# AIGC-Audio/AudioGPT

Hardware: AMD Instinct MI355X
Metric: generated audio-seconds/sec (10s clip, 100 DDIM steps) [3 independent batches of 8 prompts in flight per GPU] (higher is better)
Workload: dtype bf16x3; 1 GPU; Make-An-Audio T2A batch=8/GPU, 100 DDIM steps, CFG 1.5, UNet+VAE+HiFi-GAN(16k), fp32 storage, bf16x3-split MFMA (hi/lo, fp32 accumulate; meets the fp32 parity gates); prompts_per_gpu=8, ddim_steps=100, mel_frames=624, hipgraph=True, batches_in_flight=3, cfg_lanes=1, concurrency_hint=3, parallelism=prompt-sharded x1 (RCCL bcast cond / gather wav)

## Files before the change

### audiogpt_amd/_lib.py

```python
import ctypes as C
import os

import torch

_HERE = os.path.dirname(os.path.abspath(__file__))
LIB_PATH = os.environ.get("AUDIOGPT_AMD_LIB") or os.path.join(_HERE, "libaudiogpt_mi355x.so")


class MaaError(RuntimeError):
    pass


class maa_tensor(C.Structure):
    _fields_ = [("name", C.c_char_p), ("data", C.POINTER(C.c_float)), ("ndim", C.c_int), ("shape", C.c_int64 * 6)]


class maa_prof_row(C.Structure):
    _fields_ = [("name", C.c_char * 48), ("launches", C.c_int64), ("ms", C.c_double), ("flops", C.c_double),
                ("bytes", C.c_double)]


class maa_unet_config(C.Structure):
    _fields_ = [("in_channels", C.c_int), ("out_channels", C.c_int), ("model_channels", C.c_int),
                ("num_res_blocks", C.c_int),
                ("n_channel_mult", C.c_int), ("channel_mult", C.c_int * 8),
                ("n_attention_resolutions", C.c_int), ("attention_resolutions", C.c_int * 8),
                ("num_heads", C.c_int), ("num_head_channels", C.c_int),
                ("use_spatial_transformer", C.c_int), ("transformer_depth", C.c_int), ("context_dim", C.c_int),
                ("legacy", C.c_int), ("resblock_updown", C.c_int), ("add_context_to_emb", C.c_int)]


class maa_ddim_args(C.Structure):
    _fields_ = [("S", C.c_int), ("B", C.c_int), ("C", C.c_int), ("H", C.c_int), ("W", C.c_int),
                ("scale", C.c_float),
                ("d_cond", C.c_void_p), ("d_uncond", C.c_void_p), ("L", C.c_int),
                ("d_concat", C.c_void_p), ("Cc", C.c_int),
                ("h_timesteps", C.POINTER(C.c_int32)), ("h_alphas", C.POINTER(C.c_float)),
                ("h_alphas_prev", C.POINTER(C.c_float)), ("use_graph", C.c_int),
                ("d_mask", C.c_void_p), ("d_x0", C.c_void_p), ("d_noise_q", C.c_void_p),
                ("h_sqrt_ac", C.POINTER(C.c_float)), ("h_sqrt_1mac", C.POINTER(C.c_float)),
                ("h_sigmas", C.POINTER(C.c_float)), ("d_noise_p", C.c_void_p), ("temperature", C.c_float),
                ("log_every_t", C.c_int), ("n_log", C.c_int), ("d_log_x", C.c_void_p), ("d_log_x0", C.c_void_p),
                ("split_kh", C.c_int), ("split_kw", C.c_int), ("split_sh", C.c_int), ("split_sw", C.c_int),
                ("h_split_weight", C.POINTER(C.c_float))]


class maa_ddpm_args(C.Structure):
    _fields_ = [("loop", maa_ddim_args), ("start", C.c_int), ("n", C.c_int), ("clip_denoised", C.c_int),
                ("h_sqrt_recip_ac", C.POINTER(C.c_float)), ("h_sqrt_recipm1_ac", C.POINTER(C.c_float)),
                ("h_coef1", C.POINTER(C.c_float)), ("h_coef2", C.POINTER(C.c_float)), ("h_logvar", C.POINTER(C.c_float)),
                ("h_sqrt_ac", C.POINTER(C.c_float)), ("h_sqrt_1mac", C.POINTER(C.c_float)),
                ("h_temperature", C.POINTER(C.c_float))]


class maa_vae_config(C.Structure):
    _fields_ = [("ch", C.c_int), ("out_ch", C.c_int), ("in_channels", C.c_int), ("z_channels", C.c_int),
                ("embed_dim", C.c_int), ("resolution", C.c_int), ("num_res_blocks", C.c_int), ("double_z", C.c_int),
                ("n_ch_mult", C.c_int), ("ch_mult", C.c_int * 8),
                ("n_attn_resolutions", C.c_int), ("attn_resolutions", C.c_int * 8)]


class maa_vocoder_config(C.Structure):
    _fields_ = [("kind", C.c_int), ("num_mels", C.c_int), ("upsample_initial_channel", C.c_int),
                ("n_upsamples", C.c_int), ("upsample_rates", C.c_int * 8), ("upsample_kernel_sizes", C.c_int * 8),
                ("n_kernels", C.c_int), ("resblock_kernel_sizes", C.c_int * 8),
                ("n_dilations", C.c_int), ("resblock_dilation_sizes", (C.c_int * 8) * 8),
                ("snake_beta", C.c_int), ("snake_logscale", C.c_int),
                ("use_pitch_embed", C.c_int), ("sampling_rate", C.c_int), ("harmonic_num", C.c_int),
                ("resblock", C.c_int)]


class maa_diffnet_config(C.Structure):
    _fields_ = [("in_dims", C.c_int), ("hidden_size", C.c_int), ("residual_layers", C.c_int),
                ("residual_channels", C.c_int), ("dilation_cycle_length", C.c_int)]


class maa_pitch_extractor_config(C.Structure):
    _fields_ = [("n_mel_bins", C.c_int), ("hidden_size", C.c_int), ("predictor_hidden", C.c_int), ("predictor_kernel", C.c_int),
                ("conv_layers", C.c_int), ("ffn_padding_same", C.c_int), ("use_uv", C.c_int), ("pitch_norm", C.c_int),
                ("f0_mean", C.c_float), ("f0_std", C.c_float)]


class maa_encoder_config(C.Structure):
    _fields_ = [("kind", C.c_int), ("layers", C.c_int), ("width", C.c_int), ("heads", C.c_int), ("mlp_dim", C.c_int),
                ("d_proj", C.c_int), ("vocab", C.c_int), ("max_positions", C.c_int), ("patch", C.c_int),
                ("image", C.c_int), ("ln_eps", C.c_float)]


class maa_clap_audio_config(C.Structure):
    _fields_ = [("mel_bins", C.c_int), ("n_blocks", C.c_int), ("channels", C.c_int * 8), ("out_emb", C.c_int),
                ("d_proj", C.c_int), ("bn_eps", C.c_float)]


class maa_spectral_config(C.Structure):
    _fields_ = [("n_fft", C.c_int), ("hop", C.c_int), ("n_freq", C.c_int), ("n_mels", C.c_int), ("pad_mode", C.c_int),
                ("power", C.c_int), ("log_kind", C.c_int), ("amin", C.c_float), ("ref", C.c_float), ("out_layout", C.c_int)]


class maa_plms_args(C.Structure):
    _fields_ = [("B", C.c_int), ("T", C.c_int), ("K_step", C.c_int), ("interval", C.c_int), ("timesteps", C.c_int),
                ("d_cond", C.c_void_p), ("h_alphas_cumprod", C.POINTER(C.c_float)), ("use_graph", C.c_int)]


class maa_ds_ddpm_args(C.Structure):
    _fields_ = [("B", C.c_int), ("T", C.c_int), ("start", C.c_int), ("n", C.c_int), ("timesteps", C.c_int),
                ("clip_denoised", C.c_int), ("use_graph", C.c_int),
                ("d_cond", C.c_void_p), ("d_noise", C.c_void_p),
                ("h_sqrt_recip_ac", C.POINTER(C.c_float)), ("h_sqrt_recipm1_ac", C.POINTER(C.c_float)),
                ("h_coef1", C.POINTER(C.c_float)), ("h_coef2", C.POINTER(C.c_float)), ("h_sigma", C.POINTER(C.c_float))]


EXPORTS = [
    "maa_last_error", "maa_version", "maa_ctx_create", "maa_ctx_destroy", "maa_ctx_synchronize",
    "maa_ctx_set_stream", "maa_ctx_set_precision", "maa_ctx_set_cfg_split", "maa_ctx_set_concurrency", "maa_ctx_reload_tuning", "maa_ctx_workspace_bytes", "maa_prof_begin", "maa_prof_end", "maa_unet_create", "maa_unet_destroy",
    "maa_unet_set_context", "maa_unet_forward", "maa_ddim_update", "maa_ddim_sample", "maa_ddim_stochastic_encode", "maa_ddim_decode",
    "maa_ldm_plms_sample", "maa_ddpm_sample", "maa_ddpm_update",
    "maa_vae_create",
    "maa_vae_destroy", "maa_vae_decode", "maa_vae_decode_spec", "maa_vae_encode_moments", "maa_vocoder_create", "maa_vocoder_destroy",
    "maa_vocoder_forward", "maa_vocoder_forward_f0", "maa_diffnet_create", "maa_diffnet_destroy", "maa_diffnet_forward",
    "maa_plms_sample", "maa_ds_ddpm_sample", "maa_ds_ddpm_update",
    "maa_pitch_extractor_create", "maa_pitch_extractor_destroy", "maa_pitch_extractor_forward",
    "maa_encoder_create", "maa_encoder_destroy", "maa_encoder_text", "maa_encoder_image",
    "maa_encoder_text_cls", "maa_clap_audio_create", "maa_clap_audio_destroy", "maa_clap_audio_embed", "maa_clap_similarity",
    "maa_spectral_create", "maa_spectral_destroy", "maa_spectral_forward", "maa_resampler_create", "maa_resampler_destroy",
    "maa_resampler_forward", "maa_op_linear", "maa_op_conv", "maa_op_groupnorm", "maa_op_layernorm",
    "maa_op_attention", "maa_op_attention_ex", "maa_op_conv_transpose1d", "maa_op_snake_aa", "maa_op_bench_conv", "maa_calib",
    "maa_op_mrf_pair", "maa_op_groupnorm_ex", "maa_op_layernorm_ex", "maa_op_split32",
    "maa_unet_forward_split", "maa_op_unfold", "maa_op_fold",
]

_lib = None


def load():
    global _lib
    if _lib is not None:
        return _lib
    if not os.path.exists(LIB_PATH):
        raise MaaError("%s not found -- run `python -m audiogpt_amd.build` (hipcc, gfx950)" % LIB_PATH)
    try:
        lib = C.CDLL(LIB_PATH)
    except OSError as e:
        raise MaaError("cannot load %s: %s" % (LIB_PATH, e))
    vp, ci, cf, fp = C.c_void_p, C.c_int, C.c_float, C.POINTER(C.c_float)
    lib.maa_last_error.restype = C.c_char_p
    lib.maa_version.restype = C.c_char_p
    sig = {
        "maa_ctx_create": [ci, vp, C.POINTER(vp)],
        "maa_ctx_destroy": [vp],
        "maa_ctx_synchronize": [vp],
        "maa_ctx_set_stream": [vp, vp],
        "maa_ctx_workspace_bytes": [vp, C.POINTER(C.c_size_t)],
        "maa_ctx_set_precision": [vp, ci],
        "maa_ctx_set_cfg_split": [vp, ci],
        "maa_ctx_set_concurrency": [vp, ci],
        "maa_ctx_reload_tuning": [vp],
        "maa_prof_begin": [vp, ci],
        "maa_prof_end": [vp, C.POINTER(maa_prof_row), ci, C.POINTER(ci)],
        "maa_unet_create": [vp, C.POINTER(maa_unet_config), C.POINTER(maa_tensor), ci, C.POINTER(vp)],
        "maa_unet_destroy": [vp],
        "maa_unet_set_context": [vp, vp, vp, ci, ci],
        "maa_unet_forward": [vp, vp, vp, vp, ci, ci, ci, vp],
        "maa_ddim_update": [vp, vp, vp, vp, cf, vp, C.c_int64, vp, vp],
        "maa_ddim_sample": [vp, vp, C.POINTER(maa_ddim_args), vp],
        "maa_ddim_stochastic_encode": [vp, vp, ci, cf, vp, vp, fp, fp, ci, vp, ci, ci, ci, ci, vp],
        "maa_ddim_decode": [vp, vp, C.POINTER(maa_ddim_args), ci, vp],
        "maa_ldm_plms_sample": [vp, vp, C.POINTER(maa_ddim_args), vp],
        "maa_ddpm_sample": [vp, vp, C.POINTER(maa_ddpm_args), vp],
        "maa_ddpm_update": [vp, vp, vp, vp, fp, fp, fp, fp, fp, ci, vp, cf, ci, ci, ci, ci, ci, vp, vp],
        "maa_vae_create": [vp, C.POINTER(maa_vae_config), C.POINTER(maa_tensor), ci, C.POINTER(vp)],
        "maa_vae_destroy": [vp],
        "maa_vae_decode": [vp, vp, vp, ci, ci, ci, cf, vp],
        "maa_vae_decode_spec": [vp, vp, vp, ci, ci, ci, cf, vp],
        "maa_vae_encode_moments": [vp, vp, vp, ci, ci, ci, vp],
        "maa_vocoder_create": [vp, C.POINTER(maa_vocoder_config), C.POINTER(maa_tensor), ci, C.POINTER(vp)],
        "maa_vocoder_destroy": [vp],
        "maa_vocoder_forward": [vp, vp, vp, ci, ci, vp],
        "maa_vocoder_forward_f0": [vp, vp, vp, vp, vp, vp, ci, ci, vp],
        "maa_diffnet_create": [vp, C.POINTER(maa_diffnet_config), C.POINTER(maa_tensor), ci, C.POINTER(vp)],
        "maa_diffnet_destroy": [vp],
        "maa_diffnet_forward": [vp, vp, vp, vp, vp, ci, ci, vp],
        "maa_plms_sample": [vp, vp, C.POINTER(maa_plms_args), vp],
        "maa_ds_ddpm_sample": [vp, vp, C.POINTER(maa_ds_ddpm_args), vp],
        "maa_ds_ddpm_update": [vp, vp, vp, vp, fp, fp, fp, fp, fp, ci, ci, ci, ci, ci, vp],
        "maa_pitch_extractor_create": [vp, C.POINTER(maa_pitch_extractor_config), C.POINTER(maa_tensor), ci, C.POINTER(vp)],
        "maa_pitch_extractor_destroy": [vp],
        "maa_pitch_extractor_forward": [vp, vp, vp, ci, ci, vp, vp, vp],
        "maa_encoder_create": [vp, C.POINTER(maa_encoder_config), C.POINTER(maa_tensor), ci, C.POINTER(vp)],
        "maa_encoder_destroy": [vp],
        "maa_encoder_text": [vp, vp, vp, ci, ci, vp],
        "maa_encoder_image": [vp, vp, vp, ci, vp],
        "maa_encoder_text_cls": [vp, vp, vp, ci, ci, vp],
        "maa_clap_audio_create": [vp, C.POINTER(maa_clap_audio_config), C.POINTER(maa_tensor), ci, C.POINTER(vp)],
        "maa_clap_audio_destroy": [vp],
        "maa_clap_audio_embed": [vp, vp, vp, ci, ci, vp, vp],
        "maa_clap_similarity": [vp, vp, vp, ci, ci, ci, cf, vp],
        "maa_spectral_create": [vp, C.POINTER(maa_spectral_config), fp, fp, C.POINTER(vp)],
        "maa_spectral_destroy": [vp],
        "maa_spectral_forward": [vp, vp, vp, ci, ci, vp],
        "maa_resampler_create": [vp, ci, ci, ci, ci, fp, C.POINTER(vp)],
        "maa_resampler_destroy": [vp],
        "maa_resampler_forward": [vp, vp, vp, ci, ci, vp],
        "maa_op_linear": [vp, vp, ci, ci, fp, fp, ci, ci, vp, vp, ci],
        "maa_op_conv": [vp, vp, ci, ci, ci, ci, fp, fp, ci, ci, ci, ci, ci, ci, ci, cf, vp, ci, ci, vp, vp, ci],
        "maa_op_groupnorm": [vp, vp, ci, ci, ci, fp, fp, cf, ci, vp],
        "maa_op_layernorm": [vp, vp, ci, ci, fp, fp, cf, vp],
        "maa_op_attention": [vp, vp, vp, vp, ci, ci, ci, ci, ci, cf, vp],
        "maa_op_attention_ex": [vp, vp, ci, ci, vp, ci, ci, vp, ci, ci, ci, ci, ci, ci, ci, cf, vp, ci, ci, ci],
        "maa_op_conv_transpose1d": [vp, vp, ci, ci, ci, fp, fp, ci, ci, ci, cf, vp],
        "maa_op_snake_aa": [vp, vp, ci, ci, ci, fp, fp, ci, vp],
        "maa_op_bench_conv": [vp, ci, ci, ci, ci, ci, ci, ci, ci, C.POINTER(C.c_float)],
        "maa_calib": [vp, ci, C.POINTER(C.c_double)],
        "maa_op_mrf_pair": [vp, vp, ci, ci, ci, fp, fp, ci, ci, cf, fp, fp, ci, ci, cf, cf, ci, vp],
        "maa_op_groupnorm_ex": [vp, vp, ci, ci, vp, ci, ci, ci, ci, ci, fp, fp, cf, ci, vp, ci, vp],
        "maa_op_layernorm_ex": [vp, vp, ci, ci, fp, fp, cf, vp, ci],
        "maa_op_split32": [vp, vp, ci, ci, cf, ci, vp],
        "maa_unet_forward_split": [vp, vp, vp, vp, vp, ci, ci, ci, ci, ci, ci, ci, fp, vp],
        "maa_op_unfold": [vp, vp, ci, ci, ci, ci, ci, ci, ci, ci, vp],
        "maa_op_fold": [vp, vp, fp, ci, ci, ci, ci, ci, ci, ci, ci, vp],
    }
    for name, argtypes in sig.items():
        fn = getattr(lib, name)
        fn.argtypes = argtypes
        fn.restype = ci
    _lib = lib
    return lib


def check(status):
    if status != 0:
        raise MaaError("libaudiogpt_mi355x: %s (status %d)" % (load().maa_last_error().decode(), status))


def host_f32(t):
    t = t.detach().to(device="cpu", dtype=torch.float32).contiguous()
    return t, C.cast(t.data_ptr(), C.POINTER(C.c_float))


def tensor_list(state_dict):
    items = list(state_dict.items())
    arr = (maa_tensor * len(items))()
    keep = []
    for i, (name, t) in enumerate(items):
        ht, ptr = host_f32(t)
        bname = name.encode()
        keep.append((ht, bname))
        arr[i].name = bname
        arr[i].data = ptr
        arr[i].ndim = ht.dim()
        for d, s in enumerate(ht.shape):
            arr[i].shape[d] = s
    return arr, len(items), keep


def dptr(t):
    assert t.is_cuda and t.dtype == torch.float32 and t.is_contiguous(), (t.device, t.dtype, t.is_contiguous())
    return C.c_void_p(t.data_ptr())
```

### audiogpt_amd/backend.py

```python
import ctypes as C
import threading
import weakref

import numpy as np
import torch

from . import _lib as L


def default_precision():
    import os
    p = os.environ.get("AUDIOGPT_AMD_PRECISION", "bf16x3")
    if p not in Context.PRECISIONS:
        raise ValueError("AUDIOGPT_AMD_PRECISION must be one of %s" % sorted(Context.PRECISIONS))
    return p


_contexts = weakref.WeakSet()


def reload_tuning():
    for c in list(_contexts):
        c.reload_tuning()


def _f32(t, device):
    return t.detach().to(device=device, dtype=torch.float32).contiguous()


class Context:

    PRECISIONS = {"f32": 0, "bf16x3": 1, "bf16": 2}

    def __init__(self, device="cuda:0", stream=None, precision="f32"):
        self.lib = L.load()
        if not torch.cuda.is_available():
            raise L.MaaError("no MI355X visible: the HIP backend has no CPU fallback")
        self.device = torch.device(device)
        idx = self.device.index if self.device.index is not None else torch.cuda.current_device()
        self.device = torch.device("cuda", idx)
        torch.cuda.set_device(idx)
        self._stream = stream
        sp = C.c_void_p(stream.cuda_stream) if stream is not None else None
        h = C.c_void_p()
        L.check(self.lib.maa_ctx_create(idx, sp, C.byref(h)))
        self.h = h
        self.lock = threading.RLock()
        self.precision = "f32"
        self.set_precision(precision)
        _contexts.add(self)

    def reload_tuning(self):
        if getattr(self, "h", None):
            with self.lock:
                L.check(self.lib.maa_ctx_reload_tuning(self.h))

    def set_precision(self, precision):
        L.check(self.lib.maa_ctx_set_precision(self.h, self.PRECISIONS[precision]))
        self.precision = precision

    def set_cfg_split(self, mode):
        L.check(self.lib.maa_ctx_set_cfg_split(self.h, -1 if mode is None else int(bool(mode))))

    def set_concurrency(self, n):
        L.check(self.lib.maa_ctx_set_concurrency(self.h, -1 if n is None else int(n)))

    def synchronize(self):
        L.check(self.lib.maa_ctx_synchronize(self.h))

    def workspace_bytes(self):
        n = C.c_size_t()
        L.check(self.lib.maa_ctx_workspace_bytes(self.h, C.byref(n)))
        return n.value

    def prof_begin(self, detail=False):
        L.check(self.lib.maa_prof_begin(self.h, int(detail)))

    def prof_end(self):
        rows = (L.maa_prof_row * 512)()
        n = C.c_int()
        L.check(self.lib.maa_prof_end(self.h, rows, 512, C.byref(n)))
        return {rows[i].name.decode(): dict(launches=int(rows[i].launches), ms=rows[i].ms, flops=rows[i].flops,
                                            bytes=rows[i].bytes) for i in range(n.value)}

    def calib(self):
        out = {}
        for kind, key in ((0, "mfma_bf16_tflops"), (1, "copy_gbs"), (2, "l2_read_gbs"), (3, "infinity_cache_read_gbs")):
            v = C.c_double()
            L.check(self.lib.maa_calib(self.h, kind, C.byref(v)))
            out[key] = v.value
        return out

    def close(self):
        if getattr(self, "h", None):
            self.lib.maa_ctx_destroy(self.h)
            self.h = None

    def __del__(self):
        try:
            self.close()
        except Exception:
            pass

    def op_linear(self, a, w, b=None, geglu=False, res=None, split_out=False):
        a = _f32(a, self.device)
        M, K = a.shape
        N = w.shape[0]
        wt, wp = L.host_f32(w)
        bt, bp = L.host_f32(b) if b is not None else (None, None)
        y = torch.empty(M, N // 2 if geglu else N, device=self.device)
        r = _f32(res, self.device) if res is not None else None
        assert r is None or tuple(r.shape) == tuple(y.shape)
        L.check(self.lib.maa_op_linear(self.h, L.dptr(a), M, K, wp, bp, N, int(geglu), L.dptr(y),
                                       L.dptr(r) if r is not None else None, int(split_out)))
        return y

    def op_conv(self, x, w, b=None, stride=1, pad=0, dil=1, up=False, leaky=0.0, out_hw=None, rowadd=None, res=None,
                split_out=False):
        x = _f32(x, self.device)
        B, Cin, H, W = x.shape
        Cout, _, KH, KW = w.shape
        if out_hw is None:
            He, We = (2 * H, 2 * W) if up else (H, W)
            ph = pad if KH > 1 else 0
            Ho = (He + 2 * ph - dil * (KH - 1) - 1) // stride + 1
            Wo = (We + 2 * pad - dil * (KW - 1) - 1) // stride + 1
        else:
            Ho, Wo = out_hw
        wt, wp = L.host_f32(w)
        bt, bp = L.host_f32(b) if b is not None else (None, None)
        y = torch.empty((B, Ho, Wo, Cout) if split_out else (B, Cout, Ho, Wo), device=self.device)
        ra = _f32(rowadd, self.device) if rowadd is not None else None
        r = _f32(res, self.device) if res is not None else None
        assert ra is None or tuple(ra.shape) == (B, Cout)
        assert r is None or tuple(r.shape) == (B, Cout, Ho, Wo)
        L.check(self.lib.maa_op_conv(self.h, L.dptr(x), B, Cin, H, W, wp, bp, Cout, KH, KW, stride, pad, dil,
                                     int(up), float(leaky), L.dptr(y), Ho, Wo, L.dptr(ra) if ra is not None else None,
                                     L.dptr(r) if r is not None else None, int(split_out)))
        return y

    def op_groupnorm(self, x, gamma, beta, eps, silu=False):
        x = _f32(x, self.device)
        B, Cc = x.shape[:2]
        HW = int(np.prod(x.shape[2:]))
        gt, gp = L.host_f32(gamma)
        bt, bp = L.host_f32(beta)
        y = torch.empty_like(x)
        L.check(self.lib.maa_op_groupnorm(self.h, L.dptr(x), B, Cc, HW, gp, bp, float(eps), int(silu), L.dptr(y)))
        return y

    def op_layernorm(self, x, gamma, beta, eps=1e-5):
        x = _f32(x, self.device)
        rows, Cc = x.reshape(-1, x.shape[-1]).shape
        gt, gp = L.host_f32(gamma)
        bt, bp = L.host_f32(beta)
        y = torch.empty_like(x)
        L.check(self.lib.maa_op_layernorm(self.h, L.dptr(x), rows, Cc, gp, bp, float(eps), L.dptr(y)))
        return y

    def op_attention(self, q, k, v, heads, alpha):
        q, k, v = _f32(q, self.device), _f32(k, self.device), _f32(v, self.device)
        B, Nq, Cc = q.shape
        Nk = k.shape[1]
        y = torch.empty_like(q)
        L.check(self.lib.maa_op_attention(self.h, L.dptr(q), L.dptr(k), L.dptr(v), B, heads, Cc // heads, Nq, Nk,
                                          float(alpha), L.dptr(y)))
        return y

    def op_attention_ex(self, q, ldq, hsq, k, ldk, hsk, v, ldv, hsv, B, heads, dh, Nq, Nk, alpha, out, ldo,
                        out_split=0, causal=0):
        for t in (q, k, v, out):
            assert t.is_cuda and t.dtype == torch.float32, (t.device, t.dtype)
        L.check(self.lib.maa_op_attention_ex(self.h, C.c_void_p(q.data_ptr()), int(ldq), int(hsq),
                                             C.c_void_p(k.data_ptr()), int(ldk), int(hsk),
                                             C.c_void_p(v.data_ptr()), int(ldv), int(hsv), int(B), int(heads), int(dh),
                                             int(Nq), int(Nk), float(alpha), C.c_void_p(out.data_ptr()), int(ldo),
                                             int(out_split), int(causal)))
        return out

    def op_groupnorm_ex(self, x1, ld1, C1, x2, ld2, C2, B, HW, groups, gamma, beta, eps, silu, out, out_split=0, raw=None):
        for t in (x1, x2, out, raw):
            assert t is None or (t.is_cuda and t.dtype == torch.float32), (t.device, t.dtype)
        gt, gp = L.host_f32(gamma)
        bt, bp = L.host_f32(beta)
        assert gt.numel() == C1 + C2 and bt.numel() == C1 + C2
        ptr = lambda t: C.c_void_p(t.data_ptr()) if t is not None else None
        L.check(self.lib.maa_op_groupnorm_ex(self.h, ptr(x1), int(ld1), int(C1), ptr(x2), int(ld2), int(C2), int(B), int(HW),
                                             int(groups), gp, bp, float(eps), int(silu), ptr(out), int(out_split), ptr(raw)))
        return out

    def op_layernorm_ex(self, x, gamma, beta, eps=1e-5, out_split=0):
        x = _f32(x, self.device)
        rows, Cc = x.reshape(-1, x.shape[-1]).shape
        gt, gp = L.host_f32(gamma)
        bt, bp = L.host_f32(beta)
        y = torch.empty_like(x)
        L.check(self.lib.maa_op_layernorm_ex(self.h, L.dptr(x), rows, Cc, gp, bp, float(eps), L.dptr(y), int(out_split)))
        return y

    def op_split32(self, x, slope=1.0, unpack=False):
        x = _f32(x, self.device)
        rows, Cc = x.shape
        y = torch.empty_like(x)
        L.check(self.lib.maa_op_split32(self.h, L.dptr(x), rows, Cc, float(slope), int(unpack), L.dptr(y)))
        return y

    def op_unfold(self, x, ks, stride):
        x = _f32(x, self.device)
        B, Cc, H, W = x.shape
        (kh, kw), (sh, sw) = ks, stride
        n = ((H - kh) // sh + 1) * ((W - kw) // sw + 1) if min(kh, kw, sh, sw) > 0 else 0
        y = torch.empty(B * max(n, 0), Cc, kh, kw, device=self.device)
        L.check(self.lib.maa_op_unfold(self.h, L.dptr(x), B, Cc, H, W, kh, kw, sh, sw, L.dptr(y)))
        return y

    def op_fold(self, crops, weight, size, ks, stride):
        crops = _f32(crops, self.device)
        (H, W), (kh, kw), (sh, sw) = size, ks, stride
        wt, wp = L.host_f32(weight)
        n = wt.shape[1]
        assert wt.shape[0] == kh * kw and crops.shape[0] % n == 0 and tuple(crops.shape[2:]) == (kh, kw)
        B, Cc = crops.shape[0] // n, crops.shape[1]
        y = torch.empty(B, Cc, H, W, device=self.device)
        L.check(self.lib.maa_op_fold(self.h, L.dptr(crops), wp, B, Cc, H, W, kh, kw, sh, sw, L.dptr(y)))
        return y

    def op_conv_transpose1d(self, x, w, b, stride, leaky=0.0):
        x = _f32(x, self.device)
        B, Cin, Ln = x.shape
        _, Cout, k = w.shape
        wt, wp = L.host_f32(w)
        bt, bp = L.host_f32(b)
        y = torch.empty(B, Cout, Ln * stride, device=self.device)
        L.check(self.lib.maa_op_conv_transpose1d(self.h, L.dptr(x), B, Cin, Ln, wp, bp, Cout, k, stride, float(leaky),
                                                 L.dptr(y)))
        return y

    def op_mrf_pair(self, x, w1, b1, d1, slope1, w2=None, b2=None, d2=1, slope2=0.0, out_scale=1.0, out=None):
        x = _f32(x, self.device)
        B, Cc, Ln = x.shape
        w1t, w1p = L.host_f32(w1)
        b1t, b1p = L.host_f32(b1) if b1 is not None else (None, None)
        w2t, w2p = L.host_f32(w2) if w2 is not None else (None, None)
        b2t, b2p = L.host_f32(b2) if b2 is not None else (None, None)
        y = _f32(out, self.device).clone() if out is not None else torch.empty_like(x)
        assert y.shape == x.shape
        L.check(self.lib.maa_op_mrf_pair(self.h, L.dptr(x), B, Cc, Ln, w1p, b1p, w1.shape[2], int(d1), float(slope1), w2p, b2p,
                                         w2.shape[2] if w2 is not None else 1, int(d2), float(slope2), float(out_scale),
                                         int(out is not None), L.dptr(y)))
        return y

    def op_bench_conv(self, B, H, W, Cin, Cout, taps=9, pre_split=True, iters=20):
        ms = C.c_float()
        L.check(self.lib.maa_op_bench_conv(self.h, B, H, W, Cin, Cout, taps, int(pre_split), iters, C.byref(ms)))
        return ms.value

    def op_snake_aa(self, x, alpha, beta, logscale):
        x = _f32(x, self.device)
        B, Cc, Ln = x.shape
        at, ap = L.host_f32(alpha)
        bt, bp = L.host_f32(beta)
        y = torch.empty_like(x)
        L.check(self.lib.maa_op_snake_aa(self.h, L.dptr(x), B, Cc, Ln, ap, bp, int(logscale), L.dptr(y)))
        return y


def _fill(arr, values):
# ... 934 lines not shown
```

### audiogpt_amd/csrc/api.cpp

```cpp
#include "models.h"

#include <cstdint>
#include <cstring>
#include <memory>

namespace maa {
const char* last_error_cstr();
}

struct maa_ctx {
    maa::Ctx c;
    bool owns_stream = false;
};
struct maa_unet {
    std::unique_ptr<maa::UNet> m;
};
struct maa_vae {
    std::unique_ptr<maa::VAE> m;
};
struct maa_vocoder {
    std::unique_ptr<maa::Vocoder> m;
};
struct maa_diffnet {
    std::unique_ptr<maa::DiffNet> m;
// ... 521 lines not shown
}

int maa_encoder_create(maa_ctx* ctx, const maa_encoder_config* cfg, const maa_tensor* tensors, int n_tensors,
                       maa_encoder** out) {
    return guarded([&] {
        bind(ctx);
        MAA_CHECK(cfg && out && cfg->kind >= 0 && cfg->kind <= 2 && cfg->layers > 0 && cfg->width > 0 && cfg->heads > 0 &&
                      cfg->width % cfg->heads == 0 && cfg->width % 4 == 0 && cfg->mlp_dim > 0 && cfg->d_proj > 0 &&
                      cfg->d_proj % 4 == 0 && cfg->ln_eps > 0.f,
                  "bad encoder config");
        if (cfg->kind != 1)
            MAA_CHECK(cfg->vocab > 0 && cfg->max_positions > 0, "bad text encoder config");
        else
            MAA_CHECK(cfg->patch > 0 && cfg->image > 0 && cfg->image % cfg->patch == 0, "bad image encoder config");
        auto sd = to_state_dict(tensors, n_tensors);
        auto* e = new maa_encoder;
        e->m.reset(new maa::Encoder(*cfg, sd, ctx->c.dtype));
        *out = e;
    });
}
int maa_encoder_destroy(maa_encoder* e) {
    return guarded([&] { delete e; });
}
int maa_encoder_text(maa_ctx* ctx, maa_encoder* e, const int* d_ids, int B, int L, float* d_out) {
    return guarded([&] {
        bind(ctx);
        MAA_CHECK(e && d_ids && d_out && B > 0 && L > 0, "bad encoder_text arguments");
        e->m->text(ctx->c, d_ids, B, L, d_out);
    });
}
int maa_encoder_image(maa_ctx* ctx, maa_encoder* e, const float* d_img, int B, float* d_out) {
    return guarded([&] {
        bind(ctx);
        MAA_CHECK(e && d_img && d_out && B > 0, "bad encoder_image arguments");
        e->m->image(ctx->c, d_img, B, d_out);
    });
}

int maa_encoder_text_cls(maa_ctx* ctx, maa_encoder* e, const int* d_ids, int B, int L, float* d_out) {
    return guarded([&] {
        bind(ctx);
        MAA_CHECK(e && d_ids && d_out && B > 0 && L > 0, "bad encoder_text_cls arguments");
        e->m->text_cls(ctx->c, d_ids, B, L, d_out);
    });
}

int maa_clap_audio_create(maa_ctx* ctx, const maa_clap_audio_config* cfg, const maa_tensor* tensors, int n_tensors,
                          maa_clap_audio** out) {
    return guarded([&] {
        bind(ctx);
        MAA_CHECK(cfg && out && cfg->mel_bins > 0 && cfg->n_blocks > 0 && cfg->n_blocks <= 8 && cfg->out_emb > 0 &&
                      cfg->d_proj > 0 && cfg->d_proj % 4 == 0 && cfg->bn_eps > 0.f,
                  "bad clap_audio config");
        for (int i = 0; i < cfg->n_blocks; ++i) MAA_CHECK(cfg->channels[i] > 0, "bad clap_audio channel list");
        auto sd = to_state_dict(tensors, n_tensors);
        auto* a = new maa_clap_audio;
        a->m.reset(new maa::ClapAudio(*cfg, sd, ctx->c.dtype));
        *out = a;
    });
}
int maa_clap_audio_destroy(maa_clap_audio* a) {
    return guarded([&] { delete a; });
}
int maa_clap_audio_embed(maa_ctx* ctx, maa_clap_audio* a, const float* d_logmel, int B, int T, float* d_embedding,
                         float* d_z) {
    return guarded([&] {
        bind(ctx);
        MAA_CHECK(a && d_logmel && d_z && B > 0 && T > 0, "bad clap_audio_embed arguments");
        a->m->embed(ctx->c, d_logmel, B, T, d_embedding, d_z);
    });
}
int maa_clap_similarity(maa_ctx* ctx, const float* d_audio, const float* d_text, int Na, int Nt, int D, float scale,
                        float* d_out) {
    return guarded([&] {
        bind(ctx);
        MAA_CHECK(d_audio && d_text && d_out && Na > 0 && Nt > 0 && D > 0, "bad clap_similarity arguments");
        maa::launch_similarity(ctx->c, d_audio, d_text, Na, Nt, D, scale, d_out);
    });
}

int maa_spectral_create(maa_ctx* ctx, const maa_spectral_config* cfg, const float* h_basis, const float* h_melw,
                        maa_spectral** out) {
    return guarded([&] {
        bind(ctx);
        MAA_CHECK(cfg && h_basis && h_melw && out, "bad spectral arguments");
        MAA_CHECK(cfg->n_fft > 0 && cfg->n_fft % 4 == 0 && cfg->hop > 0 && cfg->hop % 4 == 0 && cfg->n_freq == cfg->n_fft / 2 + 1 &&
                      cfg->n_mels > 0 && (cfg->pad_mode == 0 || cfg->pad_mode == 1) && (cfg->power == 1 || cfg->power == 2) &&
                      (cfg->log_kind == 0 || cfg->log_kind == 1) && cfg->amin > 0.f && (cfg->out_layout == 0 || cfg->out_layout == 1),
                  "bad spectral config (n_fft and hop must be multiples of 4)");
        auto* s = new maa_spectral;
        s->m.reset(new maa::Spectral(*cfg, h_basis, h_melw));
        *out = s;
    });
}
int maa_spectral_destroy(maa_spectral* s) {
    return guarded([&] { delete s; });
}
int maa_spectral_forward(maa_ctx* ctx, maa_spectral* s, const float* d_wav, int B, int n, float* d_out) {
    return guarded([&] {
        bind(ctx);
        MAA_CHECK(s && d_wav && d_out && B > 0 && n > 0, "bad spectral_forward arguments");
        MAA_CHECK(s->m->config().pad_mode == 0 || n > s->m->config().n_fft / 2, "signal too short for reflect padding");
        s->m->forward(ctx->c, d_wav, B, n, d_out);
    });
}

int maa_resampler_create(maa_ctx* ctx, int orig, int neu, int width, int klen, const float* h_kernels, maa_resampler** out) {
    return guarded([&] {
        bind(ctx);
        MAA_CHECK(out && h_kernels && orig > 0 && neu > 0 && width > 0 && klen > 0, "bad resampler arguments");
        auto* r = new maa_resampler;
        r->m.reset(new maa::Resampler(orig, neu, width, klen, h_kernels));
        *out = r;
    });
}
int maa_resampler_destroy(maa_resampler* r) {
    return guarded([&] { delete r; });
}
int maa_resampler_forward(maa_ctx* ctx, maa_resampler* r, const float* d_wav, int B, int n, float* d_out) {
    return guarded([&] {
        bind(ctx);
        MAA_CHECK(r && d_wav && d_out && B > 0 && n > 0, "bad resampler_forward arguments");
        r->m->forward(ctx->c, d_wav, B, n, d_out);
    });
}

static bool op_presplit(const maa::Ctx& c, int channels, bool other_prologue) {
    return c.tune.op_presplit && c.dtype != 0 && channels % 32 == 0 && !other_prologue;
}

int maa_op_linear(maa_ctx* ctx, const float* d_a, int M, int K, const float* h_w, const float* h_bias, int N,
                  int geglu, float* d_y, const float* d_res, int c_split) {
    return guarded([&] {
        bind(ctx);
        MAA_CHECK(d_a && h_w && d_y && M > 0 && K > 0 && N > 0, "bad op_linear arguments");
        MAA_CHECK(!c_split || N % 32 == 0, "op_linear: split32 output needs a multiple of 32 columns");
        MAA_CHECK(!geglu || (!d_res && !c_split), "op_linear: GEGLU takes neither a residual nor split32 output here");
        OneShot s;
        s.add("w", h_w, {N, K});
        if (h_bias) s.add("b", h_bias, {N});
        maa::WeightStore ws(ctx->c.dtype != 0);
        maa::Ctx& c = ctx->c;
        MAA_CHECK(!geglu || h_bias, "geglu needs a bias");
        maa::PackedW pw = geglu ? ws.pack_geglu(s.sd, "w", "b") : ws.pack_conv(s.sd, "w", h_bias ? "b" : "", 1, 1);
        const bool pre = op_presplit(c, K, false);
        maa::run_sized(c, [&] {
            const float* a = d_a;
            if (pre) {
                float* sp = c.ws.alloc_f((size_t)M * K);
                maa::launch_split32_pack(c, d_a, M, K, sp);
                a = sp;
            }
            maa::linear_into(c, a, K, M, K, pw, d_res, N, d_y, geglu ? N / 2 : N, geglu, 0, pre ? M : 0, c_split);
        });
        MAA_HIP(hipStreamSynchronize(c.stream));
    });
}

int maa_op_conv(maa_ctx* ctx, const float* d_x, int B, int Cin, int H, int W, const float* h_w, const float* h_bias,
                int Cout, int KH, int KW, int stride, int pad, int dil, int upsample2, float leaky_slope, float* d_y,
                int Ho, int Wo, const float* d_rowadd, const float* d_res, int c_split) {
    return guarded([&] {
        bind(ctx);
        MAA_CHECK(d_x && h_w && d_y, "bad op_conv arguments");
        const bool extras = d_rowadd || d_res || c_split;
        MAA_CHECK(!extras || !upsample2, "op_conv: row add, residual and split32 output are not combined with the upsample");
        MAA_CHECK(!c_split || Cout % 32 == 0, "op_conv: split32 output needs a multiple of 32 channels");
        OneShot s;
        s.add("w", h_w, {Cout, Cin, KH, KW});
        if (h_bias) s.add("b", h_bias, {Cout});
        maa::WeightStore ws(ctx->c.dtype != 0);
        maa::Ctx& c = ctx->c;
        maa::PackedW pw = ws.pack_conv(s.sd, "w", h_bias ? "b" : "", KH, KW);
        maa::PackedW pw4;
        if (upsample2 && KH == 3 && KW == 3 && stride == 1 && pad == 1 && dil == 1 && leaky_slope == 0.f)
            pw4 = ws.pack_conv_up2(s.sd, "w", h_bias ? "b" : "");
        maa::run_sized(c, [&] {
            maa::T4 x = maa::alloc_t(c, B, H, W, Cin);
            maa::launch_nchw_to_nhwc(c, d_x, B, Cin, H * W, x.p);
            if (!pw4.w && op_presplit(c, Cin, leaky_slope != 0.f)) {
                maa::T4 xs = maa::alloc_t(c, B, H, W, Cin);
                maa::launch_split32_pack(c, x.p, (long long)B * H * W, Cin, xs.p);
                xs.split = true;
                x = xs;
            }
            if (x.split && Cout <= 4 && h_bias && KH == 3 && KW == 3 && stride == 1 && pad == 1 && dil == 1 && !upsample2 && !extras && c.tune.up2) {
                maa::PackedW pn = ws.pack_narrow3x3(s.sd, "w", "b");
                if (maa::launch_narrow_conv3x3(c, x.p, Cin, B, H, W, Cin, pn.w, pn.bias, Cout, d_y)) return;
            }
            maa::T4 y = maa::alloc_t(c, B, Ho, Wo, Cout);
            maa::ConvOpt o;
            o.KH = KH;
            o.KW = KW;
            o.stride = stride;
            o.pad = pad;
            o.dil = dil;
            o.up = upsample2;
            if (leaky_slope != 0.f) {
                o.a_act = 1;
                o.a_slope = leaky_slope;
            }
            o.rowadd = d_rowadd;
            o.ld_rowadd = Cout;
            if (d_res) {
                maa::T4 r = maa::alloc_t(c, B, Ho, Wo, Cout);
                maa::launch_nchw_to_nhwc(c, d_res, B, Cout, Ho * Wo, r.p);
                o.res = r.p;
            }
            if (c_split) {
                o.c_split = 1;
                y.p = d_y;
                maa::conv_into(c, x, nullptr, pw, o, y);
                return;
            }
            if (!(pw4.w && maa::conv_up2_into(c, x, pw4, y))) maa::conv_into(c, x, nullptr, pw, o, y);
            maa::launch_nhwc_to_nchw(c, y.p, B, Cout, Ho * Wo, d_y, Cout);
        });
        MAA_HIP(hipStreamSynchronize(c.stream));
    });
}

int maa_calib(maa_ctx* ctx, int kind, double* out_value) {
    return guarded([&] {
        bind(ctx);
        MAA_CHECK(out_value && kind >= 0 && kind <= 3, "bad calib arguments");
        *out_value = maa::calib_run(ctx->c, kind);
    });
}

int maa_op_groupnorm(maa_ctx* ctx, const float* d_x, int B, int C, int HW, const float* h_gamma, const float* h_beta,
                     float eps, int silu, float* d_y) {
    return guarded([&] {
        bind(ctx);
        MAA_CHECK(d_x && h_gamma && h_beta && d_y, "bad op_groupnorm arguments");
        maa::WeightStore ws(ctx->c.dtype != 0);
        maa::Ctx& c = ctx->c;
        float* g = ws.upload(std::vector<float>(h_gamma, h_gamma + C));
        float* b = ws.upload(std::vector<float>(h_beta, h_beta + C));
        maa::run_sized(c, [&] {
            maa::T4 x = maa::alloc_t(c, B, 1, HW, C), y = maa::alloc_t(c, B, 1, HW, C);
            maa::launch_nchw_to_nhwc(c, d_x, B, C, HW, x.p);
            maa::launch_groupnorm(c, x.p, C, C, nullptr, 0, 0, B, HW, 32, g, b, eps, silu, y.p);
            maa::launch_nhwc_to_nchw(c, y.p, B, C, HW, d_y, C);
        });
        MAA_HIP(hipStreamSynchronize(c.stream));
    });
}

int maa_op_layernorm(maa_ctx* ctx, const float* d_x, int rows, int C, const float* h_gamma, const float* h_beta,
                     float eps, float* d_y) {
    return guarded([&] {
        bind(ctx);
        MAA_CHECK(d_x && h_gamma && h_beta && d_y, "bad op_layernorm arguments");
        maa::WeightStore ws(ctx->c.dtype != 0);
        maa::Ctx& c = ctx->c;
        float* g = ws.upload(std::vector<float>(h_gamma, h_gamma + C));
        float* b = ws.upload(std::vector<float>(h_beta, h_beta + C));
        maa::launch_layernorm(c, d_x, rows, C, g, b, eps, d_y);
        MAA_HIP(hipStreamSynchronize(c.stream));
    });
}

int maa_op_attention(maa_ctx* ctx, const float* d_q, const float* d_k, const float* d_v, int B, int heads, int dh,
                     int Nq, int Nk, float alpha, float* d_y) {
    return guarded([&] {
        bind(ctx);
        MAA_CHECK(d_q && d_k && d_v && d_y, "bad op_attention arguments");
        maa::Ctx& c = ctx->c;
        const int C = heads * dh;
        maa::run_sized(c, [&] {
            maa::attention_into(c, d_q, C, dh, d_k, C, dh, d_v, C, dh, B, heads, dh, Nq, Nk, alpha, d_y, C);
        });
        MAA_HIP(hipStreamSynchronize(c.stream));
    });
}

int maa_op_attention_ex(maa_ctx* ctx, const float* d_q, int ldq, int hsq, const float* d_k, int ldk, int hsk,
                        const float* d_v, int ldv, int hsv, int B, int heads, int dh, int Nq, int Nk, float alpha,
                        float* d_y, int ldo, int out_split, int causal) {
    return guarded([&] {
        bind(ctx);
        MAA_CHECK(d_q && d_k && d_v && d_y, "bad op_attention_ex arguments");
        MAA_CHECK(B > 0 && heads > 0 && dh > 0 && Nq > 0 && Nk > 0, "bad op_attention_ex sizes");
        MAA_CHECK(ldq >= dh && ldk >= dh && ldv >= dh && hsq >= 0 && hsk >= 0 && hsv >= 0 && ldo >= heads * dh,
                  "bad op_attention_ex strides");
        maa::Ctx& c = ctx->c;
        maa::run_sized(c, [&] {
            maa::attention_into(c, d_q, ldq, hsq, d_k, ldk, hsk, d_v, ldv, hsv, B, heads, dh, Nq, Nk, alpha, d_y, ldo,
                                out_split, causal);
        });
        MAA_HIP(hipStreamSynchronize(c.stream));
    });
}

int maa_op_groupnorm_ex(maa_ctx* ctx, const float* d_x1, int ld1, int C1, const float* d_x2, int ld2, int C2, int B, int HW,
                        int groups, const float* h_gamma, const float* h_beta, float eps, int silu, float* d_y, int out_split,
                        float* d_raw) {
    return guarded([&] {
        bind(ctx);
        MAA_CHECK(d_x1 && h_gamma && h_beta && d_y, "bad op_groupnorm_ex arguments");
        MAA_CHECK(B > 0 && HW > 0 && groups > 0 && C1 > 0 && C2 >= 0 && eps > 0.f, "bad op_groupnorm_ex sizes");
        MAA_CHECK((C2 == 0) == (d_x2 == nullptr), "op_groupnorm_ex: a second source needs both d_x2 and C2");
        MAA_CHECK(ld1 >= C1 && (C2 == 0 || ld2 >= C2), "bad op_groupnorm_ex strides");
        const int C = C1 + C2;
        MAA_CHECK(C % groups == 0 && C / groups <= 256 && C1 % 4 == 0 && C2 % 4 == 0 && ld1 % 4 == 0 && ld2 % 4 == 0,
                  "op_groupnorm_ex: channels and pitches in whole float4s, at most 256 channels per group");
// ... 272 lines not shown
```

### audiogpt_amd/csrc/blocks.cpp

```cpp
#include "blocks.h"

namespace maa {

void conv_into(Ctx& ctx, const T4& x1, const T4* x2, const PackedW& w, const ConvOpt& o, T4& out) {
    IGemm p;
    p.a1 = x1.p;
    p.lda1 = x1.ld ? x1.ld : x1.C;
    p.C1 = x1.C;
    if (x2) {
        MAA_CHECK(x2->B == x1.B && x2->H == x1.H && x2->W == x1.W, "concat sources differ in shape");
        p.a2 = x2->p;
        p.lda2 = x2->C;
        p.C2 = x2->C;
    }
    p.Hin = x1.H;
    p.Win = x1.W;
    p.Hout = out.H;
    p.Wout = out.W;
    p.KH = o.KH;
    p.KW = o.KW;
    p.sh = p.sw = o.stride;
    p.dh = p.dw = o.dil;
    p.pw = o.pad;
    p.ph = o.pad_h >= 0 ? o.pad_h : (o.KH > 1 ? o.pad : 0);
    p.up = o.up;
    p.a_act = o.a_act;
    p.a_slope = o.a_slope;
    p.b = w.w;
    p.ldb = w.ld;
    p.b_nk = w.nk;
    p.b_split = w.split;
    if (x1.split) {
        MAA_CHECK(!x2, "a split source cannot be concatenated");
        p.a_split = 1;
    }
    p.M = out.B * out.H * out.W;
    p.K = o.KH * o.KW * (p.C1 + p.C2);
    MAA_CHECK(p.K == w.K, "conv weight K mismatch");
    p.N = o.geglu ? w.N : out.C;
    MAA_CHECK(p.N <= w.N, "conv weight N mismatch");
    p.bias = w.bias;
    p.rowadd = o.rowadd;
    p.ld_rowadd = o.ld_rowadd;
    p.res = o.res;
    p.ldr = out.C;
    p.act = o.act;
    p.act_slope = o.act_slope;
    p.out_scale = o.out_scale;
    p.accumulate = o.accumulate;
    p.geglu = o.geglu;
    p.c_split = o.c_split;
    p.c = out.p;
    p.ldc = out.C;
    p.c2 = o.c2;
    p.ldc2 = out.C;
    p.c2_slope = o.c2_slope;
    launch_igemm(ctx, p);
}

void conv1d_same(Ctx& ctx, const T4& x, const PackedW& w, int k, int dil, float leaky, const float* res, float out_scale,
                 int accumulate, T4& out) {
    if (x.C == out.C && !x.split && x.H == 1 && x.ld == 0 &&
        launch_halo_conv1d(ctx, x.p, x.B, x.W, x.C, w, k, dil, leaky != 0.f ? leaky : 1.f, res, out_scale, accumulate, out.p))
        return;
    ConvOpt o;
    o.KH = 1;
    o.KW = k;
    o.dil = dil;
    o.pad = (k * dil - dil) / 2;
    o.pad_h = 0;
    if (leaky != 0.f) {
        o.a_act = 1;
        o.a_slope = leaky;
    }
    o.res = res;
    o.out_scale = out_scale;
    o.accumulate = accumulate;
    conv_into(ctx, x, nullptr, w, o, out);
}

void mrf_pair(Ctx& ctx, const T4& x, const PackedW& w1, int k1, int d1, float slope1, const PackedW& w2, int k2, int d2,
              float slope2, const float* res, float out_scale, int accumulate, T4& t1, T4& out) {
    if (!x.split && x.ld == 0 &&
        launch_halo_pair(ctx, x.p, x.B, x.W, x.C, w1, k1, d1, slope1 != 0.f ? slope1 : 1.f, w2, k2, d2,
                         slope2 != 0.f ? slope2 : 1.f, res, out_scale, accumulate, out.p))
        return;
    conv1d_same(ctx, x, w1, k1, d1, slope1, nullptr, 1.f, 0, t1);
    conv1d_same(ctx, t1, w2, k2, d2, slope2, res, out_scale, accumulate, out);
}

void check_convtr_polyphase(int k, int stride) {
    const std::string at = " (kernel " + std::to_string(k) + ", stride " + std::to_string(stride) + ")";
    MAA_CHECK(stride >= 1 && k >= stride, "conv-transpose needs stride >= 1 and kernel >= stride" + at);
    MAA_CHECK(k % stride == 0, "conv-transpose kernel must be a multiple of the stride" + at);
    MAA_CHECK((k - stride) % 2 == 0, "conv-transpose kernel - stride must be even: padding (kernel - stride) / 2 gives length * stride outputs" + at);
    MAA_CHECK((stride - 1 + (k - stride) / 2) / stride <= 1,
              "conv-transpose polyphase carry (stride - 1 + (kernel - stride) / 2) / stride must be 0 or 1" + at);
}

bool conv_up2_into(Ctx& ctx, const T4& x, const PackedW& w4, T4& out) {
    if (!ctx.tune.up2 || !w4.w || w4.phase_rows == 0 || ctx.dtype == 0 || x.split || x.C % 32 != 0 || x.ld != 0) return false;
    MAA_CHECK(out.B == x.B && out.H == 2 * x.H && out.W == 2 * x.W && out.C == w4.N, "conv_up2: output shape");
    const size_t mk = ctx.ws.mark();
    const long long M = x.rows();
    float* xs = ctx.ws.alloc_f((size_t)x.numel());
    float* planes = ctx.ws.alloc_f((size_t)4 * M * out.C);
    IGemm p;
    p.a1 = xs;
    p.lda1 = x.C;
    p.C1 = x.C;
    p.a_split = 1;
    p.Hin = p.Hout = x.H;
    p.Win = p.Wout = x.W;
    p.KH = p.KW = 2;
    p.ph = p.pw = 1;
    p.b = w4.w;
    p.ldb = w4.ld;
    p.b_nk = w4.nk;
    p.b_split = w4.split;
    p.M = (int)M;
    p.K = 4 * x.C;
    p.N = out.C;
    p.bias = w4.bias;
    p.c = planes;
    p.ldc = out.C;
    p.ldr = out.C;
    p.ldc2 = out.C;
    p.zeros = ctx.zeros;
    MAA_CHECK(p.K == w4.K, "conv_up2 weight K mismatch");
    if (!ctx.ws.dry) launch_split32_pack(ctx, x.p, M, x.C, xs);
    const bool ok = launch_igemm_pp_up2(ctx, p, w4.Npad, (long long)w4.phase_rows * w4.ld);
    if (ok) launch_pixel_shuffle2(ctx, planes, x.B, x.H, x.W, out.C, out.p);
    ctx.ws.release(mk);
    return ok;
}

void linear_into(Ctx& ctx, const float* a, int lda, long long rows, int K, const PackedW& w, const float* res,
                 int ldr, float* out, int ldc, int geglu, int a_act, long long a_split_rows, int c_split, int act) {
    IGemm p;
    p.a1 = a;
    p.lda1 = lda;
    p.C1 = K;
    p.Hout = 1;
    p.Wout = 1;
    p.M = (int)rows;
    p.K = K;
    MAA_CHECK(K == w.K, "linear weight K mismatch");
    p.N = w.N;
    p.b = w.w;
    p.ldb = w.ld;
    p.b_nk = w.nk;
    p.b_split = w.split;
    if (a_split_rows > 0) {
        p.a_split = 1;
    }
    p.bias = w.bias;
    p.res = res;
    p.ldr = ldr;
    p.geglu = geglu;
    p.a_act = a_act;
    p.c_split = c_split;
    p.act = act;
    p.c = out;
    p.ldc = ldc;
    launch_igemm(ctx, p);
}

void attention_into(Ctx& ctx, const float* q, int ldq, int hsq, const float* k, int ldk, int hsk, const float* v,
                    int ldv, int hsv, int B, int heads, int dh, int Nq, int Nk, float alpha, float* out, int ldo,
                    int out_split, int causal) {
    MAA_CHECK(!causal || Nq == Nk, "causal attention needs Nq == Nk");
    if (launch_flash_attention(ctx, q, ldq, hsq, k, ldk, hsk, v, ldv, hsv, B, heads, dh, Nq, Nk, alpha, out, ldo,
                               out_split, causal))
        return;
    MAA_CHECK(!out_split, "split32 attention output needs the fused kernel");
    const size_t mk = ctx.ws.mark();
    const int ldS = (Nk + 3) / 4 * 4;
    float* S = ctx.ws.alloc_f((size_t)B * heads * Nq * ldS);
    IGemm p;
    p.a1 = q;
    p.lda1 = ldq;
    p.C1 = dh;
    p.M = Nq;
    p.K = dh;
    p.N = Nk;
    p.b = k;
    p.ldb = ldk;
    p.b_nk = 1;
    p.Z = B * heads;
    p.zin = heads;
    p.a_so = (long long)Nq * ldq;
    p.a_si = hsq;
    p.b_so = (long long)Nk * ldk;
    p.b_si = hsk;
    p.c_so = (long long)heads * Nq * ldS;
    p.c_si = (long long)Nq * ldS;
    p.alpha = alpha;
    p.c = S;
    p.ldc = ldS;
    launch_igemm(ctx, p);
    launch_softmax(ctx, S, (long long)B * heads * Nq, Nk, ldS, causal ? Nq : 0);
    IGemm r;
    r.a1 = S;
    r.lda1 = ldS;
    r.C1 = Nk;
    r.M = Nq;
    r.K = Nk;
    r.N = dh;
    r.b = v;
    r.ldb = ldv;
    r.Z = B * heads;
    r.zin = heads;
    r.a_so = (long long)heads * Nq * ldS;
    r.a_si = (long long)Nq * ldS;
    r.b_so = (long long)Nk * ldv;
    r.b_si = hsv;
    r.c_so = (long long)Nq * ldo;
    r.c_si = dh;
    r.c = out;
    r.ldc = ldo;
    launch_igemm(ctx, r);
    ctx.ws.release(mk);
}

}
```

### audiogpt_amd/csrc/blocks.h

```cpp
#pragma once
#include "maa_internal.h"

namespace maa {

struct T4 {
    float* p = nullptr;
    int B = 0, H = 0, W = 0, C = 0;
    bool split = false;
    int ld = 0;
    long long numel() const { return (long long)B * H * W * C; }
    long long rows() const { return (long long)B * H * W; }
};

inline T4 alloc_t(Ctx& ctx, int B, int H, int W, int C) {
    T4 t;
    t.B = B;
    t.H = H;
    t.W = W;
    t.C = C;
    t.p = ctx.ws.alloc_f((size_t)t.numel());
    return t;
}

struct ConvOpt {
    int KH = 1, KW = 1, stride = 1, pad = 0, dil = 1;
    int pad_h = -1;
    int up = 0;
    int a_act = 0;
    float a_slope = 0.f;
    const float* rowadd = nullptr;
    int ld_rowadd = 0;
    const float* res = nullptr;
    int act = 0;
    float act_slope = 0.f;
    float out_scale = 1.f;
    int accumulate = 0;
    int geglu = 0;
    int c_split = 0;
    float* c2 = nullptr;
    float c2_slope = 1.f;
};

void conv_into(Ctx& ctx, const T4& x1, const T4* x2, const PackedW& w, const ConvOpt& o, T4& out);
void conv1d_same(Ctx& ctx, const T4& x, const PackedW& w, int k, int dil, float leaky, const float* res, float out_scale,
                 int accumulate, T4& out);
void mrf_pair(Ctx& ctx, const T4& x, const PackedW& w1, int k1, int d1, float slope1, const PackedW& w2, int k2, int d2,
              float slope2, const float* res, float out_scale, int accumulate, T4& t1, T4& out);
void check_convtr_polyphase(int k, int stride);
bool conv_up2_into(Ctx& ctx, const T4& x, const PackedW& w4, T4& out);
void linear_into(Ctx& ctx, const float* a, int lda, long long rows, int K, const PackedW& w, const float* res,
                 int ldr, float* out, int ldc, int geglu = 0, int a_act = 0, long long a_split_rows = 0,
                 int c_split = 0, int act = 0);

void attention_into(Ctx& ctx, const float* q, int ldq, int hsq, const float* k, int ldk, int hsk, const float* v,
                    int ldv, int hsv, int B, int heads, int dh, int Nq, int Nk, float alpha, float* out, int ldo,
                    int out_split = 0, int causal = 0);

inline bool split_for_gemm(const Ctx& ctx, int C) { return ctx.dtype != 0 && C % 32 == 0; }

struct PrecisionGuard {
    Ctx& ctx;
    int saved;
    PrecisionGuard(Ctx& c, int mode) : ctx(c), saved(c.dtype) { c.dtype = mode; }
    ~PrecisionGuard() { ctx.dtype = saved; }
};

template <class F>
void run_sized(Ctx& ctx, F&& f) {
    ctx.ws.reset();
    ctx.ws.dry = true;
    try {
        f();
    } catch (...) {
        ctx.ws.dry = false;
        throw;
    }
    ctx.ws.dry = false;
    const size_t need = ctx.ws.mark_high();
    if (need > ctx.ws.capacity()) ctx.ws.reserve(need + need / 8);
    ctx.ws.reset();
    f();
}

}
```

### audiogpt_amd/csrc/igemm_dispatch.cpp

```cpp
#include "maa_internal.h"

namespace maa {

namespace {

bool al16(const void* q) { return (reinterpret_cast<uintptr_t>(q) & 15) == 0; }

bool gather_aligned(const IGemm& p, int chunk) {
    const int taps = p.KH * p.KW, Ctot = p.C1 + p.C2;
    bool fast = (taps == 1 ? (p.C2 == 0 ? (Ctot % 4 == 0 || p.lda1 >= (Ctot + 3) / 4 * 4)
                                        : (p.C1 % chunk == 0 && Ctot % 4 == 0))
                           : (Ctot % chunk == 0 && p.C1 % chunk == 0)) &&
                p.lda1 % 4 == 0 && al16(p.a1) && p.a_so % 4 == 0 && p.a_si % 4 == 0;
    if (p.C2 > 0) fast = fast && p.lda2 % 4 == 0 && al16(p.a2);
    return fast;
}

constexpr int kTileM[5] = {128, 128, 64, 256, 128}, kTileN[5] = {128, 64, 64, 32, 32};

struct TileKnobs {
    double eff[3] = {1.00, 0.92, 0.80};
    double conc[3] = {0.55, 0.85, 1.00};
};

bool plan_bf16(const Ctx& ctx, const IGemm& p, IGemmPlan& pl) {
    if (!p.b_nk) {
        MAA_CHECK(!p.a_split && !p.b_split, "split operands need the k-contiguous bf16 engine");
        return false;
    }
    const int taps = p.KH * p.KW, Ctot = p.C1 + p.C2;
    bool fast;
    if (p.a_split)
        fast = p.C2 == 0 && Ctot % 32 == 0 && p.lda1 % 32 == 0 && al16(p.a1) && p.Z == 1 && p.a_act == 0;
    else
        fast = gather_aligned(p, 32);
    if (p.b_split)
        fast = fast && p.ldb % 32 == 0 && al16(p.b) && p.K % 32 == 0 && p.ldb >= p.K && p.Z == 1;
    else
        fast = fast && p.ldb % 4 == 0 && al16(p.b) && p.b_so % 4 == 0 && p.b_si % 4 == 0 && p.ldb >= (p.K + 3) / 4 * 4;
    fast = fast && p.K == taps * Ctot && (p.a_act == 0 || p.a_act == 1);
    if (!fast) {
        MAA_CHECK(!p.a_split && !p.b_split, "split operand given to a problem the bf16 engine cannot take");
        return false;
    }
    MAA_CHECK(!(p.c_split || p.c2) || p.N % 32 == 0, "split32 outputs are whole 32-channel lines");
    const int ncols = p.N * (p.geglu ? 2 : 1);
    pl.fast = true;
    pl.Nb = ncols;
    if (p.geglu) {
        if (ncols % 64 != 0) return false;
        pl.cfg = 0;
    } else if (ncols <= 32) {
        pl.cfg = (long long)((p.M + 255) / 256) * p.Z < 128 ? 4 : 3;
    } else {
        pl.cfg = choose_tile(p.M, ncols, p.Z, true, ctx.kept_full() ? 1 : 0);
    }
    pl.engine = IGemmPlan::BF16_REG;
    if (p.a_split && p.b_split && pl.cfg < 3 && !ctx.tune.no_dma) {
        if (!igemm_pp_takes(ctx, p, pl) && !igemm_pp1_takes(ctx, p, pl) && !igemm_dma2_takes(ctx, p, pl)) igemm_dma_takes(ctx, p, pl);
    }
    if (pl.S > 1) {
        const int bm = pl.engine == IGemmPlan::DMA2 ? 128 : 256, bn = pl.engine == IGemmPlan::DMA2 ? 128 : pl.bn;
        const long long tiles = (long long)((p.M + bm - 1) / bm) * ((ncols + bn - 1) / bn);
        pl.slab_floats = (size_t)(tiles * pl.S * bm * bn);
    }
    return true;
}

const char* plan_row(const Ctx& ctx, const IGemm& p, const IGemmPlan& pl, char (&buf)[64], double& flops, double& bytes) {
    const int ncols = p.N * (p.geglu ? 2 : 1), taps = p.KH * p.KW;
    flops = 2.0 * p.M * (double)ncols * p.K * p.Z;
    bytes = 4.0 * ((double)p.K * ncols + (double)p.M * p.N * p.Z);
    const bool detail = ctx.prof && ctx.prof->detail;
    const char* mode = ctx.dtype == 2 ? "_bf16" : "_bf16x3";
    const char* splitk = pl.S > 1 ? ",splitK" : "";
    switch (pl.engine) {
        case IGemmPlan::PP:
        case IGemmPlan::PP1: {
            const bool one = pl.engine == IGemmPlan::PP1;
            if (detail) std::snprintf(buf, sizeof(buf), "p%c%d M%d N%d K%d S%d", one ? 'q' : 'p', pl.bn, p.M, ncols, p.K, pl.S);
            else std::snprintf(buf, sizeof(buf), "igemm_pp%s%s<256x%d%s>", one ? "1" : "", mode, pl.bn, splitk);
            break;
        }
        case IGemmPlan::DMA2:
            if (detail) std::snprintf(buf, sizeof(buf), "b2 M%d N%d K%d t%d", p.M, ncols, p.K, taps);
            else std::snprintf(buf, sizeof(buf), "igemm_dma2%s<128x128%s>", mode, splitk);
            break;
        case IGemmPlan::DMA:
        case IGemmPlan::BF16_REG: {
            const bool dma = pl.engine == IGemmPlan::DMA;
            if (detail) std::snprintf(buf, sizeof(buf), "b%c%d M%d N%d K%d t%d Z%d", dma ? 'd' : 'g', pl.cfg, p.M, ncols, p.K, taps, p.Z);
            else std::snprintf(buf, sizeof(buf), "igemm%s%s<%dx%d>", dma ? "_dma" : "", mode, kTileM[pl.cfg], kTileN[pl.cfg]);
            break;
        }
        default:
            if (detail) std::snprintf(buf, sizeof(buf), "ig%d M%d N%d K%d t%d Z%d%s", pl.cfg, p.M, ncols, p.K, taps, p.Z, p.b_nk ? "T" : "");
            else std::snprintf(buf, sizeof(buf), "igemm_f32<%dx%d>", kTileM[pl.cfg], kTileN[pl.cfg]);
            break;
    }
    return buf;
}

}

int choose_tile(long long M, long long N, int Z, bool bf16, int mode) {
    static const TileKnobs k;
    const int max_occ[3] = {bf16 ? 2 : 3, bf16 ? 2 : 4, 4};
    int best = 0;
    double best_cost = 1e300;
    for (int c = 0; c < 3; ++c) {
        const int bm = kTileM[c], bn = kTileN[c];
        const long long blocks = ((M + bm - 1) / bm) * ((N + bn - 1) / bn) * Z;
        const long long per_cu = (blocks + 255) / 256;
        const int co = (int)(per_cu < max_occ[c] ? per_cu : max_occ[c]);
        const double cost = mode == 1 ? (double)blocks * bm * bn / k.eff[c]
                                      : (double)per_cu * bm * bn / (k.eff[c] * k.conc[co >= 3 ? 2 : co - 1]);
        if (cost < best_cost) {
            best_cost = cost;
            best = c;
        }
    }
    return best;
}

int fit_slices(int nchunks, int S) {
    if (S < 1) S = 1;
    if (S > nchunks) S = nchunks;
    for (; S > 1; --S) {
        const int cps = (nchunks + S - 1) / S;
        if ((nchunks + cps - 1) / cps == S) break;
    }
    return S;
}

IGemmPlan igemm_plan(const Ctx& ctx, const IGemm& p) {
    IGemmPlan pl;
    if (ctx.dtype != 0 && plan_bf16(ctx, p, pl)) return pl;
    pl = IGemmPlan();
    if (ctx.ws.dry) return pl;
    MAA_CHECK(p.M > 0 && p.N > 0 && p.K > 0, "empty igemm");
    MAA_CHECK(!p.c_split, "split32 output asked of a problem only the fp32 engine can take");
    const int taps = p.KH * p.KW, Ctot = p.C1 + p.C2;
    MAA_CHECK(p.K <= taps * Ctot && p.K > (taps - 1) * Ctot, "igemm K mismatch");
    MAA_CHECK(p.a_act == 0 || p.a_act == 1, "igemm A activation");
    pl.fast = gather_aligned(p, 16);
    if (p.Z > 1) MAA_CHECK(p.C2 == 0, "batched igemm takes one A source");
    MAA_CHECK(pl.fast || p.K == taps * Ctot, "padded K needs the aligned gather");
    const int ncols = p.N * (p.geglu ? 2 : 1);
    pl.Nb = ncols;
    MAA_CHECK(p.ldb % 4 == 0 && al16(p.b) && p.b_so % 4 == 0 && p.b_si % 4 == 0, "B operand alignment");
    if (!p.b_nk) {
        pl.Nb = (ncols + 3) / 4 * 4;
        if (pl.Nb > p.ldb) pl.Nb = p.ldb / 4 * 4;
    } else {
        MAA_CHECK(p.ldb >= (p.K + 3) / 4 * 4, "B [N][K] rows must be padded to a multiple of 4");
    }
    if (p.geglu) {
        MAA_CHECK(ncols % 64 == 0, "geglu needs packed N multiple of 64");
        pl.cfg = 0;
    } else if (ncols <= 32) {
        pl.cfg = 3;
    } else {
        pl.cfg = choose_tile(p.M, ncols, p.Z, false);
    }
    return pl;
}

void launch_igemm(const Ctx& ctx, const IGemm& p_in) {
    IGemm p = p_in;
    p.zeros = ctx.zeros;
    MAA_CHECK(p.zeros != nullptr, "context has no zero page");
    const IGemmPlan pl = igemm_plan(ctx, p);
    const size_t mk = ctx.ws.mark();
    float* part = pl.slab_floats ? ctx.ws.alloc_f(pl.slab_floats) : nullptr;
    if (!ctx.ws.dry) {
        char row[64];
        double flops, bytes;
        const char* name = plan_row(ctx, p, pl, row, flops, bytes);
        ProfScope prof(ctx, name, flops, bytes);
        switch (pl.engine) {
            case IGemmPlan::PP: launch_igemm_pp(ctx, p, pl, part); break;
            case IGemmPlan::PP1: launch_igemm_pp1(ctx, p, pl, part); break;
            case IGemmPlan::DMA2: launch_igemm_dma2(ctx, p, pl, part); break;
            case IGemmPlan::DMA: launch_igemm_dma(ctx, p, pl); break;
            case IGemmPlan::BF16_REG: launch_igemm_bf16_reg(ctx, p, pl); break;
            case IGemmPlan::F32: launch_igemm_f32(ctx, p, pl); break;
        }
        MAA_HIP(hipGetLastError());
    }
    ctx.ws.release(mk);
}

}
```

### audiogpt_amd/csrc/igemm_epilogue.h

```cpp
#pragma once
#include "igemm_device.h"
#include "maa_internal.h"

namespace maa {

__device__ __forceinline__ float fast_erff(float x) {
    const float t = fminf(fabsf(x), 4.0f);
    const float s = t * t;
    float r = -5.654105860e-04f;
    r = fmaf(r, s, 4.923277665e-03f);
    r = fmaf(r, s, -2.671638510e-02f);
    r = fmaf(r, s, 1.128036441e-01f);
    r = fmaf(r, s, -3.761234978e-01f);
    r = fmaf(r, s, 1.128379127e+00f);
    const float small = r * t;
    float q = 1.330939039e-05f;
    q = fmaf(q, t, -3.175720346e-04f);
    q = fmaf(q, t, 3.436867598e-03f);
    q = fmaf(q, t, -2.262198592e-02f);
    q = fmaf(q, t, 1.033189800e-01f);
    q = fmaf(q, t, 6.390933195e-01f);
    q = fmaf(q, t, 1.125925949e+00f);
    q = fmaf(q, t, 7.569686250e-04f);
    const float large = 1.0f - __builtin_amdgcn_exp2f(q * -1.4426950408889634f);
    return copysignf(t < 1.0f ? small : large, x);
}

__device__ __forceinline__ void settle(float& x) { asm volatile("" : "+v"(x)); }

__device__ __forceinline__ void store_split_pair(float* row, int n, float v) {
    const __bf16 h = (__bf16)v;
    const unsigned hb = __builtin_bit_cast(unsigned short, h);
    const __bf16 l = (__bf16)(v - __builtin_bit_cast(float, hb << 16));
    const unsigned lb = __builtin_bit_cast(unsigned short, l);
    const bool even = (n & 1) == 0;
    const unsigned mine = even ? lb : hb;
    const unsigned theirs = (unsigned)__builtin_amdgcn_update_dpp(0, (int)mine, 0xB1, 0xF, 0xF, false);
    unsigned* o = reinterpret_cast<unsigned*>(reinterpret_cast<unsigned short*>(row) + (n >> 5) * 64 + ((n & 31) & ~1) + (even ? 0 : 32));
    *o = even ? (hb | (theirs << 16)) : (theirs | (lb << 16));
}

template <int MI, int NI, bool PAIR, bool RSEL>
__device__ __forceinline__ void igemm_epilogue_impl(const IGemm& p, f32x16 (&acc)[MI][NI], int m_base, int n_base,
                                                    int lrow, int lk, long long coff, int Nb, int rpb) {
    float* cp = p.c + coff;
    const float* resp = p.res ? p.res + coff : nullptr;
    if (p.geglu) {
        if constexpr (NI % 2 == 0) {
#pragma unroll
            for (int i = 0; i < MI; ++i)
#pragma unroll
                for (int j = 0; j < NI; j += 2) {
                    const int cpk = n_base + j * 32 + lrow;
                    const int ncol = (cpk >> 6) * 32 + lrow;
                    if (cpk + 32 < Nb && ncol < p.N) {
                        float bv = p.bias ? p.bias[cpk] : 0.f;
                        float bg = p.bias ? p.bias[cpk + 32] : 0.f;
                        settle(bv);
                        settle(bg);
                        float outv[16];
#pragma unroll
                        for (int r = 0; r < 16; ++r) {
                            const float val = acc[i][j][r] * p.alpha + bv;
                            const float g = acc[i][j + 1][r] * p.alpha + bg;
                            const float gl = 0.5f * g * (1.f + fast_erff(g * 0.70710678118654752440f));
                            outv[r] = val * gl;
                        }
#pragma unroll
                        for (int r = 0; r < 16; ++r) {
                            const int m = m_base + i * 32 + (r & 3) + 8 * (r >> 2) + 4 * lk;
                            if (m < p.M) {
                                if (p.c_split)
                                    store_split_pair(cp + (long long)m * p.ldc, ncol, outv[r]);
                                else
                                    cp[(long long)m * p.ldc + ncol] = outv[r];
                            }
                        }
                    }
                }
        }
        return;
    }
#pragma unroll
    for (int i = 0; i < MI; ++i) {
        const int mb = m_base + i * 32;
        const int b0 = (mb < p.M ? mb : p.M - 1) / rpb;
        const int nextb = (b0 + 1) * rpb;
#pragma unroll
        for (int j = 0; j < NI; ++j) {
            const int n = n_base + j * 32 + lrow;
            if (n < p.N) {
                float bias = p.bias ? p.bias[n] : 0.f;
                float ra[16], rs[16], cv[16];
                long long mc[16];
#pragma unroll
                for (int r = 0; r < 16; ++r) {
                    const int m = mb + (r & 3) + 8 * (r >> 2) + 4 * lk;
                    mc[r] = m < p.M ? m : p.M - 1;
                    ra[r] = rs[r] = cv[r] = 0.f;
                }
                if (p.rowadd) {
                    if constexpr (RSEL) {
                        const float* ra0 = p.rowadd + (long long)b0 * p.ld_rowadd + n;
#pragma unroll
                        for (int r = 0; r < 16; ++r) ra[r] = ra0[mc[r] < nextb ? 0 : p.ld_rowadd];
                    } else {
#pragma unroll
                        for (int r = 0; r < 16; ++r) ra[r] = p.rowadd[(long long)((int)mc[r] / rpb) * p.ld_rowadd + n];
                    }
                }
                if (resp) {
#pragma unroll
                    for (int r = 0; r < 16; ++r) rs[r] = resp[mc[r] * p.ldr + n];
                }
                if (p.accumulate && !p.c_split) {
#pragma unroll
                    for (int r = 0; r < 16; ++r) cv[r] = cp[mc[r] * p.ldc + n];
                }
                settle(bias);
#pragma unroll
                for (int r = 0; r < 16; ++r) {
                    settle(ra[r]);
                    settle(rs[r]);
                    settle(cv[r]);
                }
                float outv[16];
#pragma unroll
                for (int r = 0; r < 16; ++r) {
                    float v = acc[i][j][r] * p.alpha + bias;
                    if (p.rowadd) v += ra[r];
                    if (resp) v += rs[r];
                    outv[r] = v;
                }
                if (p.act != 0) {
#pragma unroll
                    for (int r = 0; r < 16; ++r) {
                        float v = outv[r];
                        if (p.act == 1) v = tanhf(v);
                        else if (p.act == 2) v = fmaxf(v, 0.f);
                        else if (p.act == 3) v = 0.5f * v * (1.f + fast_erff(v * 0.70710678118654752440f));
                        else if (p.act == 4) v = v > 0.f ? v : v * p.act_slope;
                        outv[r] = v;
                    }
                }
#pragma unroll
                for (int r = 0; r < 16; ++r) {
                    float v = outv[r] * p.out_scale;
                    if (p.accumulate && !p.c_split) v += cv[r];
                    outv[r] = v;
                }
                if constexpr (PAIR) {
                    const bool even = (lrow & 1) == 0;
#pragma unroll
                    for (int rp = 0; rp < 8; ++rp) {
                        const float keep = even ? outv[2 * rp] : outv[2 * rp + 1];
                        const float give = even ? outv[2 * rp + 1] : outv[2 * rp];
                        const float got = __builtin_bit_cast(float, __builtin_amdgcn_update_dpp(0, __builtin_bit_cast(int, give), 0xB1, 0xF, 0xF, false));
                        const int r = 2 * rp + (even ? 0 : 1);
                        const int m = mb + (r & 3) + 8 * (r >> 2) + 4 * lk;
                        if (m < p.M) {
                            const f32x2 v2 = even ? f32x2{keep, got} : f32x2{got, keep};
                            *reinterpret_cast<f32x2*>(cp + (long long)m * p.ldc + (n & ~1)) = v2;
                        }
                    }
                } else {
#pragma unroll
                    for (int r = 0; r < 16; ++r) {
                        const int m = mb + (r & 3) + 8 * (r >> 2) + 4 * lk;
                        if (m < p.M) {
                            if (p.c_split)
                                store_split_pair(cp + (long long)m * p.ldc, n, outv[r]);
                            else
                                cp[(long long)m * p.ldc + n] = outv[r];
                            if (p.c2) {
                                const float w = outv[r] > 0.f ? outv[r] : outv[r] * p.c2_slope;
                                store_split_pair(p.c2 + coff + (long long)m * p.ldc2, n, w);
                            }
                        }
                    }
                }
            }
        }
    }
}

template <int MI, int NI>
__device__ __forceinline__ void igemm_epilogue(const IGemm& p, f32x16 (&acc)[MI][NI], int m_base, int n_base, int lrow,
                                               int lk, long long coff, int Nb, int rpb) {
    const bool pair = !p.geglu && !p.c_split && p.c2 == nullptr && (p.N & 1) == 0 && (p.ldc & 1) == 0 && (coff & 1) == 0 &&
                      (reinterpret_cast<uintptr_t>(p.c) & 7) == 0;
    const bool rsel = !(p.rowadd && rpb < 32);
    if (pair && rsel)
        igemm_epilogue_impl<MI, NI, true, true>(p, acc, m_base, n_base, lrow, lk, coff, Nb, rpb);
    else if (pair)
        igemm_epilogue_impl<MI, NI, true, false>(p, acc, m_base, n_base, lrow, lk, coff, Nb, rpb);
    else if (rsel)
        igemm_epilogue_impl<MI, NI, false, true>(p, acc, m_base, n_base, lrow, lk, coff, Nb, rpb);
    else
        igemm_epilogue_impl<MI, NI, false, false>(p, acc, m_base, n_base, lrow, lk, coff, Nb, rpb);
}

}
```

### audiogpt_amd/csrc/igemm_pp.hip

```cpp
#include "igemm_epilogue.h"

#include <cstdio>
#include <cstdlib>
#include <type_traits>

namespace maa {

namespace {

constexpr int BM = 256;
constexpr int NSB = 3;

__device__ __forceinline__ void wait_lgkm0() { asm volatile("s_waitcnt lgkmcnt(0)" ::: "memory"); }

struct PPArgs {
    int W, H;
    int T, KW;
    int rowstep, colstep;
    int dh, dw, ph, pw;
    int padflat;
    int NLp;
    int CAPl;
    int ntiles, tiles;
    int items;
// ... 130 lines not shown

    const int cap8 = q.CAPl >> 3;
    int a_o = 0, a_on8 = 0;
    int ci = 0, t = 0, kx = 0, shift = 0, slot = 0;
    int slot2 = 0, t2 = 0;
    long long boff2 = 0;

    auto reads = [&]() __attribute__((always_inline)) {
#pragma unroll
        for (int i = 0; i < MI; ++i) {
            const unsigned l0 = (unsigned)(a_o + shift) + (unsigned)a_r[i];
            const unsigned line = min(l0, l0 - (unsigned)q.CAPl);
            const unsigned t1 = (unsigned)lk16 ^ ((line << 3) & 0x70u);
            const bool ok = (valid9[i] >> t) & 1u;
            const unsigned base = ok ? line * 128u : zaddr;
            ah[0][i] = *reinterpret_cast<const bf16x8*>(smem + (base + (0x00u ^ t1)));
            ah[1][i] = *reinterpret_cast<const bf16x8*>(smem + (base + (0x20u ^ t1)));
            if constexpr (TERMS == 3) {
                al[0][i] = *reinterpret_cast<const bf16x8*>(smem + (base + (0x40u ^ t1)));
                al[1][i] = *reinterpret_cast<const bf16x8*>(smem + (base + (0x60u ^ t1)));
            }
        }
        const char* const bs = sB + slot * (BN * 128);
#pragma unroll
        for (int jn = 0; jn < NI; ++jn) {
#pragma unroll
            for (int ks = 0; ks < 2; ++ks) {
                bh[ks][jn] = *reinterpret_cast<const bf16x8*>(bs + jn * 4096 + b_off[0][ks]);
                if constexpr (TERMS == 3) bl[ks][jn] = *reinterpret_cast<const bf16x8*>(bs + jn * 4096 + b_off[1][ks]);
            }
        }
    };
    auto copies = [&](int j) __attribute__((always_inline)) {
        const bool live = j + (NSB - 1) < NQ;
        static_for<0, NPB>([&](auto kc) {
            constexpr int k = decltype(kc)::value;
            const bool real = live && (k * 4 + wq < BPG);
            char* dst = real ? sB + slot2 * (BN * 128) + (grp * BPG + k * 4 + wq) * 1024 : sD;
            __builtin_amdgcn_global_load_lds((gptr_t)(gpb[k] + boff2), (lptr_t)dst, 16, 0, 0);
        });
        static_for<0, NPA>([&](auto ic) {
            constexpr int i = decltype(ic)::value;
            const int pa = ((t * 2 + grp) * 4 + wq) * NPA + i;
            const bool real = t < TAPS - 1 && ci + 1 < c_end && pa < a_pieces;
            const int P = min(max(a_P0 + 8 * pa, 0), Mlast);
            const unsigned swz16 = (unsigned)((sl ^ (((r8 >> 1) + 4 * (pa & 1)) & 7)) << 4);
            const char* src = a_base + ((unsigned long long)(ci + 1) * 128u) + ((unsigned long long)(unsigned)P * lda4 + swz16);
            int pp = a_on8 + pa;
            if (pp >= cap8) pp -= cap8;
            char* dst = real ? sA + pp * 1024 : sD;
            __builtin_amdgcn_global_load_lds((gptr_t)src, (lptr_t)dst, 16, 0, 0);
        });
    };
    auto load_phase = [&](int j) __attribute__((always_inline)) {
        reads();
        copies(j);
        wait_lgkm0();
        wait_vmcnt<NP>();
    };
    auto advance = [&]() __attribute__((always_inline)) {
        shift += q.colstep;
        if (++kx == q.KW) {
            kx = 0;
            shift += q.rowstep - q.KW * q.colstep;
        }
        if (++t == TAPS) {
            t = 0;
            shift = 0;
            ++ci;
            a_o = a_on8 * 8;
            a_on8 += a_pieces;
            if (a_on8 >= cap8) a_on8 -= cap8;
        }
        if (++slot == NSB) slot = 0;
        if (++slot2 == NSB) slot2 = 0;
        boff2 += C4;
        if (++t2 == TAPS) {
            t2 = 0;
            boff2 += 128 - (long long)TAPS * C4;
        }
    };

    auto mma_phase = [&]() __attribute__((always_inline)) {
#pragma unroll
        for (int ks = 0; ks < 2; ++ks) {
            if constexpr (TERMS == 3) {
#pragma unroll
                for (int i = 0; i < MI; ++i)
#pragma unroll
                    for (int jn = 0; jn < NI; ++jn)
                        acc[i][jn] = __builtin_amdgcn_mfma_f32_32x32x16_bf16(al[ks][i], bh[ks][jn], acc[i][jn], 0, 0, 0);
#pragma unroll
                for (int i = 0; i < MI; ++i)
#pragma unroll
                    for (int jn = 0; jn < NI; ++jn)
                        acc[i][jn] = __builtin_amdgcn_mfma_f32_32x32x16_bf16(ah[ks][i], bl[ks][jn], acc[i][jn], 0, 0, 0);
            }
#pragma unroll
            for (int i = 0; i < MI; ++i)
#pragma unroll
                for (int jn = 0; jn < NI; ++jn)
                    acc[i][jn] = __builtin_amdgcn_mfma_f32_32x32x16_bf16(ah[ks][i], bh[ks][jn], acc[i][jn], 0, 0, 0);
        }
    };

    setup_item(w_cur);
    prologue();
    for (;;) {
        wait_vmcnt<0>();
        __syncthreads();
#pragma unroll
        for (int i = 0; i < MI; ++i)
#pragma unroll
            for (int j = 0; j < NI; ++j)
#pragma unroll
                for (int r = 0; r < 16; ++r) acc[i][j][r] = 0.f;
        a_o = 0;
        a_on8 = a_pieces;
        ci = c_begin;
        t = kx = shift = slot = 0;
        slot2 = t2 = NSB - 1;
        boff2 = (long long)(NSB - 1) * C4 + (long long)c_begin * 128;

        if (grp == 1) {
            __builtin_amdgcn_sched_barrier(0);
            __builtin_amdgcn_s_barrier();
            __builtin_amdgcn_sched_barrier(0);
        }
        for (int j = 0; j < NQ; ++j) {
            load_phase(j);
            __builtin_amdgcn_sched_barrier(0);
            __builtin_amdgcn_s_barrier();
            __builtin_amdgcn_sched_barrier(0);
            mma_phase();
            __builtin_amdgcn_sched_barrier(0);
            if (!(grp == 1 && j == NQ - 1)) __builtin_amdgcn_s_barrier();
            __builtin_amdgcn_sched_barrier(0);
            advance();
        }
        const int e_slab = cur_slab, e_m0 = m0, e_n0 = n0, e_phase = phase;
        const int w_next = w_cur + w_step;
        bool more = false;
        if constexpr (PERSIST) {
            more = w_next < w_cnt;
            if (more) {
                setup_item(w_next);
                prologue();
            }
        }

        const int rpb = p.Hout * p.Wout;
        const int row_base = e_m0 + grp * 128 + wm * (32 * MI), col_base = e_n0 + wn * (32 * NI);
        if constexpr (OUT == 1) {
            igemm_epilogue<MI, NI>(p, acc, row_base, col_base, lrow, lk, UP2 ? (long long)e_phase * p.M * p.ldc : 0LL, q.Nb, rpb);
        } else {
            float* pp = q.part + ((long long)e_slab * (MI * NI * 4) * 512 + tid) * 4;
#pragma unroll
            for (int i = 0; i < MI; ++i)
#pragma unroll
                for (int jn = 0; jn < NI; ++jn)
#pragma unroll
                    for (int qd = 0; qd < 4; ++qd) {
                        const f32x4 v = {acc[i][jn][4 * qd], acc[i][jn][4 * qd + 1], acc[i][jn][4 * qd + 2], acc[i][jn][4 * qd + 3]};
                        *reinterpret_cast<f32x4*>(pp + (long long)((i * NI + jn) * 4 + qd) * 512 * 4) = v;
                    }
        }
        if (!more) break;
        w_cur = w_next;
    }
    wait_vmcnt<0>();
}

struct PPGeom {
    int T, KW, rowstep, colstep, padflat, NLp, npa;
};
PPGeom pp_geom(const IGemm& p) {
    PPGeom g;
    g.T = p.KH * p.KW;
    g.KW = p.KW;
    g.rowstep = p.dh * p.Win;
    g.colstep = p.dw;
    g.padflat = p.ph * p.Win + p.pw;
    g.NLp = (BM + (p.KH - 1) * g.rowstep + (p.KW - 1) * g.colstep + 15) / 16 * 16;
    const int need = (g.NLp / 8 + 8 * (g.T - 1) - 1) / (8 * (g.T - 1));
    g.npa = need <= 1 ? 1 : need <= 3 ? 3 : 0;
    return g;
}
int pp_ring_lines(const PPGeom& g, int bn) {
    const int room = (163840 - 1152 - NSB * bn * 128) / 128 / 16 * 16;
    if (room >= 2 * g.NLp) return 2 * g.NLp;
    int X = 0;
    for (int pa = 0; pa < g.NLp / 8; ++pa) {
        const int t = pa / (8 * g.npa);
        if (t >= g.T - 1) return 0;
        const int need = 8 * pa + 8 - ((t / g.KW) * g.rowstep + (t % g.KW) * g.colstep);
        if (need > X) X = need;
    }
    const int cap = g.NLp + (X + 15) / 16 * 16;
    return cap <= room ? cap : 0;
}

template <int MI, int NI, int GWM, int GWN, int NPA, int TERMS>
void launch_npa_terms(const Ctx& ctx, const IGemm& p, const PPArgs& q, int items, size_t lds) {
    auto go = [&](auto kern) {
        ensure_dynamic_lds(reinterpret_cast<const void*>(kern), ctx.device, 163840);
        hipLaunchKernelGGL(kern, dim3((unsigned)items), dim3(512), lds, ctx.stream, p, q);
    };
    const bool persist = q.items > items, slab = q.part != nullptr;
    if (persist && slab) go(igemm_pp_kernel<MI, NI, GWM, GWN, NPA, true, 2, TERMS>);
    else if (persist) go(igemm_pp_kernel<MI, NI, GWM, GWN, NPA, true, 1, TERMS>);
    else if (slab) go(igemm_pp_kernel<MI, NI, GWM, GWN, NPA, false, 2, TERMS>);
    else go(igemm_pp_kernel<MI, NI, GWM, GWN, NPA, false, 1, TERMS>);
}

template <int MI, int NI, int GWM, int GWN, int NPA>
void launch_npa(const Ctx& ctx, const IGemm& p, const PPArgs& q, int items, size_t lds) {
    if (ctx.dtype == 2)
        launch_npa_terms<MI, NI, GWM, GWN, NPA, 1>(ctx, p, q, items, lds);
    else
        launch_npa_terms<MI, NI, GWM, GWN, NPA, 3>(ctx, p, q, items, lds);
}

template <int MI, int NI, int GWM, int GWN>
void launch_one(const Ctx& ctx, const IGemm& p, const IGemmPlan& pl, float* part) {
    const int Nb = pl.Nb;
    constexpr int BN = GWN * NI * 32;
    const int ncols = p.N;
    const int mtiles = (p.M + BM - 1) / BM, ntiles = (ncols + BN - 1) / BN;
    const PPGeom g = pp_geom(p);
    PPArgs q;
    q.W = p.Win;
    q.H = p.Hin;
    q.T = g.T;
    q.KW = g.KW;
    q.rowstep = g.rowstep;
    q.colstep = g.colstep;
    q.dh = p.dh;
    q.dw = p.dw;
    q.ph = p.ph;
    q.pw = p.pw;
    q.padflat = g.padflat;
    q.NLp = g.NLp;
    q.CAPl = pp_ring_lines(g, BN);
    q.ntiles = ntiles;
    q.tiles = mtiles * ntiles;
    q.nci = p.C1 / BK;
    q.cps = (q.nci + pl.S - 1) / pl.S;
    q.Nb = Nb;
    q.part = pl.S > 1 ? part : nullptr;
    q.S = pl.S;
    q.tile_major = ctx.tune.pp_tile_major && pl.S > 1 ? 1 : 0;
    q.tiles_pp = q.tiles;
    q.b_phase = 0;
    MAA_CHECK((q.nci + q.cps - 1) / q.cps == pl.S, "igemm_pp: K split leaves an empty slice");
    MAA_CHECK(q.CAPl > 0, "igemm_pp: the A ring does not fit beside the weight ring");
    const size_t lds = (size_t)q.CAPl * 128 + (size_t)NSB * BN * 128 + 128 + 1024;
    MAA_CHECK(lds <= 163840, "igemm_pp: LDS per workgroup");
    q.items = q.tiles * pl.S;
    const int cus = device_cu_count(ctx.device);
    const int grid = q.items < cus ? q.items : cus;
    if (g.npa == 1)
        launch_npa<MI, NI, GWM, GWN, 1>(ctx, p, q, grid, lds);
    else
        launch_npa<MI, NI, GWM, GWN, 3>(ctx, p, q, grid, lds);
    if (pl.S > 1) launch_splitk_reduce(ctx, p, part, pl.S, q.tiles, ntiles, Nb, BM, BN, GWN, MI, NI, 512);
}

template <int MI, int NI, int GWM, int GWN>
void launch_up2(const Ctx& ctx, const IGemm& p, int Nb, long long b_phase) {
    constexpr int BN = GWN * NI * 32;
    const int mtiles = (p.M + BM - 1) / BM, ntiles = (p.N + BN - 1) / BN;
    const PPGeom g = pp_geom(p);
    PPArgs q;
    q.W = p.Win;
    q.H = p.Hin;
    q.T = g.T;
    q.KW = g.KW;
    q.rowstep = g.rowstep;
    q.colstep = g.colstep;
    q.dh = p.dh;
    q.dw = p.dw;
    q.ph = 1;
    q.pw = 1;
    q.padflat = p.Win + 1;
    q.NLp = g.NLp;
    q.CAPl = pp_ring_lines(g, BN);
    q.ntiles = ntiles;
    q.tiles_pp = mtiles * ntiles;
    q.tiles = 4 * q.tiles_pp;
    q.nci = p.C1 / BK;
    q.cps = q.nci;
    q.Nb = Nb;
    q.part = nullptr;
    q.S = 1;
    q.tile_major = 0;
    q.b_phase = b_phase;
    MAA_CHECK(q.CAPl > 0, "igemm_pp up2: the A ring does not fit beside the weight ring");
    const size_t lds = (size_t)q.CAPl * 128 + (size_t)NSB * BN * 128 + 128 + 1024;
    MAA_CHECK(lds <= 163840, "igemm_pp up2: LDS per workgroup");
    q.items = q.tiles;
    const int cus = device_cu_count(ctx.device);
    const int grid = q.items < cus ? q.items : cus;
    auto go = [&](auto kern) {
        ensure_dynamic_lds(reinterpret_cast<const void*>(kern), ctx.device, 163840);
        hipLaunchKernelGGL(kern, dim3((unsigned)grid), dim3(512), lds, ctx.stream, p, q);
    };
    const bool one = ctx.dtype == 2;
// ... 319 lines not shown
```

### audiogpt_amd/csrc/maa_internal.h

```cpp
#pragma once
#include <hip/hip_runtime.h>

#include <cstdint>
#include <cstdio>
#include <map>
#include <stdexcept>
#include <string>
#include <vector>

namespace maa {

struct Error : std::runtime_error {
    using std::runtime_error::runtime_error;
};
void set_last_error(const std::string& s);

#define MAA_HIP(expr)                                                                              \
    do {                                                                                           \
        hipError_t _e = (expr);                                                                    \
        if (_e != hipSuccess)                                                                      \
            throw ::maa::Error(std::string(#expr) + ": " + hipGetErrorString(_e));                 \
    } while (0)
#define MAA_CHECK(cond, msg)                                                                       \
    do {                                                                                           \
        if (!(cond)) throw ::maa::Error(std::string("check failed: ") + #cond + " -- " + (msg));   \
    } while (0)

class Arena {
public:
    ~Arena();
    void reserve(size_t bytes);
    void reset() { off_ = 0; run_high_ = 0; }
    size_t mark() const { return off_; }
    void release(size_t m) { off_ = m; }
    float* alloc_f(size_t n_floats);
    size_t capacity() const { return cap_; }
    const void* base() const { return base_; }
    size_t high_water() const { return high_; }
    size_t mark_high() const { return run_high_; }
    bool dry = false;

private:
    char* base_ = nullptr;
    size_t cap_ = 0, off_ = 0, high_ = 0, run_high_ = 0;
};

struct ProfRow {
    std::string name;
    long long launches = 0;
    double ms = 0.0, flops = 0.0, bytes = 0.0;
};
class Profiler {
public:
    ~Profiler();
    struct Pending {
        std::string name;
        double flops, bytes;
        hipEvent_t e0, e1;
    };
    hipEvent_t get_event();
    std::vector<Pending> pending;
    std::vector<hipEvent_t> pool;
    size_t next = 0;
    int detail = 0;
    std::vector<ProfRow> collect(hipStream_t stream);
};
struct Ctx;
struct ProfScope {
    ProfScope(const Ctx& ctx, const char* name, double flops, double bytes);
    ~ProfScope();
    const Ctx* ctx_ = nullptr;
    size_t idx_ = 0;
};

void ensure_dynamic_lds(const void* kernel, int device, int bytes);
int device_cu_count(int device);

struct DevSlab {
    void* p = nullptr;
    size_t cap = 0;
    ~DevSlab();
    void* get(size_t bytes, hipStream_t stream);
    DevSlab() = default;
    DevSlab(const DevSlab&) = delete;
    DevSlab& operator=(const DevSlab&) = delete;
};

struct StepGraph {
    std::vector<unsigned long long> key;
    hipGraph_t graph = nullptr;
    hipGraphExec_t exec = nullptr;
    void clear();
    ~StepGraph() { clear(); }
    StepGraph() = default;
    StepGraph(const StepGraph&) = delete;
    StepGraph& operator=(const StepGraph&) = delete;
};

struct Tuning {
    std::string dma2;
    std::string pp, pp1;
    int pp_s_narrow = 2, pp_s_wide = 4;
    bool up2 = true;
    bool pp_tile_major = false;
    bool op_presplit = false;
    bool no_dma = false;
    int halo = 2;
    bool cfg_shared = true;
    bool gn_two_pass = false;
    void load();
};

struct Ctx {
    Ctx() = default;
    Ctx(const Ctx&) = delete;
    Ctx& operator=(const Ctx&) = delete;
    ~Ctx();
    Ctx* side = nullptr;
    hipEvent_t ev_fork = nullptr, ev_join = nullptr;
    int concurrency = -1;
    bool kept_full() const { return concurrency >= 3; }
    int cfg_split = -1;
    bool split_cfg() const { return cfg_split < 0 ? !kept_full() : cfg_split != 0; }
    Tuning tune;
    StepGraph ddim_graph;
    DevSlab sampler_scratch;
    DevSlab encode_scratch;
    StepGraph plms_graph;
    DevSlab plms_ring;
    StepGraph ddpm_graph;
    DevSlab ddpm_tab;
    DevSlab ddpm_scratch;
    DevSlab split_scratch;
    Profiler* prof = nullptr;
    float* zeros = nullptr;
    int device = 0;
    hipStream_t stream = nullptr;
    mutable Arena ws;
    int dtype = 0;
};

Ctx& side_lane(Ctx& ctx);

struct IGemm {
    const float* a1 = nullptr;
    const float* a2 = nullptr;
    int lda1 = 0, lda2 = 0;
    int C1 = 0, C2 = 0;
    int Hin = 1, Win = 1, Hout = 1, Wout = 1;
    int KH = 1, KW = 1, sh = 1, sw = 1, ph = 0, pw = 0, dh = 1, dw = 1;
    int up = 0;
    int a_split = 0;
    int a_act = 0;
    float a_slope = 0.f;
    const float* b = nullptr;
    int ldb = 0;
    int b_nk = 0;
    int b_split = 0;
    int M = 0, N = 0, K = 0;
    int Z = 1, zin = 1;
    long long a_so = 0, a_si = 0, b_so = 0, b_si = 0, c_so = 0, c_si = 0;
    float alpha = 1.f;
    const float* bias = nullptr;
    const float* rowadd = nullptr;
    int ld_rowadd = 0;
    const float* res = nullptr;
    int ldr = 0;
    int geglu = 0;
    int act = 0;
    float act_slope = 0.f;
    float out_scale = 1.f;
    int accumulate = 0;
    int c_split = 0;
    float* c = nullptr;
    int ldc = 0;
    float* c2 = nullptr;
    int ldc2 = 0;
    float c2_slope = 1.f;
    const float* zeros = nullptr;
};
struct IGemmPlan {
    enum Engine { F32, BF16_REG, DMA, DMA2, PP, PP1 } engine = F32;
    int cfg = 0;
    int bn = 0;
    int S = 1;
    int Nb = 0;
    bool fast = false;
    size_t slab_floats = 0;
};
IGemmPlan igemm_plan(const Ctx& ctx, const IGemm& p);
void launch_igemm(const Ctx& ctx, const IGemm& p);
int choose_tile(long long M, long long N, int Z, bool bf16, int mode = 0);
int fit_slices(int nchunks, int S);
void launch_igemm_f32(const Ctx& ctx, const IGemm& p, const IGemmPlan& pl);
void launch_igemm_bf16_reg(const Ctx& ctx, const IGemm& p, const IGemmPlan& pl);
bool igemm_dma_takes(const Ctx& ctx, const IGemm& p, IGemmPlan& pl);
void launch_igemm_dma(const Ctx& ctx, const IGemm& p, const IGemmPlan& pl);
bool igemm_dma2_takes(const Ctx& ctx, const IGemm& p, IGemmPlan& pl);
void launch_igemm_dma2(const Ctx& ctx, const IGemm& p, const IGemmPlan& pl, float* part);
bool igemm_pp_takes(const Ctx& ctx, const IGemm& p, IGemmPlan& pl);
void launch_igemm_pp(const Ctx& ctx, const IGemm& p, const IGemmPlan& pl, float* part);
bool igemm_pp1_takes(const Ctx& ctx, const IGemm& p, IGemmPlan& pl);
void launch_igemm_pp1(const Ctx& ctx, const IGemm& p, const IGemmPlan& pl, float* part);
void launch_splitk_reduce(const Ctx& ctx, const IGemm& p, const float* part, int S, int tiles, int ntiles, int Nb, int BM,
                          int BN, int WGN, int MI, int NI, int NTH);

void launch_groupnorm(Ctx& ctx, const float* x1, int ld1, int C1, const float* x2, int ld2, int C2, int B, int HW,
                      int groups, const float* gamma, const float* beta, float eps, int silu, float* out,
                      int out_split = 0, float* raw_split = nullptr);
void launch_layernorm(const Ctx& ctx, const float* x, long long rows, int C, const float* gamma, const float* beta,
                      float eps, float* out, int out_split = 0);
bool launch_igemm_pp_up2(const Ctx& ctx, const IGemm& p, int Nb, long long b_phase);
bool launch_narrow_conv3x3(const Ctx& ctx, const float* a_split, int lda, int B, int H, int W, int C, const float* w4, const float* bias,
                           int N, float* out_nchw);
void launch_pixel_shuffle2(const Ctx& ctx, const float* planes, int B, int H, int W, int C, float* out);
void launch_split32_pack(const Ctx& ctx, const float* x, long long rows, int C, float* out, float slope = 1.f);
void launch_split32_unpack(const Ctx& ctx, const float* x, long long rows, int C, float* out);
bool launch_flash_attention(const Ctx& ctx, const float* q, int ldq, int hsq, const float* k, int ldk, int hsk,
                            const float* v, int ldv, int hsv, int B, int heads, int dh, int Nq, int Nk, float alpha,
                            float* out, int ldo, int out_split = 0, int causal = 0);
bool flash_attention_covers(const Ctx& ctx, int dh);
void launch_softmax(const Ctx& ctx, float* s, long long rows, int cols, int ld, int causal_nq = 0);

void launch_timestep_embedding(const Ctx& ctx, const float* t, int B, int dim, float* out);
void launch_silu(const Ctx& ctx, const float* x, long long n, float* out);
void launch_add(const Ctx& ctx, const float* a, const float* b, long long n, float* out);
void launch_nchw_to_nhwc(const Ctx& ctx, const float* x, int B, int C, int HW, float* out);
void launch_nhwc_to_nchw(const Ctx& ctx, const float* x, int B, int C, int HW, float* out, int ld_in);
void launch_avgpool2(const Ctx& ctx, const float* x, int B, int H, int W, int C, float* out);
void launch_upsample2(const Ctx& ctx, const float* x, int B, int H, int W, int C, float* out);
void launch_dup_half(const Ctx& ctx, const float* x, long long n, float* out);
void split_check(int H, int W, int kh, int kw, int sh, int sw);
int split_crops(int H, int W, int kh, int kw, int sh, int sw);
void launch_split_unfold(const Ctx& ctx, const float* x, int nB, int C, int H, int W, int kh, int kw, int sh, int sw, float* out);
void launch_split_norm(const Ctx& ctx, const float* wT, int H, int W, int kh, int kw, int sh, int sw, float* norm);
void launch_split_fold(const Ctx& ctx, const float* e, const float* wT, const float* norm, int nB, int C, int H, int W, int kh,
                       int kw, int sh, int sw, float* out);
void launch_repeat_rows(const Ctx& ctx, const float* src, long long rows, long long len, int rep, float* dst);
void launch_scale(const Ctx& ctx, const float* x, long long n, float s, float* out);
void launch_ddim_update(const Ctx& ctx, const float* x, const float* eps_u, const float* eps_c, float scale,
                        const float* coef, long long n, float* x_prev, float* pred_x0, int* step = nullptr);
void launch_ddim_prepare(const Ctx& ctx, const float* x, const float* concat, int B, int nB, long long per,
                         long long per_c, const float* tab_t, const float* tab_coef, const int* step, float* xin,
                         float* cur_t, float* cur_coef, const float* mask = nullptr, const float* x0 = nullptr,
                         const float* noise_q = nullptr, int S = 0, const float* emb_tab = nullptr, int emb_w = 0,
                         float* cur_emb = nullptr, int n_t = 0);
void launch_ddim_step(const Ctx& ctx, const float* xin, long long per, long long per_in, const float* eps_u, const float* eps_c,
                      float scale, const float* coef, long long n, float* x_prev, const float* noise_p, float temperature, int S,
                      float* log_x, float* log_x0, int* step);
void launch_ldm_plms_step(const Ctx& ctx, const float* xin, long long per, long long per_in, const float* eps_u, const float* eps_c,
                          float scale, const float* coef, long long n, float* x_prev, float* ring, int S, float* log_x, float* log_x0,
                          int* step);
void launch_ldm_plms_euler_mid(const Ctx& ctx, float* xin, long long per, long long per_in, int B, int nB, const float* eps_u,
                               const float* eps_c, float scale, const float* coef, float* x_save, float* e_keep, const float* tab_t,
                               float* cur_t, const float* emb_tab, int emb_w, float* cur_emb, int n_t = 0);
void launch_ldm_plms_euler_final(const Ctx& ctx, const float* eps_u, const float* eps_c, float scale, const float* coef, long long n,
                                 float* x, const float* e_keep, float* log_x, float* log_x0, int* step);
constexpr int DDPM_TAB_W = 9;
void launch_ddpm_step(const Ctx& ctx, const float* xin, long long per, long long per_in, const float* eps_u, const float* eps_c,
                      float scale, const float* coef, const float* tab, long long n, float* x_prev, const float* noise_p, int start,
                      bool clip, const float* mask, const float* x0, const float* noise_q, float* log_x, float* log_x0, int* step);
void launch_ddpm_update(const Ctx& ctx, const float* x, const float* eps, const int* t, const float* tab, int n_tab, const float* noise,
                        float temperature, bool clip, int B, long long per, float* x_prev, float* x_recon, int* bad);
void launch_ddim_stochastic_encode(const Ctx& ctx, const float* x0, const float* moments, float scale_factor, const float* n_post,
                                   const int* t, const float* tab, int n_tab, const float* noise, int B, long long per, float* out,
                                   int* bad);
void launch_snake_aa(const Ctx& ctx, const float* x, int B, int L, int C, const float* inv_beta, const float* alpha,
                     float* out);
void launch_nsf_source(const Ctx& ctx, const float* f0, int B, int T, int hop, float sampling_rate, const float* rand_ini,
                       const float* noise, int harmonics, const float* w, const float* bias, float* sines, float* har);
void launch_similarity(const Ctx& ctx, const float* audio, const float* text, int Na, int Nt, int D, float scale, float* out);
void launch_leaky(const Ctx& ctx, const float* x, long long n, float slope, float* out);
void launch_clamp_affine(const Ctx& ctx, const float* x, long long n, float mul, float add, float lo, float hi,
                         float* out);
void launch_spec_from_mel(const Ctx& ctx, const float* mel, long long n, float* spec);

double calib_run(const Ctx& ctx, int kind);

struct HostTensor {
    const float* data = nullptr;
    std::vector<long long> shape;
    long long numel() const {
        long long n = 1;
        for (auto s : shape) n *= s;
        return n;
    }
};
using StateDict = std::map<std::string, HostTensor>;

struct PackedW {
    int phase_rows = 0;
    float* w = nullptr;
    float* bias = nullptr;
    int K = 0, N = 0, Npad = 0;
    int ld = 0, nk = 0;
    int split = 0;
};

bool launch_halo_conv1d(const Ctx& ctx, const float* x, int B, int L, int C, const PackedW& w, int k, int dil, float slope,
                        const float* res, float out_scale, int accumulate, float* out);
bool launch_halo_pair(const Ctx& ctx, const float* x, int B, int L, int C, const PackedW& w1, int k1, int d1, float slope1,
                      const PackedW& w2, int k2, int d2, float slope2, const float* res, float out_scale, int accumulate,
                      float* out);

class WeightStore {
public:
    explicit WeightStore(bool nk_layout = false) : nk_(nk_layout) {}
    ~WeightStore();
    void finish(PackedW& pw, const std::vector<float>& kn, bool bf16_ok = false);
    PackedW pack_conv_up2(const StateDict& sd, const std::string& wname, const std::string& bname);
    PackedW pack_narrow3x3(const StateDict& sd, const std::string& wname, const std::string& bname);
    void* upload_raw(const void* host, size_t bytes);
    float* upload(const std::vector<float>& host);
    PackedW pack_conv(const StateDict& sd, const std::string& wname, const std::string& bname, int KH, int KW);
    PackedW pack_concat(const StateDict& sd, const std::vector<std::string>& wnames,
                        const std::vector<std::string>& bnames);
    PackedW pack_geglu(const StateDict& sd, const std::string& wname, const std::string& bname);
    PackedW pack_convtr_phase(const StateDict& sd, const std::string& wname, const std::string& bname, int stride,
                              int pad, int carry, int* r_start, int* r_count);
    float* vec(const StateDict& sd, const std::string& name);
    size_t bytes() const { return bytes_; }

private:
    std::vector<void*> bufs_;
    size_t bytes_ = 0;
    bool nk_ = false;
};

const HostTensor& get(const StateDict& sd, const std::string& name);
bool has(const StateDict& sd, const std::string& name);

}
```

### audiogpt_amd/csrc/runtime.cpp

```cpp
#include "maa_internal.h"

#include <mutex>

#include <cstdlib>
#include <cstring>

extern char** environ;

namespace maa {

static thread_local std::string g_last_error;
void set_last_error(const std::string& s) { g_last_error = s; }
const char* last_error_cstr() { return g_last_error.c_str(); }

Arena::~Arena() {
    if (base_) (void)hipFree(base_);
}
void Arena::reserve(size_t bytes) {
    if (bytes <= cap_) return;
    if (base_) MAA_HIP(hipFree(base_));
    base_ = nullptr;
    cap_ = 0;
    MAA_HIP(hipMalloc(reinterpret_cast<void**>(&base_), bytes));
    cap_ = bytes;
}
float* Arena::alloc_f(size_t n_floats) {
    const size_t bytes = (n_floats * sizeof(float) + 255) / 256 * 256;
    const size_t at = off_;
    off_ += bytes;
    if (off_ > high_) high_ = off_;
    if (off_ > run_high_) run_high_ = off_;
    if (dry) return reinterpret_cast<float*>(static_cast<uintptr_t>(0x1000) + at);
    if (off_ > cap_) throw Error("workspace arena exhausted (" + std::to_string(off_) + " > " + std::to_string(cap_) + ")");
    return reinterpret_cast<float*>(base_ + at);
}

DevSlab::~DevSlab() {
    if (p) (void)hipFree(p);
}
void* DevSlab::get(size_t bytes, hipStream_t stream) {
    if (bytes > cap) {
        if (p) {
            MAA_HIP(hipStreamSynchronize(stream));
            MAA_HIP(hipFree(p));
            p = nullptr;
            cap = 0;
        }
        const size_t want = bytes + bytes / 4;
        MAA_HIP(hipMalloc(&p, want));
        cap = want;
    }
    return p;
}

Profiler::~Profiler() {
    for (hipEvent_t e : pool) (void)hipEventDestroy(e);
}
hipEvent_t Profiler::get_event() {
    if (next == pool.size()) {
        hipEvent_t e;
        MAA_HIP(hipEventCreate(&e));
        pool.push_back(e);
    }
    return pool[next++];
}
std::vector<ProfRow> Profiler::collect(hipStream_t stream) {
    MAA_HIP(hipStreamSynchronize(stream));
    std::map<std::string, ProfRow> agg;
    for (auto& p : pending) {
        float ms = 0.f;
        MAA_HIP(hipEventElapsedTime(&ms, p.e0, p.e1));
        ProfRow& r = agg[p.name];
        r.name = p.name;
        r.launches += 1;
        r.ms += ms;
        r.flops += p.flops;
        r.bytes += p.bytes;
    }
    pending.clear();
    next = 0;
    std::vector<ProfRow> out;
    for (auto& kv : agg) out.push_back(kv.second);
    return out;
}
ProfScope::ProfScope(const Ctx& ctx, const char* name, double flops, double bytes) {
    if (!ctx.prof || ctx.ws.dry) return;
    hipStreamCaptureStatus st = hipStreamCaptureStatusNone;
    if (hipStreamIsCapturing(ctx.stream, &st) != hipSuccess || st != hipStreamCaptureStatusNone) return;
    ctx_ = &ctx;
    Profiler::Pending p;
    p.name = name;
    p.flops = flops;
    p.bytes = bytes;
    p.e0 = ctx.prof->get_event();
    p.e1 = ctx.prof->get_event();
    (void)hipEventRecord(p.e0, ctx.stream);
    idx_ = ctx.prof->pending.size();
    ctx.prof->pending.push_back(p);
}
ProfScope::~ProfScope() {
    if (ctx_) (void)hipEventRecord(ctx_->prof->pending[idx_].e1, ctx_->stream);
}

const HostTensor& get(const StateDict& sd, const std::string& name) {
    auto it = sd.find(name);
    if (it == sd.end()) throw Error("missing weight tensor: " + name);
    return it->second;
}
bool has(const StateDict& sd, const std::string& name) { return sd.find(name) != sd.end(); }

void Tuning::load() {
#ifdef MAA_NO_TUNING
    return;
#endif
    auto get_s = [](const char* name) {
        const char* e = std::getenv(name);
        return std::string(e ? e : "");
    };
    dma2 = get_s("MAA_DMA2");
    pp = get_s("MAA_PP");
    pp1 = get_s("MAA_PP1");
    pp_s_narrow = 2;
    pp_s_wide = 4;
    const std::string pss = get_s("MAA_PP_S");
    if (!pss.empty()) std::sscanf(pss.c_str(), "%d,%d", &pp_s_narrow, &pp_s_wide);
    if (pp_s_narrow < 1) pp_s_narrow = 1;
    if (pp_s_wide < 1) pp_s_wide = 1;
    pp_tile_major = get_s("MAA_PP_TILE_MAJOR") == "1";
    up2 = get_s("MAA_UP2") != "0";
    cfg_shared = get_s("MAA_CFG_SHARED") != "0";
    const std::string ps = get_s("MAA_OP_PRESPLIT");
    op_presplit = !ps.empty() && ps[0] == '1';
    no_dma = !get_s("MAA_NO_DMA").empty();
    const std::string hs = get_s("MAA_HALO");
    halo = hs == "off" ? 0 : hs == "single" ? 1 : 2;
    gn_two_pass = get_s("MAA_GN_TWO_PASS") == "1";
    if (!dma2.empty() && dma2 != "off") {
        int cfg = 0, ns = 4, pipe = 1, S = 1, kmin = 0, kmax = 0;
        const int k = std::sscanf(dma2.c_str(), "%d,%d,%d,%d,%d,%d", &cfg, &ns, &pipe, &S, &kmin, &kmax);
        if (k < 4 || cfg != 0 || ns != 4 || pipe != 1 || S < 1) {
            const std::string bad = dma2;
            dma2.clear();
            throw Error("MAA_DMA2=\"" + bad + "\": expected \"off\" or \"0,4,1,S[,kmin[,kmax]]\" (the split-K engine keeps one "
                        "instantiation: tile 0, 4 stages, pipelined; S = K slices)");
        }
    }
}

Ctx::~Ctx() {
    if (side) {
        (void)hipStreamSynchronize(side->stream);
        (void)hipStreamDestroy(side->stream);
        side->stream = nullptr;
        delete side->prof;
        side->prof = nullptr;
        delete side;
    }
    if (ev_fork) (void)hipEventDestroy(ev_fork);
    if (ev_join) (void)hipEventDestroy(ev_join);
}
Ctx& side_lane(Ctx& ctx) {
    if (!ctx.side) {
        hipStream_t s = nullptr;
        MAA_HIP(hipStreamCreateWithFlags(&s, hipStreamNonBlocking));
        Ctx* sd = new Ctx;
        sd->stream = s;
        sd->device = ctx.device;
        sd->zeros = ctx.zeros;
        ctx.side = sd;
        MAA_HIP(hipEventCreateWithFlags(&ctx.ev_fork, hipEventDisableTiming));
        MAA_HIP(hipEventCreateWithFlags(&ctx.ev_join, hipEventDisableTiming));
    }
    ctx.side->tune = ctx.tune;
    ctx.side->dtype = ctx.dtype;
    ctx.side->concurrency = ctx.kept_full() ? 3 : 1;
    return *ctx.side;
}

void StepGraph::clear() {
    if (exec) (void)hipGraphExecDestroy(exec);
    if (graph) (void)hipGraphDestroy(graph);
    exec = nullptr;
    graph = nullptr;
    key.clear();
}

namespace {
std::mutex g_launch_mu;
std::map<std::pair<const void*, int>, int> g_lds_attr;
std::map<int, int> g_cus;
}

void ensure_dynamic_lds(const void* kernel, int device, int bytes) {
    std::lock_guard<std::mutex> lk(g_launch_mu);
    int& have = g_lds_attr[{kernel, device}];
    if (have >= bytes) return;
    MAA_HIP(hipFuncSetAttribute(kernel, hipFuncAttributeMaxDynamicSharedMemorySize, bytes));
    have = bytes;
}

int device_cu_count(int device) {
    std::lock_guard<std::mutex> lk(g_launch_mu);
    int& c = g_cus[device];
    if (!c) {
        hipDeviceProp_t prop;
        MAA_HIP(hipGetDeviceProperties(&prop, device));
        c = prop.multiProcessorCount;
    }
    return c;
}

WeightStore::~WeightStore() {
    for (void* p : bufs_) (void)hipFree(p);
}
float* WeightStore::upload(const std::vector<float>& host) {
    void* d = nullptr;
    const size_t bytes = host.size() * sizeof(float);
    MAA_HIP(hipMalloc(&d, bytes ? bytes : 4));
    if (bytes) MAA_HIP(hipMemcpy(d, host.data(), bytes, hipMemcpyHostToDevice));
    bufs_.push_back(d);
    bytes_ += bytes;
    return static_cast<float*>(d);
}
float* WeightStore::vec(const StateDict& sd, const std::string& name) {
    const HostTensor& t = get(sd, name);
    return upload(std::vector<float>(t.data, t.data + t.numel()));
}

static int pad32(int n) { return (n + 31) / 32 * 32; }

static inline unsigned short f2bf(float f) {
    unsigned u;
    std::memcpy(&u, &f, 4);
    u += 0x7fffu + ((u >> 16) & 1u);
    return (unsigned short)(u >> 16);
}
static inline float bf2f(unsigned short h) {
    const unsigned u = (unsigned)h << 16;
    float f;
    std::memcpy(&f, &u, 4);
    return f;
}
void* WeightStore::upload_raw(const void* host, size_t bytes) {
    void* d = nullptr;
    MAA_HIP(hipMalloc(&d, bytes ? bytes : 4));
    if (bytes) MAA_HIP(hipMemcpy(d, host, bytes, hipMemcpyHostToDevice));
    bufs_.push_back(d);
    bytes_ += bytes;
    return d;
}

void WeightStore::finish(PackedW& pw, const std::vector<float>& kn, bool bf16_ok) {
    if (nk_ && bf16_ok) {
        MAA_CHECK(pw.K % 32 == 0, "split32 weights need K % 32 == 0");
        const int ldk = pw.K;
        std::vector<unsigned short> t((size_t)pw.Npad * ldk * 2, 0);
        for (int k = 0; k < pw.K; ++k)
            for (int n = 0; n < pw.Npad; ++n) {
                const float w = kn[(size_t)k * pw.Npad + n];
                const unsigned short hi = f2bf(w);
                const size_t at = (size_t)n * ldk * 2 + (size_t)(k >> 5) * 64 + (k & 31);
                t[at] = hi;
                t[at + 32] = f2bf(w - bf2f(hi));
            }
        pw.w = static_cast<float*>(upload_raw(t.data(), t.size() * sizeof(unsigned short)));
        pw.ld = ldk;
        pw.nk = 1;
        pw.split = 1;
        return;
    }
    if (!nk_) {
        pw.w = upload(kn);
        pw.ld = pw.Npad;
        pw.nk = 0;
        return;
    }
    const int Kp = (pw.K + 3) / 4 * 4;
    std::vector<float> t((size_t)pw.Npad * Kp, 0.f);
    for (int k = 0; k < pw.K; ++k)
        for (int n = 0; n < pw.Npad; ++n) t[(size_t)n * Kp + k] = kn[(size_t)k * pw.Npad + n];
    pw.w = upload(t);
    pw.ld = Kp;
    pw.nk = 1;
}

PackedW WeightStore::pack_conv(const StateDict& sd, const std::string& wname, const std::string& bname, int KH,
                               int KW) {
    const HostTensor& w = get(sd, wname);
    MAA_CHECK(w.shape.size() >= 2, wname);
    const int Cout = (int)w.shape[0], Cin = (int)w.shape[1];
    MAA_CHECK(w.numel() == (long long)Cout * Cin * KH * KW, "conv weight shape " + wname);
    PackedW pw;
    pw.K = KH * KW * Cin;
    pw.N = Cout;
    pw.Npad = pad32(Cout);
    std::vector<float> h((size_t)pw.K * pw.Npad, 0.f);
    for (int co = 0; co < Cout; ++co)
        for (int ci = 0; ci < Cin; ++ci)
            for (int t = 0; t < KH * KW; ++t)
                h[((size_t)t * Cin + ci) * pw.Npad + co] = w.data[((size_t)co * Cin + ci) * KH * KW + t];
    finish(pw, h, Cin % 32 == 0);
    if (!bname.empty()) {
        const HostTensor& b = get(sd, bname);
        std::vector<float> hb(pw.Npad, 0.f);
        std::memcpy(hb.data(), b.data, sizeof(float) * Cout);
        pw.bias = upload(hb);
    }
    return pw;
}

PackedW WeightStore::pack_conv_up2(const StateDict& sd, const std::string& wname, const std::string& bname) {
    PackedW pw;
    const HostTensor& w = get(sd, wname);
    const int Cout = (int)w.shape[0], Cin = (int)w.shape[1];
    if (!nk_ || Cin % 32 != 0 || w.numel() != (long long)Cout * Cin * 9) return pw;
    const int np = pad32(Cout);
    pw.K = 4 * Cin;
    pw.Npad = 4 * np;
    std::vector<float> h((size_t)pw.K * pw.Npad, 0.f);
    for (int py = 0; py < 2; ++py)
        for (int px = 0; px < 2; ++px) {
            const int phase = py * 2 + px;
            for (int ky = 0; ky < 3; ++ky)
                for (int kx = 0; kx < 3; ++kx) {
                    const int ty = py == 0 ? (ky == 0 ? 0 : 1) : (ky == 2 ? 1 : 0);
                    const int tx = px == 0 ? (kx == 0 ? 0 : 1) : (kx == 2 ? 1 : 0);
                    const int t = ty * 2 + tx;
                    for (int co = 0; co < Cout; ++co)
                        for (int ci = 0; ci < Cin; ++ci)
                            h[((size_t)t * Cin + ci) * pw.Npad + (size_t)phase * np + co] += w.data[((size_t)co * Cin + ci) * 9 + ky * 3 + kx];
                }
        }
    finish(pw, h, true);
    pw.N = Cout;
    pw.Npad = np;
    pw.phase_rows = np;
    if (!bname.empty()) {
        const HostTensor& b = get(sd, bname);
        std::vector<float> hb(np, 0.f);
        std::memcpy(hb.data(), b.data, sizeof(float) * Cout);
        pw.bias = upload(hb);
    }
    return pw;
}

PackedW WeightStore::pack_narrow3x3(const StateDict& sd, const std::string& wname, const std::string& bname) {
    PackedW pw;
    const HostTensor& w = get(sd, wname);
    const int Cout = (int)w.shape[0], Cin = (int)w.shape[1];
    if (Cout > 4 || Cin % 8 != 0 || w.numel() != (long long)Cout * Cin * 9 || bname.empty()) return pw;
    std::vector<float> h((size_t)9 * Cin * 4, 0.f), hb(4, 0.f);
    for (int t = 0; t < 9; ++t)
        for (int ci = 0; ci < Cin; ++ci)
            for (int co = 0; co < Cout; ++co)
                h[(((size_t)t * 8 + (ci & 7)) * (Cin / 8) + (ci >> 3)) * 4 + co] = w.data[((size_t)co * Cin + ci) * 9 + t];
    const HostTensor& b = get(sd, bname);
    std::memcpy(hb.data(), b.data, sizeof(float) * Cout);
    pw.w = upload(h);
    pw.bias = upload(hb);
    pw.K = 9 * Cin;
    pw.N = Cout;
    pw.Npad = 4;
    return pw;
}

PackedW WeightStore::pack_concat(const StateDict& sd, const std::vector<std::string>& wnames,
                                 const std::vector<std::string>& bnames) {
    int N = 0, Cin = -1;
    for (auto& n : wnames) {
        const HostTensor& w = get(sd, n);
        const int cin = (int)(w.numel() / w.shape[0]);
        MAA_CHECK(Cin < 0 || Cin == cin, "pack_concat: input width mismatch " + n);
        Cin = cin;
        N += (int)w.shape[0];
    }
    PackedW pw;
    pw.K = Cin;
    pw.N = N;
    pw.Npad = pad32(N);
    std::vector<float> h((size_t)Cin * pw.Npad, 0.f), hb(pw.Npad, 0.f);
    int col = 0;
    for (size_t i = 0; i < wnames.size(); ++i) {
        const HostTensor& w = get(sd, wnames[i]);
        const int co_n = (int)w.shape[0];
        for (int co = 0; co < co_n; ++co)
            for (int ci = 0; ci < Cin; ++ci) h[(size_t)ci * pw.Npad + col + co] = w.data[(size_t)co * Cin + ci];
        if (!bnames.empty() && !bnames[i].empty()) {
            const HostTensor& b = get(sd, bnames[i]);
            std::memcpy(hb.data() + col, b.data, sizeof(float) * co_n);
        }
        col += co_n;
    }
    finish(pw, h, Cin % 32 == 0);
    bool any_bias = false;
    for (auto& b : bnames) any_bias = any_bias || !b.empty();
    if (any_bias) pw.bias = upload(hb);
    return pw;
}

PackedW WeightStore::pack_geglu(const StateDict& sd, const std::string& wname, const std::string& bname) {
    const HostTensor& w = get(sd, wname);
    const HostTensor& b = get(sd, bname);
    const int N2 = (int)w.shape[0], Cin = (int)w.shape[1], inner = N2 / 2;
    MAA_CHECK(inner % 32 == 0, "geglu inner width must be a multiple of 32");
    PackedW pw;
    pw.K = Cin;
    pw.N = inner;
    pw.Npad = N2;
    std::vector<float> h((size_t)Cin * N2), hb(N2);
    for (int j = 0; j < inner; ++j) {
        const int g = j / 32, jj = j % 32;
        const int cv = g * 64 + jj, cg = g * 64 + 32 + jj;
        for (int ci = 0; ci < Cin; ++ci) {
            h[(size_t)ci * N2 + cv] = w.data[(size_t)j * Cin + ci];
            h[(size_t)ci * N2 + cg] = w.data[(size_t)(inner + j) * Cin + ci];
        }
        hb[cv] = b.data[j];
        hb[cg] = b.data[inner + j];
    }
    finish(pw, h, Cin % 32 == 0);
    pw.bias = upload(hb);
    return pw;
}

PackedW WeightStore::pack_convtr_phase(const StateDict& sd, const std::string& wname, const std::string& bname,
                                       int stride, int pad, int carry, int* r_start, int* r_count) {
    const HostTensor& w = get(sd, wname);
    const int Cin = (int)w.shape[0], Cout = (int)w.shape[1], k = (int)w.shape[2];
    MAA_CHECK(k % stride == 0, "conv-transpose kernel must be a multiple of the stride");
    const int U = k / stride;
    std::vector<int> rs;
    for (int r = 0; r < stride; ++r)
        if ((r + pad) / stride == carry) rs.push_back(r);
    MAA_CHECK(!rs.empty(), "empty polyphase group");
    *r_start = rs.front();
    *r_count = (int)rs.size();
    MAA_CHECK(rs.back() - rs.front() + 1 == (int)rs.size(), "polyphase group not contiguous");
    PackedW pw;
    pw.K = U * Cin;
    pw.N = (int)rs.size() * Cout;
    pw.Npad = pad32(pw.N);
    std::vector<float> h((size_t)pw.K * pw.Npad, 0.f), hb(pw.Npad, 0.f);
    const HostTensor& b = get(sd, bname);
    for (size_t ri = 0; ri < rs.size(); ++ri) {
        const int phi = (rs[ri] + pad) % stride;
        for (int kx = 0; kx < U; ++kx) {
            const int u = U - 1 - kx;
            for (int ci = 0; ci < Cin; ++ci)
                for (int co = 0; co < Cout; ++co)
                    h[((size_t)kx * Cin + ci) * pw.Npad + ri * Cout + co] =
                        w.data[((size_t)ci * Cout + co) * k + phi + stride * u];
        }
        for (int co = 0; co < Cout; ++co) hb[ri * Cout + co] = b.data[co];
    }
    finish(pw, h, Cin % 32 == 0);
    pw.bias = upload(hb);
    return pw;
}

}
```

### audiogpt_amd/csrc/unet.cpp

```cpp
#include "models.h"

#include <atomic>
#include <cmath>
#include <cstdlib>

namespace maa {

namespace {

struct ResW {
    int cin = 0, cout = 0, updown = 0;
    float *g1 = nullptr, *b1 = nullptr, *g2 = nullptr, *b2 = nullptr;
    PackedW conv1, conv2, skip;
    bool has_skip = false;
    int emb_off = 0;
};
struct STBlockW {
    float *ln1g, *ln1b, *ln2g, *ln2b, *ln3g, *ln3b;
    PackedW qkv1, out1, q2, kv2, out2, ff1, ff2;
    int kv_slot = -1;
};
struct STW {
    int ch = 0, heads = 0, dh = 0;
    float *ng = nullptr, *nb = nullptr;
    PackedW proj_in, proj_out;
    std::vector<STBlockW> blocks;
};
struct AttnW {
    int ch = 0, heads = 0;
    float *ng = nullptr, *nb = nullptr;
    PackedW qkv, proj;
};
struct ConvW {
    PackedW w, w_up2;
    int cin = 0, cout = 0;
};
enum Kind { kConv, kRes, kST, kAttn, kDown, kUp };
struct Layer {
    Kind kind;
    int idx;
};

}

struct UNet::Impl {
    maa_unet_config cfg;
    int precision = 0;
    WeightStore ws;
    explicit Impl(int prec) : precision(prec), ws(prec != 0) {}
    std::vector<ResW> res;
    std::vector<STW> st;
    std::vector<AttnW> attn;
    std::vector<ConvW> convs;
    std::vector<std::vector<Layer>> input, output;
    std::vector<Layer> middle;
    PackedW te0, te2, emb_all, out_conv, out_narrow;
    float *out_g = nullptr, *out_b = nullptr;
    int emb_dim = 0, emb_total = 0;
    unsigned long long serial = next_serial();
    static unsigned long long next_serial() {
        static std::atomic<unsigned long long> n{1};
        return n.fetch_add(1);
    }
    std::vector<float*> kv_cache;
    std::vector<int> kv_inner;
    int kv_rows = 0, kv_len = 0, kv_batch = 0;
    size_t kv_cap_rows = 0;
    DevSlab cfg_context;
    DevSlab tiled_context;
    struct Prefix {
        const float *hs0 = nullptr, *xres = nullptr, *y1 = nullptr, *q = nullptr;
        int B = 0, H = 0, W = 0;
        hipEvent_t ready = nullptr;
    } prefix;
    int share = 0;

    bool prefix_ok() const {
        return cfg.use_spatial_transformer && !cfg.add_context_to_emb && input.size() >= 2 && input[0].size() == 1 &&
               input[0][0].kind == kConv && input[1].size() == 2 && input[1][0].kind == kRes && input[1][1].kind == kST &&
               !st[input[1][1].idx].blocks.empty();
    }

    ~Impl() {
        for (float* p : kv_cache)
            if (p) (void)hipFree(p);
        if (prefix.ready) (void)hipEventDestroy(prefix.ready);
    }

    Layer add_res(const StateDict& sd, const std::string& p, int cin, int cout, int updown) {
        ResW r;
        r.cin = cin;
        r.cout = cout;
        r.updown = updown;
        r.g1 = ws.vec(sd, p + "in_layers.0.weight");
        r.b1 = ws.vec(sd, p + "in_layers.0.bias");
        r.conv1 = ws.pack_conv(sd, p + "in_layers.2.weight", p + "in_layers.2.bias", 3, 3);
        r.g2 = ws.vec(sd, p + "out_layers.0.weight");
        r.b2 = ws.vec(sd, p + "out_layers.0.bias");
        r.conv2 = ws.pack_conv(sd, p + "out_layers.3.weight", p + "out_layers.3.bias", 3, 3);
        r.has_skip = has(sd, p + "skip_connection.weight");
        if (r.has_skip) r.skip = ws.pack_conv(sd, p + "skip_connection.weight", p + "skip_connection.bias", 1, 1);
        MAA_CHECK(r.has_skip == (cin != cout), "skip_connection presence " + p);
        r.emb_off = emb_total;
        emb_total += cout;
        emb_w.push_back(p + "emb_layers.1.weight");
        emb_b.push_back(p + "emb_layers.1.bias");
        res.push_back(r);
        return {kRes, (int)res.size() - 1};
    }
    Layer add_st(const StateDict& sd, const std::string& p, int ch, int heads, int dh) {
        STW s;
        s.ch = ch;
        s.heads = heads;
        s.dh = dh;
        const int inner = heads * dh;
        s.ng = ws.vec(sd, p + "norm.weight");
        s.nb = ws.vec(sd, p + "norm.bias");
        s.proj_in = ws.pack_conv(sd, p + "proj_in.weight", p + "proj_in.bias", 1, 1);
        s.proj_out = ws.pack_conv(sd, p + "proj_out.weight", p + "proj_out.bias", 1, 1);
        for (int d = 0; d < cfg.transformer_depth; ++d) {
            const std::string t = p + "transformer_blocks." + std::to_string(d) + ".";
            STBlockW b;
            b.ln1g = ws.vec(sd, t + "norm1.weight");
            b.ln1b = ws.vec(sd, t + "norm1.bias");
            b.ln2g = ws.vec(sd, t + "norm2.weight");
            b.ln2b = ws.vec(sd, t + "norm2.bias");
            b.ln3g = ws.vec(sd, t + "norm3.weight");
            b.ln3b = ws.vec(sd, t + "norm3.bias");
            b.qkv1 = ws.pack_concat(sd, {t + "attn1.to_q.weight", t + "attn1.to_k.weight", t + "attn1.to_v.weight"}, {});
            b.out1 = ws.pack_conv(sd, t + "attn1.to_out.0.weight", t + "attn1.to_out.0.bias", 1, 1);
            b.q2 = ws.pack_conv(sd, t + "attn2.to_q.weight", "", 1, 1);
            b.kv2 = ws.pack_concat(sd, {t + "attn2.to_k.weight", t + "attn2.to_v.weight"}, {});
            b.out2 = ws.pack_conv(sd, t + "attn2.to_out.0.weight", t + "attn2.to_out.0.bias", 1, 1);
            b.ff1 = ws.pack_geglu(sd, t + "ff.net.0.proj.weight", t + "ff.net.0.proj.bias");
            b.ff2 = ws.pack_conv(sd, t + "ff.net.2.weight", t + "ff.net.2.bias", 1, 1);
            b.kv_slot = (int)kv_cache.size();
            kv_cache.push_back(nullptr);
            kv_inner.push_back(inner);
            s.blocks.push_back(b);
        }
        st.push_back(s);
        return {kST, (int)st.size() - 1};
    }
    Layer add_attn(const StateDict& sd, const std::string& p, int ch, int heads) {
        AttnW a;
        a.ch = ch;
        a.heads = heads;
        a.ng = ws.vec(sd, p + "norm.weight");
        a.nb = ws.vec(sd, p + "norm.bias");
        a.qkv = ws.pack_conv(sd, p + "qkv.weight", p + "qkv.bias", 1, 1);
        a.proj = ws.pack_conv(sd, p + "proj_out.weight", p + "proj_out.bias", 1, 1);
        attn.push_back(a);
        return {kAttn, (int)attn.size() - 1};
    }
    Layer add_conv(const StateDict& sd, const std::string& p, int cin, int cout, Kind kind) {
        ConvW c;
        c.cin = cin;
        c.cout = cout;
        c.w = ws.pack_conv(sd, p + "weight", p + "bias", 3, 3);
        if (kind == kUp) c.w_up2 = ws.pack_conv_up2(sd, p + "weight", p + "bias");
        convs.push_back(c);
        return {kind, (int)convs.size() - 1};
    }
    std::vector<std::string> emb_w, emb_b;

    int cur_heads = 0;
    Layer attn_layer(const StateDict& sd, const std::string& p, int ch) {
        int heads, dh;
        if (cfg.num_head_channels == -1) {
            heads = cur_heads;
            dh = ch / heads;
        } else {
            heads = ch / cfg.num_head_channels;
            cur_heads = heads;
            dh = cfg.num_head_channels;
        }
        if (cfg.legacy) dh = cfg.use_spatial_transformer ? ch / heads : cfg.num_head_channels;
        if (cfg.use_spatial_transformer) return add_st(sd, p, ch, heads, dh);
        return add_attn(sd, p, ch, dh == -1 ? heads : ch / dh);
    }

    void build(const StateDict& sd) {
        const int mc = cfg.model_channels;
        emb_dim = mc * 4;
        cur_heads = cfg.num_heads;
        te0 = ws.pack_conv(sd, "time_embed.0.weight", "time_embed.0.bias", 1, 1);
        te2 = ws.pack_conv(sd, "time_embed.2.weight", "time_embed.2.bias", 1, 1);
        auto in_attn = [&](int ds) {
            for (int i = 0; i < cfg.n_attention_resolutions; ++i)
                if (cfg.attention_resolutions[i] == ds) return true;
            return false;
        };
        std::vector<int> chans;
        input.push_back({add_conv(sd, "input_blocks.0.0.", cfg.in_channels, mc, kConv)});
        chans.push_back(mc);
        int ch = mc, ds = 1;
        for (int level = 0; level < cfg.n_channel_mult; ++level) {
            const int m = cfg.channel_mult[level];
            for (int i = 0; i < cfg.num_res_blocks; ++i) {
                const std::string p = "input_blocks." + std::to_string(input.size()) + ".";
                std::vector<Layer> blk;
                blk.push_back(add_res(sd, p + "0.", ch, m * mc, 0));
                ch = m * mc;
                if (in_attn(ds)) blk.push_back(attn_layer(sd, p + "1.", ch));
                input.push_back(blk);
                chans.push_back(ch);
            }
            if (level != cfg.n_channel_mult - 1) {
                const std::string p = "input_blocks." + std::to_string(input.size()) + ".0.";
                if (cfg.resblock_updown)
                    input.push_back({add_res(sd, p, ch, ch, 1)});
                else
                    input.push_back({add_conv(sd, p + "op.", ch, ch, kDown)});
                chans.push_back(ch);
                ds *= 2;
            }
        }
        middle.push_back(add_res(sd, "middle_block.0.", ch, ch, 0));
        middle.push_back(attn_layer(sd, "middle_block.1.", ch));
        middle.push_back(add_res(sd, "middle_block.2.", ch, ch, 0));
        for (int level = cfg.n_channel_mult - 1; level >= 0; --level) {
            const int m = cfg.channel_mult[level];
            for (int i = 0; i < cfg.num_res_blocks + 1; ++i) {
                const int ich = chans.back();
                chans.pop_back();
                const std::string p = "output_blocks." + std::to_string(output.size()) + ".";
                std::vector<Layer> blk;
                blk.push_back(add_res(sd, p + "0.", ch + ich, mc * m, 0));
                ch = mc * m;
                int j = 1;
                if (in_attn(ds)) blk.push_back(attn_layer(sd, p + std::to_string(j++) + ".", ch));
                if (level && i == cfg.num_res_blocks) {
                    const std::string q = p + std::to_string(j++) + ".";
                    if (cfg.resblock_updown)
                        blk.push_back(add_res(sd, q, ch, ch, 2));
                    else
                        blk.push_back(add_conv(sd, q + "conv.", ch, ch, kUp));
                    ds /= 2;
                }
                output.push_back(blk);
            }
        }
        out_g = ws.vec(sd, "out.0.weight");
        out_b = ws.vec(sd, "out.0.bias");
        out_conv = ws.pack_conv(sd, "out.2.weight", "out.2.bias", 3, 3);
        out_narrow = ws.pack_narrow3x3(sd, "out.2.weight", "out.2.bias");
        emb_all = ws.pack_concat(sd, emb_w, emb_b);
        MAA_CHECK(emb_all.N == emb_total, "emb_layers packing");
    }

    T4 run_res(Ctx& ctx, const ResW& r, const T4& x1, const T4* x2, const float* emb_out) {
        const int B = x1.B, H = x1.H, W = x1.W;
        const int Ho = r.updown == 1 ? H / 2 : (r.updown == 2 ? H * 2 : H);
        const int Wo = r.updown == 1 ? W / 2 : (r.updown == 2 ? W * 2 : W);
        T4 out = alloc_t(ctx, B, Ho, Wo, r.cout);
        const size_t mk = ctx.ws.mark();
        T4 t1 = alloc_t(ctx, B, H, W, r.cin);
        t1.split = r.updown != 1 && split_for_gemm(ctx, r.cin);
        T4 xraw;
        if (r.has_skip && r.updown == 0 && split_for_gemm(ctx, r.cin) && r.skip.split) {
            xraw = alloc_t(ctx, B, H, W, r.cin);
            xraw.split = true;
        }
        launch_groupnorm(ctx, x1.p, x1.C, x1.C, x2 ? x2->p : nullptr, x2 ? x2->C : 0, x2 ? x2->C : 0, B, H * W, 32,
                         r.g1, r.b1, 1e-5f, 1, t1.p, t1.split, xraw.p);
        T4 h1 = alloc_t(ctx, B, Ho, Wo, r.cout);
        ConvOpt o1;
        o1.KH = o1.KW = 3;
        o1.pad = 1;
        o1.rowadd = emb_out + r.emb_off;
        o1.ld_rowadd = emb_ld;
        const float* resid = nullptr;
        if (r.updown == 1) {
            MAA_CHECK(!x2, "down ResBlock takes one source");
            T4 tp = alloc_t(ctx, B, Ho, Wo, r.cin), xp = alloc_t(ctx, B, Ho, Wo, r.cin);
            launch_avgpool2(ctx, t1.p, B, H, W, r.cin, tp.p);
            launch_avgpool2(ctx, x1.p, B, H, W, r.cin, xp.p);
            conv_into(ctx, tp, nullptr, r.conv1, o1, h1);
            resid = xp.p;
        } else if (r.updown == 2) {
            MAA_CHECK(!x2, "up ResBlock takes one source");
            T4 xu = alloc_t(ctx, B, Ho, Wo, r.cin);
            launch_upsample2(ctx, x1.p, B, H, W, r.cin, xu.p);
            o1.up = 1;
            conv_into(ctx, t1, nullptr, r.conv1, o1, h1);
            resid = xu.p;
        } else {
            conv_into(ctx, t1, nullptr, r.conv1, o1, h1);
            resid = x1.p;
        }
        T4 t2 = alloc_t(ctx, B, Ho, Wo, r.cout);
        t2.split = split_for_gemm(ctx, r.cout);
        launch_groupnorm(ctx, h1.p, r.cout, r.cout, nullptr, 0, 0, B, Ho * Wo, 32, r.g2, r.b2, 1e-5f, 1, t2.p, t2.split);
        if (r.has_skip) {
            MAA_CHECK(r.updown == 0, "skip conv with up/down");
            T4 sk = alloc_t(ctx, B, H, W, r.cout);
            ConvOpt os;
            if (xraw.p)
                conv_into(ctx, xraw, nullptr, r.skip, os, sk);
            else
                conv_into(ctx, x1, x2, r.skip, os, sk);
            resid = sk.p;
        } else {
            MAA_CHECK(!x2, "identity skip needs a single source");
        }
        ConvOpt o2;
        o2.KH = o2.KW = 3;
        o2.pad = 1;
        o2.res = resid;
        conv_into(ctx, t2, nullptr, r.conv2, o2, out);
        ctx.ws.release(mk);
        return out;
    }

    T4 run_st(Ctx& ctx, const STW& s, const T4& x, bool expand = false, int xp = 0) {
        const int HW = x.H * x.W, inner = s.heads * s.dh;
        int B = x.B;
        const int Bo = expand ? 2 * x.B : x.B;
        long long M = (long long)B * HW;
        const long long Mo = (long long)Bo * HW;
        T4 out = alloc_t(ctx, Bo, x.H, x.W, s.ch);
        float *y1_keep = nullptr, *q_keep = nullptr;
        if (xp == 2) {
            y1_keep = ctx.ws.alloc_f((size_t)M * inner);
            q_keep = ctx.ws.alloc_f((size_t)M * inner);
        }
        const size_t mk = ctx.ws.mark();
        const float* xres = x.p;
        if (expand) {
            float* xd = ctx.ws.alloc_f((size_t)Mo * s.ch);
            launch_dup_half(ctx, x.p, M * s.ch, xd);
            xres = xd;
        }
        const bool sp_in = split_for_gemm(ctx, s.ch), sp = split_for_gemm(ctx, inner);
        float* y = nullptr;
        if (xp != 3) {
            float* xn = ctx.ws.alloc_f((size_t)M * s.ch);
            launch_groupnorm(ctx, x.p, s.ch, s.ch, nullptr, 0, 0, B, HW, 32, s.ng, s.nb, 1e-6f, 0, xn, sp_in);
            y = ctx.ws.alloc_f((size_t)M * inner);
            linear_into(ctx, xn, s.ch, M, s.ch, s.proj_in, nullptr, 0, y, inner, 0, 0, sp_in ? M : 0);
        }
        const float scale = 1.0f / std::sqrt((float)s.dh);
        const bool no_osplit = false;
        const int o_sp = !no_osplit && sp && flash_attention_covers(ctx, s.dh) ? 1 : 0;
        const int g_sp = !no_osplit && split_for_gemm(ctx, 4 * inner) ? 1 : 0;
        int y_sp = 0;
        for (const STBlockW& b : s.blocks) {
            const bool first_block = &b == &s.blocks.front();
            float* ln = ctx.ws.alloc_f((size_t)Mo * inner);
            float* o = ctx.ws.alloc_f((size_t)Mo * inner);
            float *y1 = nullptr, *q = nullptr;
            if (xp == 3 && first_block) {
                y1 = const_cast<float*>(prefix.y1);
                q = const_cast<float*>(prefix.q);
            } else {
                launch_layernorm(ctx, y, M, inner, b.ln1g, b.ln1b, 1e-5f, ln, sp);
                float* qkv = ctx.ws.alloc_f((size_t)M * 3 * inner);
                linear_into(ctx, ln, inner, M, inner, b.qkv1, nullptr, 0, qkv, 3 * inner, 0, 0, sp ? M : 0);
                attention_into(ctx, qkv, 3 * inner, s.dh, qkv + inner, 3 * inner, s.dh, qkv + 2 * inner, 3 * inner, s.dh,
                               B, s.heads, s.dh, HW, HW, scale, o, inner, o_sp);
                y1 = xp == 2 && first_block ? y1_keep : ctx.ws.alloc_f((size_t)M * inner);
                linear_into(ctx, o, inner, M, inner, b.out1, y, inner, y1, inner, 0, 0, o_sp ? M : 0);
                launch_layernorm(ctx, y1, M, inner, b.ln2g, b.ln2b, 1e-5f, ln, sp);
                q = xp == 2 && first_block ? q_keep : ctx.ws.alloc_f((size_t)M * inner);
                linear_into(ctx, ln, inner, M, inner, b.q2, nullptr, 0, q, inner, 0, 0, sp ? M : 0);
                if (xp == 2 && first_block) {
                    prefix.y1 = y1;
                    prefix.q = q;
                    prefix.xres = x.p;
                    if (!ctx.ws.dry) MAA_HIP(hipEventRecord(prefix.ready, ctx.stream));
                }
            }
            if (B != Bo) {
                float* qd = ctx.ws.alloc_f((size_t)Mo * inner);
                float* yd = ctx.ws.alloc_f((size_t)Mo * inner);
                launch_dup_half(ctx, q, M * inner, qd);
                launch_dup_half(ctx, y1, M * inner, yd);
                q = qd;
                y1 = yd;
                B = Bo;
                M = Mo;
            }
            MAA_CHECK(ctx.ws.dry || (kv_cache[b.kv_slot] && (lane ? batch_off + B <= kv_batch : kv_batch == B)),
                      "set_context must precede forward (batch)");
            const float* kv = kv_cache[b.kv_slot] + (size_t)batch_off * kv_len * 2 * inner;
            attention_into(ctx, q, inner, s.dh, kv, 2 * inner, s.dh, kv + inner, 2 * inner, s.dh, B, s.heads, s.dh, HW,
                           kv_len, scale, o, inner, o_sp);
            float* y2 = ctx.ws.alloc_f((size_t)M * inner);
            linear_into(ctx, o, inner, M, inner, b.out2, y1, inner, y2, inner, 0, 0, o_sp ? M : 0);
            launch_layernorm(ctx, y2, M, inner, b.ln3g, b.ln3b, 1e-5f, ln, sp);
            float* g = ctx.ws.alloc_f((size_t)M * 4 * inner);
            linear_into(ctx, ln, inner, M, inner, b.ff1, nullptr, 0, g, 4 * inner, 1, 0, sp ? M : 0, g_sp);
            float* y3 = ctx.ws.alloc_f((size_t)M * inner);
            const bool last = &b == &s.blocks.back();
            y_sp = last && sp && !no_osplit ? 1 : 0;
            linear_into(ctx, g, 4 * inner, M, 4 * inner, b.ff2, y2, inner, y3, inner, 0, 0, g_sp ? M : 0, y_sp);
            y = y3;
        }
        MAA_CHECK(B == Bo, "SpatialTransformer without a transformer block cannot part the halves of a guided step");
        linear_into(ctx, y, inner, M, inner, s.proj_out, xres, s.ch, out.p, s.ch, 0, 0, y_sp ? M : 0);
        ctx.ws.release(mk);
        return out;
    }

    T4 run_attn(Ctx& ctx, const AttnW& a, const T4& x) {
        const int B = x.B, HW = x.H * x.W, C = a.ch, dh = C / a.heads;
        const long long M = (long long)B * HW;
        T4 out = alloc_t(ctx, B, x.H, x.W, C);
        const size_t mk = ctx.ws.mark();
        float* xn = ctx.ws.alloc_f((size_t)M * C);
        const bool sp = split_for_gemm(ctx, C);
        launch_groupnorm(ctx, x.p, C, C, nullptr, 0, 0, B, HW, 32, a.ng, a.nb, 1e-5f, 0, xn, sp);
        float* qkv = ctx.ws.alloc_f((size_t)M * 3 * C);
        linear_into(ctx, xn, C, M, C, a.qkv, nullptr, 0, qkv, 3 * C, 0, 0, sp ? M : 0);
        float* o = ctx.ws.alloc_f((size_t)M * C);
        const float sc = 1.0f / std::sqrt(std::sqrt((float)dh));
        attention_into(ctx, qkv, 3 * C, 3 * dh, qkv + dh, 3 * C, 3 * dh, qkv + 2 * dh, 3 * C, 3 * dh, B, a.heads, dh, HW,
                       HW, sc * sc, o, C);
        linear_into(ctx, o, C, M, C, a.proj, x.p, C, out.p, C);
        ctx.ws.release(mk);
        return out;
    }

    T4 run_layers(Ctx& ctx, const std::vector<Layer>& layers, T4 h, const T4* skip, const float* emb_out, bool* shared = nullptr) {
        bool first = true;
        for (const Layer& l : layers) {
            const T4* x2 = first ? skip : nullptr;
            switch (l.kind) {
                case kConv: {
                    T4 o = alloc_t(ctx, h.B, h.H, h.W, convs[l.idx].cout);
                    ConvOpt co;
                    co.KH = co.KW = 3;
                    co.pad = 1;
                    conv_into(ctx, h, nullptr, convs[l.idx].w, co, o);
                    h = o;
                    break;
                }
                case kRes:
                    h = run_res(ctx, res[l.idx], h, x2, emb_out);
                    break;
                case kST:
                    h = run_st(ctx, st[l.idx], h, shared && *shared, exporting ? 2 : 0);
                    exporting = false;
                    if (shared) *shared = false;
                    break;
                case kAttn:
                    h = run_attn(ctx, attn[l.idx], h);
                    break;
                case kDown: {
                    T4 o = alloc_t(ctx, h.B, (h.H + 2 - 3) / 2 + 1, (h.W + 2 - 3) / 2 + 1, convs[l.idx].cout);
                    ConvOpt co;
                    co.KH = co.KW = 3;
                    co.pad = 1;
                    co.stride = 2;
                    conv_into(ctx, h, nullptr, convs[l.idx].w, co, o);
                    h = o;
                    break;
                }
                case kUp: {
                    T4 o = alloc_t(ctx, h.B, h.H * 2, h.W * 2, convs[l.idx].cout);
                    if (!conv_up2_into(ctx, h, convs[l.idx].w_up2, o)) {
                        ConvOpt co;
                        co.KH = co.KW = 3;
                        co.pad = 1;
                        co.up = 1;
                        conv_into(ctx, h, nullptr, convs[l.idx].w, co, o);
                    }
                    h = o;
                    break;
                }
            }
            first = false;
        }
        return h;
    }

    void emb_rows(Ctx& ctx, const float* t, int rows, const float* add, float* out) {
        const int mc = cfg.model_channels;
        float* te = ctx.ws.alloc_f((size_t)rows * mc);
        launch_timestep_embedding(ctx, t, rows, mc, te);
        float* e1 = ctx.ws.alloc_f((size_t)rows * emb_dim);
        linear_into(ctx, te, mc, rows, mc, te0, nullptr, 0, e1, emb_dim);
        float* emb = ctx.ws.alloc_f((size_t)rows * emb_dim);
        launch_silu(ctx, e1, (long long)rows * emb_dim, e1);
        linear_into(ctx, e1, emb_dim, rows, emb_dim, te2, add, emb_dim, emb, emb_dim);
        float* semb = ctx.ws.alloc_f((size_t)rows * emb_dim);
        launch_silu(ctx, emb, (long long)rows * emb_dim, semb);
        linear_into(ctx, semb, emb_dim, rows, emb_dim, emb_all, nullptr, 0, out, emb_all.Npad);
    }
    bool exporting = false;
    int emb_ld = 0;
    int batch_off = 0;
    bool lane = false;

    void forward(Ctx& ctx, const float* x_nchw, const float* t, const float* context, int B, int H, int W,
                 float* out_nchw, const float* emb_row = nullptr, int share_req = 0) {
        if (context && batch_off) context += (size_t)batch_off * kv_len * cfg.context_dim;
        share = 0;
        exporting = false;
        if (emb_row) {
            emb_ld = 0;
            if (share_req == 1 && cfg.use_spatial_transformer && !lane && B % 2 == 0) share = 1;
            if ((share_req == 2 || share_req == 3) && lane && prefix_ok()) share = share_req;
            forward_body(ctx, x_nchw, B, H, W, out_nchw, emb_row);
            share = 0;
            return;
        }
        float* emb_out = ctx.ws.alloc_f((size_t)B * emb_all.Npad);
        emb_rows(ctx, t, B, cfg.add_context_to_emb ? context : nullptr, emb_out);
        emb_ld = emb_all.Npad;
        forward_body(ctx, x_nchw, B, H, W, out_nchw, emb_out);
    }

    void forward_body(Ctx& ctx, const float* x_nchw, int B, int H, int W, float* out_nchw, const float* emb_out) {
        if (share == 3) {
            forward_rest_of_lane(ctx, B, H, W, out_nchw, emb_out);
            return;
        }
        if (share == 2) {
            if (!prefix.ready) MAA_HIP(hipEventCreateWithFlags(&prefix.ready, hipEventDisableTiming));
            prefix.B = B;
            prefix.H = H;
            prefix.W = W;
            exporting = true;
        }
        bool shared = share == 1;
        auto both = [&](const T4& t) {
            T4 d = alloc_t(ctx, 2 * t.B, t.H, t.W, t.C);
            launch_dup_half(ctx, t.p, (long long)t.B * t.H * t.W * t.C, d.p);
            return d;
        };
        T4 h = alloc_t(ctx, shared ? B / 2 : B, H, W, cfg.in_channels);
        launch_nchw_to_nhwc(ctx, x_nchw, h.B, cfg.in_channels, H * W, h.p);
        std::vector<T4> hs;
        for (auto& blk : input) {
            h = run_layers(ctx, blk, h, nullptr, emb_out, &shared);
            hs.push_back(shared ? both(h) : h);
            if (share == 2 && hs.size() == 1) prefix.hs0 = h.p;
        }
        exporting = false;
        if (shared) {
            h = both(h);
            shared = false;
        }
        finish(ctx, h, hs, B, H, W, out_nchw, emb_out);
    }

    void forward_rest_of_lane(Ctx& ctx, int B, int H, int W, float* out_nchw, const float* emb_out) {
        MAA_CHECK(prefix.B == B && prefix.H == H && prefix.W == W && prefix.ready, "guided step: the lanes disagree on the shared prefix");
// ... 134 lines not shown
```

### include/maa.h

```cpp
#ifndef MAA_H_
#define MAA_H_

#include <stddef.h>
#include <stdint.h>

#ifdef __cplusplus
extern "C" {
#endif

typedef enum maa_status {
    MAA_OK = 0,
    MAA_ERR_INVALID = -1,
    MAA_ERR_HIP = -2,
    MAA_ERR_INTERNAL = -3
} maa_status;

typedef struct maa_ctx maa_ctx;
typedef struct maa_unet maa_unet;
typedef struct maa_vae maa_vae;
typedef struct maa_vocoder maa_vocoder;

const char* maa_last_error(void);
const char* maa_version(void);

// ... 79 lines not shown

int maa_ddim_stochastic_encode(maa_ctx* ctx, const float* d_x0_or_moments, int from_moments, float scale_factor,
                               const float* d_noise_post, const int32_t* d_t, const float* h_sqrt_a, const float* h_sqrt_1ma, int n_tab,
                               const float* d_noise, int B, int C, int H, int W, float* d_out);
int maa_ddim_decode(maa_ctx* ctx, maa_unet* u, const maa_ddim_args* args, int t_start, float* d_x);
int maa_ldm_plms_sample(maa_ctx* ctx, maa_unet* u, const maa_ddim_args* args, float* d_x);

typedef struct maa_ddpm_args {
    maa_ddim_args loop;
    int start, n;
    int clip_denoised;
    const float* h_sqrt_recip_ac;
    const float* h_sqrt_recipm1_ac;
    const float* h_coef1;
    const float* h_coef2;
    const float* h_logvar;
    const float* h_sqrt_ac;
    const float* h_sqrt_1mac;
    const float* h_temperature;
} maa_ddpm_args;
int maa_ddpm_sample(maa_ctx* ctx, maa_unet* u, const maa_ddpm_args* args, float* d_x);
int maa_ddpm_update(maa_ctx* ctx, const float* d_x, const float* d_eps, const int32_t* d_t, const float* h_sqrt_recip_ac,
                    const float* h_sqrt_recipm1_ac, const float* h_coef1, const float* h_coef2, const float* h_logvar, int n_tab,
                    const float* d_noise, float temperature, int clip_denoised, int B, int C, int H, int W, float* d_x_prev,
                    float* d_x_recon);

typedef struct maa_vae_config {
    int ch, out_ch, in_channels, z_channels, embed_dim, resolution, num_res_blocks, double_z;
    int n_ch_mult, ch_mult[8];
    int n_attn_resolutions, attn_resolutions[8];
} maa_vae_config;
int maa_vae_create(maa_ctx* ctx, const maa_vae_config* cfg, const maa_tensor* tensors, int n_tensors, maa_vae** out);
int maa_vae_destroy(maa_vae* v);
int maa_vae_decode(maa_ctx* ctx, maa_vae* v, const float* d_z, int B, int h, int w, float inv_scale, float* d_mel);
int maa_vae_decode_spec(maa_ctx* ctx, maa_vae* v, const float* d_z, int B, int h, int w, float inv_scale, float* d_spec);
int maa_vae_encode_moments(maa_ctx* ctx, maa_vae* v, const float* d_mel, int B, int H, int W, float* d_moments);

typedef struct maa_vocoder_config {
    int kind;
    int num_mels, upsample_initial_channel;
    int n_upsamples, upsample_rates[8], upsample_kernel_sizes[8];
    int n_kernels, resblock_kernel_sizes[8];
    int n_dilations, resblock_dilation_sizes[8][8];
    int snake_beta, snake_logscale;
    int use_pitch_embed, sampling_rate, harmonic_num;
    int resblock;
} maa_vocoder_config;
int maa_vocoder_create(maa_ctx* ctx, const maa_vocoder_config* cfg, const maa_tensor* tensors, int n_tensors,
                       maa_vocoder** out);
int maa_vocoder_destroy(maa_vocoder* v);
int maa_vocoder_forward(maa_ctx* ctx, maa_vocoder* v, const float* d_mel, int B, int T, float* d_wav);
int maa_vocoder_forward_f0(maa_ctx* ctx, maa_vocoder* v, const float* d_mel, const float* d_f0,
                           const float* d_rand_ini, const float* d_noise, int B, int T, float* d_wav);

typedef struct maa_diffnet_config {
    int in_dims, hidden_size, residual_layers, residual_channels, dilation_cycle_length;
} maa_diffnet_config;
typedef struct maa_diffnet maa_diffnet;
int maa_diffnet_create(maa_ctx* ctx, const maa_diffnet_config* cfg, const maa_tensor* tensors, int n_tensors,
                       maa_diffnet** out);
int maa_diffnet_destroy(maa_diffnet* d);
int maa_diffnet_forward(maa_ctx* ctx, maa_diffnet* d, const float* d_spec, const float* d_t, const float* d_cond, int B,
                        int T, float* d_eps);
typedef struct maa_plms_args {
    int B, T, K_step, interval, timesteps;
    const float* d_cond;
    const float* h_alphas_cumprod;
    int use_graph;
} maa_plms_args;
int maa_plms_sample(maa_ctx* ctx, maa_diffnet* d, const maa_plms_args* args, float* d_x);
typedef struct maa_ds_ddpm_args {
    int B, T, start, n, timesteps;
    int clip_denoised, use_graph;
    const float* d_cond;
    const float* d_noise;
    const float* h_sqrt_recip_ac;
    const float* h_sqrt_recipm1_ac;
    const float* h_coef1;
    const float* h_coef2;
    const float* h_sigma;
} maa_ds_ddpm_args;
int maa_ds_ddpm_sample(maa_ctx* ctx, maa_diffnet* d, const maa_ds_ddpm_args* args, float* d_x);
int maa_ds_ddpm_update(maa_ctx* ctx, const float* d_eps, const float* d_t, const float* d_noise, const float* h_sqrt_recip_ac,
                       const float* h_sqrt_recipm1_ac, const float* h_coef1, const float* h_coef2, const float* h_sigma,
                       int timesteps, int B, int M, int T, int clip_denoised, float* d_x);

typedef struct maa_pitch_extractor_config {
    int n_mel_bins, hidden_size, predictor_hidden, predictor_kernel, conv_layers;
    int ffn_padding_same;
    int use_uv;
    int pitch_norm;
    float f0_mean, f0_std;
} maa_pitch_extractor_config;
typedef struct maa_pitch_extractor maa_pitch_extractor;
int maa_pitch_extractor_create(maa_ctx* ctx, const maa_pitch_extractor_config* cfg, const maa_tensor* tensors, int n_tensors,
                               maa_pitch_extractor** out);
int maa_pitch_extractor_destroy(maa_pitch_extractor* pe);
int maa_pitch_extractor_forward(maa_ctx* ctx, maa_pitch_extractor* pe, const float* d_mel, int B, int T, float* d_pitch_pred,
                                float* d_f0, float* d_mel_hidden);

typedef struct maa_encoder_config {
    int kind;
    int layers, width, heads, mlp_dim, d_proj;
    int vocab, max_positions;
    int patch, image;
    float ln_eps;
} maa_encoder_config;
typedef struct maa_encoder maa_encoder;
int maa_encoder_create(maa_ctx* ctx, const maa_encoder_config* cfg, const maa_tensor* tensors, int n_tensors,
                       maa_encoder** out);
int maa_encoder_destroy(maa_encoder* e);
int maa_encoder_text(maa_ctx* ctx, maa_encoder* e, const int* d_ids, int B, int L, float* d_out);
int maa_encoder_image(maa_ctx* ctx, maa_encoder* e, const float* d_img, int B, float* d_out);

int maa_encoder_text_cls(maa_ctx* ctx, maa_encoder* e, const int* d_ids, int B, int L, float* d_out);

typedef struct maa_clap_audio_config {
    int mel_bins, n_blocks, channels[8];
    int out_emb, d_proj;
    float bn_eps;
} maa_clap_audio_config;
typedef struct maa_clap_audio maa_clap_audio;
int maa_clap_audio_create(maa_ctx* ctx, const maa_clap_audio_config* cfg, const maa_tensor* tensors, int n_tensors,
                          maa_clap_audio** out);
int maa_clap_audio_destroy(maa_clap_audio* a);
int maa_clap_audio_embed(maa_ctx* ctx, maa_clap_audio* a, const float* d_logmel, int B, int T, float* d_embedding,
                         float* d_z);
int maa_clap_similarity(maa_ctx* ctx, const float* d_audio, const float* d_text, int Na, int Nt, int D, float scale,
                        float* d_out);

typedef struct maa_spectral_config {
    int n_fft, hop, n_freq, n_mels;
    int pad_mode;
    int power;
    int log_kind;
    float amin, ref;
    int out_layout;
} maa_spectral_config;
typedef struct maa_spectral maa_spectral;
int maa_spectral_create(maa_ctx* ctx, const maa_spectral_config* cfg, const float* h_basis, const float* h_melw,
                        maa_spectral** out);
int maa_spectral_destroy(maa_spectral* s);
int maa_spectral_forward(maa_ctx* ctx, maa_spectral* s, const float* d_wav, int B, int n, float* d_out);

typedef struct maa_resampler maa_resampler;
int maa_resampler_create(maa_ctx* ctx, int orig, int neu, int width, int klen, const float* h_kernels, maa_resampler** out);
int maa_resampler_destroy(maa_resampler* r);
int maa_resampler_forward(maa_ctx* ctx, maa_resampler* r, const float* d_wav, int B, int n, float* d_out);

int maa_calib(maa_ctx* ctx, int kind, double* out_value);

int maa_op_linear(maa_ctx* ctx, const float* d_a, int M, int K, const float* h_w, const float* h_bias, int N,
                  int geglu, float* d_y, const float* d_res, int c_split);
int maa_op_conv(maa_ctx* ctx, const float* d_x, int B, int Cin, int H, int W, const float* h_w, const float* h_bias,
                int Cout, int KH, int KW, int stride, int pad, int dil, int upsample2, float leaky_slope,
                float* d_y, int Ho, int Wo, const float* d_rowadd, const float* d_res, int c_split);
int maa_op_groupnorm(maa_ctx* ctx, const float* d_x, int B, int C, int HW, const float* h_gamma,
                     const float* h_beta, float eps, int silu, float* d_y);
int maa_op_layernorm(maa_ctx* ctx, const float* d_x, int rows, int C, const float* h_gamma, const float* h_beta,
                     float eps, float* d_y);
int maa_op_attention(maa_ctx* ctx, const float* d_q, const float* d_k, const float* d_v, int B, int heads, int dh,
                     int Nq, int Nk, float alpha, float* d_y);
int maa_op_attention_ex(maa_ctx* ctx, const float* d_q, int ldq, int hsq, const float* d_k, int ldk, int hsk,
                        const float* d_v, int ldv, int hsv, int B, int heads, int dh, int Nq, int Nk, float alpha,
                        float* d_y, int ldo, int out_split, int causal);
int maa_op_groupnorm_ex(maa_ctx* ctx, const float* d_x1, int ld1, int C1, const float* d_x2, int ld2, int C2, int B, int HW,
                        int groups, const float* h_gamma, const float* h_beta, float eps, int silu, float* d_y, int out_split,
                        float* d_raw);
int maa_op_layernorm_ex(maa_ctx* ctx, const float* d_x, int rows, int C, const float* h_gamma, const float* h_beta, float eps,
                        float* d_y, int out_split);
int maa_op_split32(maa_ctx* ctx, const float* d_x, int rows, int C, float slope, int unpack, float* d_y);
int maa_op_conv_transpose1d(maa_ctx* ctx, const float* d_x, int B, int Cin, int L, const float* h_w,
                            const float* h_bias, int Cout, int k, int stride, float leaky_slope, float* d_y);
int maa_op_bench_conv(maa_ctx* ctx, int B, int H, int W, int Cin, int Cout, int taps, int pre_split, int iters,
                      float* ms_per_launch);
int maa_op_snake_aa(maa_ctx* ctx, const float* d_x, int B, int C, int L, const float* h_alpha, const float* h_beta,
                    int logscale, float* d_y);
int maa_op_mrf_pair(maa_ctx* ctx, const float* d_x, int B, int C, int L, const float* h_w1, const float* h_b1, int k1, int d1,
                    float slope1, const float* h_w2, const float* h_b2, int k2, int d2, float slope2, float out_scale,
                    int accumulate, float* d_out);
int maa_op_unfold(maa_ctx* ctx, const float* d_x, int B, int C, int H, int W, int kh, int kw, int sh, int sw, float* d_out);
int maa_op_fold(maa_ctx* ctx, const float* d_crops, const float* h_weight, int B, int C, int H, int W, int kh, int kw, int sh, int sw,
                float* d_out);

#ifdef __cplusplus
}
#endif
#endif
```

Before: 136.9 audio-seconds/sec.

## Fold transformer LayerNorms into adjacent GEMM epilogues of SpatialTransformer blocks

The producing linear (proj_in, out1, out2, ff2) now writes a split32 copy of its output plus per-32-column mean/M2 partial statistics in its epilogue. The consuming linear (qkv1, q2, ff1/GEGLU) uses weights pre-scaled by gamma, with a beta-derived bias and column sums. It finishes the per-row mean and rstd from those partials and applies the normalisation in its epilogue. This removes the three standalone LayerNorm kernels per transformer block and their extra activation read/write, at the cost of more epilogue work, an extra stats buffer, and a numerics change (Chan-style merged variance, folded weights). It is gated by a tuning flag ln_fold, and a test entry point maa_op_ln_linear is added.

```diff
diff --git a/audiogpt_amd/_lib.py b/audiogpt_amd/_lib.py
--- a/audiogpt_amd/_lib.py
+++ b/audiogpt_amd/_lib.py
@@ -126,7 +126,7 @@
     "maa_resampler_forward", "maa_op_linear", "maa_op_conv", "maa_op_groupnorm", "maa_op_layernorm",
     "maa_op_attention", "maa_op_attention_ex", "maa_op_conv_transpose1d", "maa_op_snake_aa", "maa_op_bench_conv", "maa_calib",
     "maa_op_mrf_pair", "maa_op_groupnorm_ex", "maa_op_layernorm_ex", "maa_op_split32",
-    "maa_unet_forward_split", "maa_op_unfold", "maa_op_fold",
+    "maa_unet_forward_split", "maa_op_unfold", "maa_op_fold", "maa_op_ln_linear",
 ]
 
 _lib = None
@@ -218,6 +218,7 @@
         "maa_unet_forward_split": [vp, vp, vp, vp, vp, ci, ci, ci, ci, ci, ci, ci, fp, vp],
         "maa_op_unfold": [vp, vp, ci, ci, ci, ci, ci, ci, ci, ci, vp],
         "maa_op_fold": [vp, vp, fp, ci, ci, ci, ci, ci, ci, ci, ci, vp],
+        "maa_op_ln_linear": [vp, vp, ci, ci, fp, fp, vp, ci, fp, fp, cf, fp, fp, ci, ci, ci, vp],
     }
     for name, argtypes in sig.items():
         fn = getattr(lib, name)
diff --git a/audiogpt_amd/backend.py b/audiogpt_amd/backend.py
--- a/audiogpt_amd/backend.py
+++ b/audiogpt_amd/backend.py
@@ -113,6 +113,19 @@
         assert r is None or tuple(r.shape) == tuple(y.shape)
         L.check(self.lib.maa_op_linear(self.h, L.dptr(a), M, K, wp, bp, N, int(geglu), L.dptr(y),
                                        L.dptr(r) if r is not None else None, int(split_out)))
+        return y
+
+    def op_ln_linear(self, a, w0, b0, gamma, beta, w1, b1=None, res=None, geglu=False, fold=True, eps=1e-5):
+        a = _f32(a, self.device)
+        M, K0 = a.shape
+        Cc, N = w0.shape[0], w1.shape[0]
+        keep = [L.host_f32(t) if t is not None else (None, None) for t in (w0, b0, gamma, beta, w1, b1)]
+        y = torch.empty(M, N // 2 if geglu else N, device=self.device)
+        r = _f32(res, self.device) if res is not None else None
+        assert r is None or tuple(r.shape) == (M, Cc)
+        L.check(self.lib.maa_op_ln_linear(self.h, L.dptr(a), M, K0, keep[0][1], keep[1][1], L.dptr(r) if r is not None else None,
+                                          Cc, keep[2][1], keep[3][1], float(eps), keep[4][1], keep[5][1], N, int(geglu),
+                                          int(fold), L.dptr(y)))
         return y
 
     def op_conv(self, x, w, b=None, stride=1, pad=0, dil=1, up=False, leaky=0.0, out_hw=None, rowadd=None, res=None,
diff --git a/audiogpt_amd/csrc/api.cpp b/audiogpt_amd/csrc/api.cpp
--- a/audiogpt_amd/csrc/api.cpp
+++ b/audiogpt_amd/csrc/api.cpp
@@ -697,6 +697,57 @@
                 a = sp;
             }
             maa::linear_into(c, a, K, M, K, pw, d_res, N, d_y, geglu ? N / 2 : N, geglu, 0, pre ? M : 0, c_split);
+        });
+        MAA_HIP(hipStreamSynchronize(c.stream));
+    });
+}
+
+int maa_op_ln_linear(maa_ctx* ctx, const float* d_a, int M, int K0, const float* h_w0, const float* h_b0, const float* d_res,
+                     int C, const float* h_gamma, const float* h_beta, float eps, const float* h_w1, const float* h_b1, int N,
+                     int geglu, int fold, float* d_y) {
+    return guarded([&] {
+        bind(ctx);
+        MAA_CHECK(d_a && h_w0 && h_gamma && h_beta && h_w1 && d_y, "bad op_ln_linear arguments");
+        MAA_CHECK(M > 0 && K0 > 0 && C > 0 && N > 0 && C % 32 == 0 && K0 % 32 == 0 && eps > 0.f, "bad op_ln_linear sizes");
+        MAA_CHECK(!geglu || (h_b1 && N % 64 == 0), "op_ln_linear: GEGLU needs a bias and value / gate halves of whole 32-column blocks");
+        maa::Ctx& c = ctx->c;
+        MAA_CHECK(c.dtype != 0, "op_ln_linear: the transformer path of the bf16 modes (split32 rows)");
+        OneShot s;
+        s.add("w0", h_w0, {C, K0});
+        if (h_b0) s.add("b0", h_b0, {C});
+        s.add("g", h_gamma, {C});
+        s.add("beta", h_beta, {C});
+        s.add("w1", h_w1, {N, C});
+        if (h_b1) s.add("b1", h_b1, {N});
+        maa::WeightStore ws(true);
+        const bool hi_only = c.dtype == 2;
+        maa::PackedW w0 = ws.pack_conv(s.sd, "w0", h_b0 ? "b0" : "", 1, 1);
+        maa::PackedW w1;
+        float *g = nullptr, *beta = nullptr;
+        if (fold) {
+            w1 = geglu ? ws.pack_geglu_ln(s.sd, "w1", "b1", "g", "beta", hi_only)
+                       : ws.pack_linear_ln(s.sd, {"w1"}, {h_b1 ? "b1" : ""}, "g", "beta", hi_only);
+            MAA_CHECK(w1.w && w1.ln_s, "op_ln_linear: folded weights");
+        } else {
+            w1 = geglu ? ws.pack_geglu(s.sd, "w1", "b1") : ws.pack_conv(s.sd, "w1", h_b1 ? "b1" : "", 1, 1);
+            g = ws.vec(s.sd, "g");
+            beta = ws.vec(s.sd, "beta");
+        }
+        maa::run_sized(c, [&] {
+            float* a = c.ws.alloc_f((size_t)M * K0);
+            if (!c.ws.dry) maa::launch_split32_pack(c, d_a, M, K0, a);
+            float* y = c.ws.alloc_f((size_t)M * C);
+            float* ln = c.ws.alloc_f((size_t)M * C);
+            maa::LnFold prod, cons;
+            if (fold) {
+                prod.sp = ln;
+                prod.part = c.ws.alloc_f((size_t)M * (C / 32) * 2);
+                cons.stats = prod.part;
+                cons.eps = eps;
+            }
+            maa::linear_into(c, a, K0, M, K0, w0, d_res, C, y, C, 0, 0, M, 0, 0, fold ? &prod : nullptr);
+            if (!fold && !c.ws.dry) maa::launch_layernorm(c, y, M, C, g, beta, eps, ln, 1);
+            maa::linear_into(c, ln, C, M, C, w1, nullptr, 0, d_y, geglu ? N / 2 : N, geglu, 0, M, 0, 0, fold ? &cons : nullptr);
         });
         MAA_HIP(hipStreamSynchronize(c.stream));
     });
diff --git a/audiogpt_amd/csrc/blocks.cpp b/audiogpt_amd/csrc/blocks.cpp
--- a/audiogpt_amd/csrc/blocks.cpp
+++ b/audiogpt_amd/csrc/blocks.cpp
@@ -136,7 +136,8 @@
 }
 
 void linear_into(Ctx& ctx, const float* a, int lda, long long rows, int K, const PackedW& w, const float* res,
-                 int ldr, float* out, int ldc, int geglu, int a_act, long long a_split_rows, int c_split, int act) {
+                 int ldr, float* out, int ldc, int geglu, int a_act, long long a_split_rows, int c_split, int act,
+                 const LnFold* ln) {
     IGemm p;
     p.a1 = a;
     p.lda1 = lda;
@@ -163,6 +164,19 @@
     p.act = act;
     p.c = out;
     p.ldc = ldc;
+    if (ln && ln->part) {
+        MAA_CHECK(ln->sp && !geglu, "LayerNorm-fold producer: split32 copy and statistics go together, not with GEGLU");
+        p.ln_sp = ln->sp;
+        p.ld_ln_sp = w.N;
+        p.ln_part = ln->part;
+    }
+    if (ln && ln->stats) {
+        MAA_CHECK(w.ln_s && a_split_rows > 0 && K % 32 == 0, "LayerNorm-fold consumer needs folded weights and split32 rows");
+        p.ln_stats = ln->stats;
+        p.ln_nblk = K / 32;
+        p.ln_s = w.ln_s;
+        p.ln_eps = ln->eps;
+    }
     launch_igemm(ctx, p);
 }
 
diff --git a/audiogpt_amd/csrc/blocks.h b/audiogpt_amd/csrc/blocks.h
--- a/audiogpt_amd/csrc/blocks.h
+++ b/audiogpt_amd/csrc/blocks.h
@@ -48,9 +48,15 @@
               float slope2, const float* res, float out_scale, int accumulate, T4& t1, T4& out);
 void check_convtr_polyphase(int k, int stride);
 bool conv_up2_into(Ctx& ctx, const T4& x, const PackedW& w4, T4& out);
+struct LnFold {
+    float* sp = nullptr;
+    float* part = nullptr;
+    const float* stats = nullptr;
+    float eps = 0.f;
+};
 void linear_into(Ctx& ctx, const float* a, int lda, long long rows, int K, const PackedW& w, const float* res,
                  int ldr, float* out, int ldc, int geglu = 0, int a_act = 0, long long a_split_rows = 0,
-                 int c_split = 0, int act = 0);
+                 int c_split = 0, int act = 0, const LnFold* ln = nullptr);
 
 void attention_into(Ctx& ctx, const float* q, int ldq, int hsq, const float* k, int ldk, int hsk, const float* v,
                     int ldv, int hsv, int B, int heads, int dh, int Nq, int Nk, float alpha, float* out, int ldo,
diff --git a/audiogpt_amd/csrc/igemm_dispatch.cpp b/audiogpt_amd/csrc/igemm_dispatch.cpp
--- a/audiogpt_amd/csrc/igemm_dispatch.cpp
+++ b/audiogpt_amd/csrc/igemm_dispatch.cpp
@@ -44,6 +44,12 @@
         return false;
     }
     MAA_CHECK(!(p.c_split || p.c2) || p.N % 32 == 0, "split32 outputs are whole 32-channel lines");
+    MAA_CHECK(!p.ln_part || (p.ln_sp && taps == 1 && p.N % 32 == 0 && p.ld_ln_sp % 32 == 0 && p.ld_ln_sp >= p.N && !p.geglu && p.Z == 1 && al16(p.ln_sp) &&
+                             (reinterpret_cast<uintptr_t>(p.ln_part) & 7) == 0),
+              "LayerNorm-fold producer: a linear's plain output of whole 32-column blocks, one batch entry (the convolution engine compiles the fold out)");
+    MAA_CHECK(!p.ln_stats || (p.ln_s && p.bias && p.a_split && taps == 1 && p.ln_nblk * 32 == p.K && p.Z == 1 &&
+                              (reinterpret_cast<uintptr_t>(p.ln_stats) & 7) == 0),
+              "LayerNorm-fold consumer: split32 rows of ln_nblk blocks, folded weights (ln_s, c)");
     const int ncols = p.N * (p.geglu ? 2 : 1);
     pl.fast = true;
     pl.Nb = ncols;
@@ -140,6 +146,7 @@
     if (ctx.ws.dry) return pl;
     MAA_CHECK(p.M > 0 && p.N > 0 && p.K > 0, "empty igemm");
     MAA_CHECK(!p.c_split, "split32 output asked of a problem only the fp32 engine can take");
+    MAA_CHECK(!p.ln_part && !p.ln_stats, "LayerNorm fold asked of a problem only the fp32 engine can take");
     const int taps = p.KH * p.KW, Ctot = p.C1 + p.C2;
     MAA_CHECK(p.K <= taps * Ctot && p.K > (taps - 1) * Ctot, "igemm K mismatch");
     MAA_CHECK(p.a_act == 0 || p.a_act == 1, "igemm A activation");
diff --git a/audiogpt_amd/csrc/igemm_epilogue.h b/audiogpt_amd/csrc/igemm_epilogue.h
--- a/audiogpt_amd/csrc/igemm_epilogue.h
+++ b/audiogpt_amd/csrc/igemm_epilogue.h
@@ -40,29 +40,130 @@
     *o = even ? (hb | (theirs << 16)) : (theirs | (lb << 16));
 }
 
-template <int MI, int NI, bool PAIR, bool RSEL>
+
+__device__ __forceinline__ void block_row_stats(const float (&v)[16], int lrow, float& sum, float& m2, int& r_mine) {
+    const bool b4 = (lrow & 16) != 0, b3 = (lrow & 8) != 0, b2 = (lrow & 4) != 0, b1 = (lrow & 2) != 0;
+    float s8[8], q8[8], s4[4], q4[4], s2[2], q2[2];
+#pragma unroll
+    for (int t = 0; t < 8; ++t) {
+        const float keep = b4 ? v[8 + t] : v[t], give = b4 ? v[t] : v[8 + t];
+        const float got = __shfl_xor(give, 16, 64);
+        const float d = keep - got;
+        s8[t] = keep + got;
+        q8[t] = (d * d) * 0.5f;
+    }
+#pragma unroll
+    for (int t = 0; t < 4; ++t) {
+        const float ks = b3 ? s8[4 + t] : s8[t], gs = b3 ? s8[t] : s8[4 + t];
+        const float kq = b3 ? q8[4 + t] : q8[t], gq = b3 ? q8[t] : q8[4 + t];
+        const float os = __shfl_xor(gs, 8, 64), oq = __shfl_xor(gq, 8, 64);
+        const float d = ks - os;
+        s4[t] = ks + os;
+        q4[t] = fmaf(d * d, 0.25f, kq + oq);
+    }
+#pragma unroll
+    for (int t = 0; t < 2; ++t) {
+        const float ks = b2 ? s4[2 + t] : s4[t], gs = b2 ? s4[t] : s4[2 + t];
+        const float kq = b2 ? q4[2 + t] : q4[t], gq = b2 ? q4[t] : q4[2 + t];
+        const float os = __shfl_xor(gs, 4, 64), oq = __shfl_xor(gq, 4, 64);
+        const float d = ks - os;
+        s2[t] = ks + os;
+        q2[t] = fmaf(d * d, 0.125f, kq + oq);
+    }
+    {
+        const float ks = b1 ? s2[1] : s2[0], gs = b1 ? s2[0] : s2[1];
+        const float kq = b1 ? q2[1] : q2[0], gq = b1 ? q2[0] : q2[1];
+        const float os = __shfl_xor(gs, 2, 64), oq = __shfl_xor(gq, 2, 64);
+        const float d = ks - os;
+        sum = ks + os;
+        m2 = fmaf(d * d, 0.0625f, kq + oq);
+    }
+    {
+        const float os = __shfl_xor(sum, 1, 64), oq = __shfl_xor(m2, 1, 64);
+        const float d = sum - os;
+        sum = sum + os;
+        m2 = fmaf(d * d, 0.03125f, m2 + oq);
+    }
+    r_mine = (b4 ? 8 : 0) + (b3 ? 4 : 0) + (b2 ? 2 : 0) + (b1 ? 1 : 0);
+}
+
+template <int MI>
+__device__ __forceinline__ void ln_rows_finish(const IGemm& p, int m_base, int lrow, int lk, float (&mu_l)[(MI + 1) / 2],
+                                               float (&rs_l)[(MI + 1) / 2]) {
+    constexpr int NB = 10;
+    const int nblk = p.ln_nblk;
+#pragma unroll
+    for (int ps = 0; ps < (MI + 1) / 2; ++ps) {
+        const int m = m_base + (2 * ps + lk) * 32 + lrow;
+        const f32x2* st = reinterpret_cast<const f32x2*>(p.ln_stats) + (long long)(m < p.M ? m : p.M - 1) * nblk;
+        float mean = 0.f, M2 = 0.f;
+        for (int b0 = 0; b0 < nblk; b0 += NB) {
+            float vs[NB], vq[NB];
+#pragma unroll
+            for (int u = 0; u < NB; ++u) {
+                const f32x2 t = st[b0 + u < nblk ? b0 + u : nblk - 1];
+                vs[u] = t[0];
+                vq[u] = t[1];
+            }
+#pragma unroll
+            for (int u = 0; u < NB; ++u) {
+                settle(vs[u]);
+                settle(vq[u]);
+            }
+#pragma unroll
+            for (int u = 0; u < NB; ++u) {
+                const int b = b0 + u;
+                if (b < nblk) {
+                    const float inv = 1.0f / (float)(b + 1);
+                    const float d = vs[u] * 0.03125f - mean;
+                    mean = fmaf(d, inv, mean);
+                    M2 = fmaf(d * d, (32.0f * (float)b) * inv, M2 + vq[u]);
+                }
+            }
+        }
+        mu_l[ps] = mean;
+        rs_l[ps] = 1.0f / sqrtf(M2 / (32.0f * (float)nblk) + p.ln_eps);
+    }
+}
+
+template <int MI, int NI, bool PAIR, bool RSEL, bool LNF>
 __device__ __forceinline__ void igemm_epilogue_impl(const IGemm& p, f32x16 (&acc)[MI][NI], int m_base, int n_base,
                                                     int lrow, int lk, long long coff, int Nb, int rpb) {
     float* cp = p.c + coff;
     const float* resp = p.res ? p.res + coff : nullptr;
+    float mu_l[(MI + 1) / 2], rs_l[(MI + 1) / 2];
+    const bool lnc = LNF && p.ln_stats != nullptr, lnp = LNF && p.ln_part != nullptr;
+    if (lnc) ln_rows_finish<MI>(p, m_base, lrow, lk, mu_l, rs_l);
     if (p.geglu) {
         if constexpr (NI % 2 == 0) {
-#pragma unroll
-            for (int i = 0; i < MI; ++i)
-#pragma unroll
-                for (int j = 0; j < NI; j += 2) {
+            static_for<0, MI>([&](auto ic) {
+                constexpr int i = decltype(ic)::value;
+                static_for<0, NI / 2>([&](auto jc) {
+                    constexpr int j = 2 * decltype(jc)::value;
                     const int cpk = n_base + j * 32 + lrow;
                     const int ncol = (cpk >> 6) * 32 + lrow;
                     if (cpk + 32 < Nb && ncol < p.N) {
                         float bv = p.bias ? p.bias[cpk] : 0.f;
                         float bg = p.bias ? p.bias[cpk + 32] : 0.f;
+                        float sv = lnc ? p.ln_s[cpk] : 0.f;
+                        float sg = lnc ? p.ln_s[cpk + 32] : 0.f;
                         settle(bv);
                         settle(bg);
+                        settle(sv);
+                        settle(sg);
                         float outv[16];
 #pragma unroll
                         for (int r = 0; r < 16; ++r) {
-                            const float val = acc[i][j][r] * p.alpha + bv;
-                            const float g = acc[i][j + 1][r] * p.alpha + bg;
+                            float val, g;
+                            if (lnc) {
+                                const int from = 32 * (i & 1) + (r & 3) + 8 * (r >> 2) + 4 * lk;
+                                const float mu = __shfl(mu_l[i >> 1], from, 64), rsd = __shfl(rs_l[i >> 1], from, 64);
+                                val = fmaf(rsd, fmaf(-mu, sv, acc[i][j][r] * p.alpha), bv);
+                                g = fmaf(rsd, fmaf(-mu, sg, acc[i][j + 1][r] * p.alpha), bg);
+                            } else {
+                                val = acc[i][j][r] * p.alpha + bv;
+                                g = acc[i][j + 1][r] * p.alpha + bg;
+                            }
                             const float gl = 0.5f * g * (1.f + fast_erff(g * 0.70710678118654752440f));
                             outv[r] = val * gl;
                         }
@@ -77,20 +178,22 @@
                             }
                         }
                     }
-                }
+                });
+            });
         }
         return;
     }
-#pragma unroll
-    for (int i = 0; i < MI; ++i) {
+    static_for<0, MI>([&](auto ic) {
+        constexpr int i = decltype(ic)::value;
         const int mb = m_base + i * 32;
         const int b0 = (mb < p.M ? mb : p.M - 1) / rpb;
         const int nextb = (b0 + 1) * rpb;
-#pragma unroll
-        for (int j = 0; j < NI; ++j) {
+        static_for<0, NI>([&](auto jc) {
+            constexpr int j = decltype(jc)::value;
             const int n = n_base + j * 32 + lrow;
             if (n < p.N) {
                 float bias = p.bias ? p.bias[n] : 0.f;
+                float lns = lnc ? p.ln_s[n] : 0.f;
                 float ra[16], rs[16], cv[16];
                 long long mc[16];
 #pragma unroll
@@ -118,6 +221,7 @@
                     for (int r = 0; r < 16; ++r) cv[r] = cp[mc[r] * p.ldc + n];
                 }
                 settle(bias);
+                settle(lns);
 #pragma unroll
                 for (int r = 0; r < 16; ++r) {
                     settle(ra[r]);
@@ -127,7 +231,14 @@
                 float outv[16];
 #pragma unroll
                 for (int r = 0; r < 16; ++r) {
-                    float v = acc[i][j][r] * p.alpha + bias;
+                    float v;
+                    if (lnc) {
+                        const int from = 32 * (i & 1) + (r & 3) + 8 * (r >> 2) + 4 * lk;
+                        const float mu = __shfl(mu_l[i >> 1], from, 64), rsd = __shfl(rs_l[i >> 1], from, 64);
+                        v = fmaf(rsd, fmaf(-mu, lns, acc[i][j][r] * p.alpha), bias);
+                    } else {
+                        v = acc[i][j][r] * p.alpha + bias;
+                    }
                     if (p.rowadd) v += ra[r];
                     if (resp) v += rs[r];
                     outv[r] = v;
@@ -164,6 +275,14 @@
                         }
                     }
                 } else {
+                    if (lnp) {
+                        float sum, m2;
+                        int rm;
+                        block_row_stats(outv, lrow, sum, m2, rm);
+                        const int m = mb + (rm & 3) + 8 * (rm >> 2) + 4 * lk;
+                        if ((lrow & 1) == 0 && m < p.M)
+                            *reinterpret_cast<f32x2*>(p.ln_part + ((long long)m * (p.N >> 5) + (n >> 5)) * 2) = f32x2{sum, m2};
+                    }
 #pragma unroll
                     for (int r = 0; r < 16; ++r) {
                         const int m = mb + (r & 3) + 8 * (r >> 2) + 4 * lk;
@@ -172,6 +291,7 @@
                                 store_split_pair(cp + (long long)m * p.ldc, n, outv[r]);
                             else
                                 cp[(long long)m * p.ldc + n] = outv[r];
+                            if (lnp) store_split_pair(p.ln_sp + (long long)m * p.ld_ln_sp, n, outv[r]);
                             if (p.c2) {
                                 const float w = outv[r] > 0.f ? outv[r] : outv[r] * p.c2_slope;
                                 store_split_pair(p.c2 + coff + (long long)m * p.ldc2, n, w);
@@ -180,24 +300,24 @@
                     }
                 }
             }
-        }
-    }
-}
-
-template <int MI, int NI>
+        });
+    });
+}
+
+template <int MI, int NI, bool LNF = true>
 __device__ __forceinline__ void igemm_epilogue(const IGemm& p, f32x16 (&acc)[MI][NI], int m_base, int n_base, int lrow,
                                                int lk, long long coff, int Nb, int rpb) {
-    const bool pair = !p.geglu && !p.c_split && p.c2 == nullptr && (p.N & 1) == 0 && (p.ldc & 1) == 0 && (coff & 1) == 0 &&
+    const bool pair = !p.geglu && !p.c_split && p.c2 == nullptr && p.ln_part == nullptr && (p.N & 1) == 0 && (p.ldc & 1) == 0 && (coff & 1) == 0 &&
                       (reinterpret_cast<uintptr_t>(p.c) & 7) == 0;
     const bool rsel = !(p.rowadd && rpb < 32);
     if (pair && rsel)
-        igemm_epilogue_impl<MI, NI, true, true>(p, acc, m_base, n_base, lrow, lk, coff, Nb, rpb);
+        igemm_epilogue_impl<MI, NI, true, true, LNF>(p, acc, m_base, n_base, lrow, lk, coff, Nb, rpb);
     else if (pair)
-        igemm_epilogue_impl<MI, NI, true, false>(p, acc, m_base, n_base, lrow, lk, coff, Nb, rpb);
+        igemm_epilogue_impl<MI, NI, true, false, LNF>(p, acc, m_base, n_base, lrow, lk, coff, Nb, rpb);
     else if (rsel)
-        igemm_epilogue_impl<MI, NI, false, true>(p, acc, m_base, n_base, lrow, lk, coff, Nb, rpb);
+        igemm_epilogue_impl<MI, NI, false, true, LNF>(p, acc, m_base, n_base, lrow, lk, coff, Nb, rpb);
     else
-        igemm_epilogue_impl<MI, NI, false, false>(p, acc, m_base, n_base, lrow, lk, coff, Nb, rpb);
-}
-
-}
+        igemm_epilogue_impl<MI, NI, false, false, LNF>(p, acc, m_base, n_base, lrow, lk, coff, Nb, rpb);
+}
+
+}
diff --git a/audiogpt_amd/csrc/igemm_pp.hip b/audiogpt_amd/csrc/igemm_pp.hip
--- a/audiogpt_amd/csrc/igemm_pp.hip
+++ b/audiogpt_amd/csrc/igemm_pp.hip
@@ -306,7 +306,7 @@
         const int rpb = p.Hout * p.Wout;
         const int row_base = e_m0 + grp * 128 + wm * (32 * MI), col_base = e_n0 + wn * (32 * NI);
         if constexpr (OUT == 1) {
-            igemm_epilogue<MI, NI>(p, acc, row_base, col_base, lrow, lk, UP2 ? (long long)e_phase * p.M * p.ldc : 0LL, q.Nb, rpb);
+            igemm_epilogue<MI, NI, false>(p, acc, row_base, col_base, lrow, lk, UP2 ? (long long)e_phase * p.M * p.ldc : 0LL, q.Nb, rpb);
         } else {
             float* pp = q.part + ((long long)e_slab * (MI * NI * 4) * 512 + tid) * 4;
 #pragma unroll
diff --git a/audiogpt_amd/csrc/maa_internal.h b/audiogpt_amd/csrc/maa_internal.h
--- a/audiogpt_amd/csrc/maa_internal.h
+++ b/audiogpt_amd/csrc/maa_internal.h
@@ -107,6 +107,7 @@
     bool no_dma = false;
     int halo = 2;
     bool cfg_shared = true;
+    bool ln_fold = false;
     bool gn_two_pass = false;
     void load();
 };
@@ -177,6 +178,13 @@
     float* c2 = nullptr;
     int ldc2 = 0;
     float c2_slope = 1.f;
+    float* ln_sp = nullptr;
+    int ld_ln_sp = 0;
+    float* ln_part = nullptr;
+    const float* ln_stats = nullptr;
+    int ln_nblk = 0;
+    const float* ln_s = nullptr;
+    float ln_eps = 0.f;
     const float* zeros = nullptr;
 };
 struct IGemmPlan {
@@ -295,6 +303,7 @@
     int K = 0, N = 0, Npad = 0;
     int ld = 0, nk = 0;
     int split = 0;
+    float* ln_s = nullptr;
 };
 
 bool launch_halo_conv1d(const Ctx& ctx, const float* x, int B, int L, int C, const PackedW& w, int k, int dil, float slope,
@@ -316,6 +325,10 @@
     PackedW pack_concat(const StateDict& sd, const std::vector<std::string>& wnames,
                         const std::vector<std::string>& bnames);
     PackedW pack_geglu(const StateDict& sd, const std::string& wname, const std::string& bname);
+    PackedW pack_linear_ln(const StateDict& sd, const std::vector<std::string>& wnames, const std::vector<std::string>& bnames,
+                           const std::string& gname, const std::string& betaname, bool hi_only = false);
+    PackedW pack_geglu_ln(const StateDict& sd, const std::string& wname, const std::string& bname, const std::string& gname,
+                          const std::string& betaname, bool hi_only = false);
     PackedW pack_convtr_phase(const StateDict& sd, const std::string& wname, const std::string& bname, int stride,
                               int pad, int carry, int* r_start, int* r_count);
     float* vec(const StateDict& sd, const std::string& name);
diff --git a/audiogpt_amd/csrc/runtime.cpp b/audiogpt_amd/csrc/runtime.cpp
--- a/audiogpt_amd/csrc/runtime.cpp
+++ b/audiogpt_amd/csrc/runtime.cpp
@@ -129,6 +129,7 @@
     pp_tile_major = get_s("MAA_PP_TILE_MAJOR") == "1";
     up2 = get_s("MAA_UP2") != "0";
     cfg_shared = get_s("MAA_CFG_SHARED") != "0";
+    ln_fold = get_s("MAA_LN_FOLD") == "1";
     const std::string ps = get_s("MAA_OP_PRESPLIT");
     op_presplit = !ps.empty() && ps[0] == '1';
     no_dma = !get_s("MAA_NO_DMA").empty();
@@ -423,6 +424,92 @@
     return pw;
 }
 
+static void fold_layernorm(WeightStore& ws, PackedW& pw, std::vector<float>& h, const std::vector<float>& hb, const float* gamma,
+                           const float* beta, bool hi_only) {
+    std::vector<float> s(pw.Npad, 0.f), c(pw.Npad, 0.f);
+    for (int n = 0; n < pw.Npad; ++n) {
+        double sn = 0.0, cn = hb.empty() ? 0.0 : (double)hb[n];
+        for (int k = 0; k < pw.K; ++k) {
+            float& w = h[(size_t)k * pw.Npad + n];
+            cn += (double)beta[k] * (double)w;
+            w = (float)((double)gamma[k] * (double)w);
+            const float hi = bf2f(f2bf(w));
+            sn += (double)hi + (hi_only ? 0.0 : (double)bf2f(f2bf(w - hi)));
+        }
+        s[n] = (float)sn;
+        c[n] = (float)cn;
+    }
+    ws.finish(pw, h, true);
+    pw.ln_s = ws.upload(s);
+    pw.bias = ws.upload(c);
+}
+
+PackedW WeightStore::pack_linear_ln(const StateDict& sd, const std::vector<std::string>& wnames,
+                                    const std::vector<std::string>& bnames, const std::string& gname,
+                                    const std::string& betaname, bool hi_only) {
+    PackedW pw;
+    int N = 0, Cin = -1;
+    for (auto& n : wnames) {
+        const HostTensor& w = get(sd, n);
+        const int cin = (int)(w.numel() / w.shape[0]);
+        MAA_CHECK(Cin < 0 || Cin == cin, "pack_linear_ln: input width mismatch " + n);
+        Cin = cin;
+        N += (int)w.shape[0];
+    }
+    const HostTensor& g = get(sd, gname);
+    const HostTensor& be = get(sd, betaname);
+    MAA_CHECK(g.numel() == Cin && be.numel() == Cin, "pack_linear_ln: LayerNorm width " + gname);
+    if (!nk_ || Cin % 32 != 0) return pw;
+    pw.K = Cin;
+    pw.N = N;
+    pw.Npad = pad32(N);
+    std::vector<float> h((size_t)Cin * pw.Npad, 0.f), hb(pw.Npad, 0.f);
+    int col = 0;
+    for (size_t i = 0; i < wnames.size(); ++i) {
+        const HostTensor& w = get(sd, wnames[i]);
+        const int co_n = (int)w.shape[0];
+        for (int co = 0; co < co_n; ++co)
+            for (int ci = 0; ci < Cin; ++ci) h[(size_t)ci * pw.Npad + col + co] = w.data[(size_t)co * Cin + ci];
+        if (!bnames.empty() && !bnames[i].empty()) {
+            const HostTensor& b = get(sd, bnames[i]);
+            MAA_CHECK(b.numel() == co_n, "pack_linear_ln: bias width " + bnames[i]);
+            std::memcpy(hb.data() + col, b.data, sizeof(float) * co_n);
+        }
+        col += co_n;
+    }
+    fold_layernorm(*this, pw, h, hb, g.data, be.data, hi_only);
+    return pw;
+}
+
+PackedW WeightStore::pack_geglu_ln(const StateDict& sd, const std::string& wname, const std::string& bname,
+                                   const std::string& gname, const std::string& betaname, bool hi_only) {
+    PackedW pw;
+    const HostTensor& w = get(sd, wname);
+    const HostTensor& b = get(sd, bname);
+    const HostTensor& g = get(sd, gname);
+    const HostTensor& be = get(sd, betaname);
+    const int N2 = (int)w.shape[0], Cin = (int)w.shape[1], inner = N2 / 2;
+    MAA_CHECK(inner % 32 == 0, "geglu inner width must be a multiple of 32");
+    MAA_CHECK(g.numel() == Cin && be.numel() == Cin && b.numel() == N2, "pack_geglu_ln: LayerNorm / bias width " + gname);
+    if (!nk_ || Cin % 32 != 0) return pw;
+    pw.K = Cin;
+    pw.N = inner;
+    pw.Npad = N2;
+    std::vector<float> h((size_t)Cin * N2), hb(N2);
+    for (int j = 0; j < inner; ++j) {
+        const int gq = j / 32, jj = j % 32;
+        const int cv = gq * 64 + jj, cg = gq * 64 + 32 + jj;
+        for (int ci = 0; ci < Cin; ++ci) {
+            h[(size_t)ci * N2 + cv] = w.data[(size_t)j * Cin + ci];
+            h[(size_t)ci * N2 + cg] = w.data[(size_t)(inner + j) * Cin + ci];
+        }
+        hb[cv] = b.data[j];
+        hb[cg] = b.data[inner + j];
+    }
+    fold_layernorm(*this, pw, h, hb, g.data, be.data, hi_only);
+    return pw;
+}
+
 PackedW WeightStore::pack_convtr_phase(const StateDict& sd, const std::string& wname, const std::string& bname,
                                        int stride, int pad, int carry, int* r_start, int* r_count) {
     const HostTensor& w = get(sd, wname);
diff --git a/audiogpt_amd/csrc/unet.cpp b/audiogpt_amd/csrc/unet.cpp
--- a/audiogpt_amd/csrc/unet.cpp
+++ b/audiogpt_amd/csrc/unet.cpp
@@ -18,6 +18,7 @@
 struct STBlockW {
     float *ln1g, *ln1b, *ln2g, *ln2b, *ln3g, *ln3b;
     PackedW qkv1, out1, q2, kv2, out2, ff1, ff2;
+    PackedW qkv1_ln, q2_ln, ff1_ln;
     int kv_slot = -1;
 };
 struct STW {
@@ -134,6 +135,10 @@
             b.out2 = ws.pack_conv(sd, t + "attn2.to_out.0.weight", t + "attn2.to_out.0.bias", 1, 1);
             b.ff1 = ws.pack_geglu(sd, t + "ff.net.0.proj.weight", t + "ff.net.0.proj.bias");
             b.ff2 = ws.pack_conv(sd, t + "ff.net.2.weight", t + "ff.net.2.bias", 1, 1);
+            b.qkv1_ln = ws.pack_linear_ln(sd, {t + "attn1.to_q.weight", t + "attn1.to_k.weight", t + "attn1.to_v.weight"}, {},
+                                          t + "norm1.weight", t + "norm1.bias", precision == 2);
+            b.q2_ln = ws.pack_linear_ln(sd, {t + "attn2.to_q.weight"}, {}, t + "norm2.weight", t + "norm2.bias", precision == 2);
+            b.ff1_ln = ws.pack_geglu_ln(sd, t + "ff.net.0.proj.weight", t + "ff.net.0.proj.bias", t + "norm3.weight", t + "norm3.bias", precision == 2);
             b.kv_slot = (int)kv_cache.size();
             kv_cache.push_back(nullptr);
             kv_inner.push_back(inner);
@@ -333,12 +338,23 @@
             xres = xd;
         }
         const bool sp_in = split_for_gemm(ctx, s.ch), sp = split_for_gemm(ctx, inner);
+        bool fold = ctx.tune.ln_fold && sp && sp_in && !s.blocks.empty();
+        for (const STBlockW& b : s.blocks) fold = fold && b.qkv1_ln.w && b.q2_ln.w && b.ff1_ln.w;
+        LnFold prod, cons;
+        if (fold) {
+            prod.sp = ctx.ws.alloc_f((size_t)Mo * inner);
+            prod.part = ctx.ws.alloc_f((size_t)Mo * (inner / 32) * 2);
+            cons.stats = prod.part;
+            cons.eps = 1e-5f;
+        }
+        const LnFold* lnp = fold ? &prod : nullptr;
+        const LnFold* lnc = fold ? &cons : nullptr;
         float* y = nullptr;
         if (xp != 3) {
             float* xn = ctx.ws.alloc_f((size_t)M * s.ch);
             launch_groupnorm(ctx, x.p, s.ch, s.ch, nullptr, 0, 0, B, HW, 32, s.ng, s.nb, 1e-6f, 0, xn, sp_in);
             y = ctx.ws.alloc_f((size_t)M * inner);
-            linear_into(ctx, xn, s.ch, M, s.ch, s.proj_in, nullptr, 0, y, inner, 0, 0, sp_in ? M : 0);
+            linear_into(ctx, xn, s.ch, M, s.ch, s.proj_in, nullptr, 0, y, inner, 0, 0, sp_in ? M : 0, 0, 0, lnp);
         }
         const float scale = 1.0f / std::sqrt((float)s.dh);
         const bool no_osplit = false;
@@ -347,23 +363,23 @@
         int y_sp = 0;
         for (const STBlockW& b : s.blocks) {
             const bool first_block = &b == &s.blocks.front();
-            float* ln = ctx.ws.alloc_f((size_t)Mo * inner);
+            float* ln = fold ? prod.sp : ctx.ws.alloc_f((size_t)Mo * inner);
             float* o = ctx.ws.alloc_f((size_t)Mo * inner);
             float *y1 = nullptr, *q = nullptr;
             if (xp == 3 && first_block) {
                 y1 = const_cast<float*>(prefix.y1);
                 q = const_cast<float*>(prefix.q);
             } else {
-                launch_layernorm(ctx, y, M, inner, b.ln1g, b.ln1b, 1e-5f, ln, sp);
+                if (!fold) launch_layernorm(ctx, y, M, inner, b.ln1g, b.ln1b, 1e-5f, ln, sp);
                 float* qkv = ctx.ws.alloc_f((size_t)M * 3 * inner);
-                linear_into(ctx, ln, inner, M, inner, b.qkv1, nullptr, 0, qkv, 3 * inner, 0, 0, sp ? M : 0);
+                linear_into(ctx, ln, inner, M, inner, fold ? b.qkv1_ln : b.qkv1, nullptr, 0, qkv, 3 * inner, 0, 0, sp ? M : 0, 0, 0, lnc);
                 attention_into(ctx, qkv, 3 * inner, s.dh, qkv + inner, 3 * inner, s.dh, qkv + 2 * inner, 3 * inner, s.dh,
                                B, s.heads, s.dh, HW, HW, scale, o, inner, o_sp);
                 y1 = xp == 2 && first_block ? y1_keep : ctx.ws.alloc_f((size_t)M * inner);
-                linear_into(ctx, o, inner, M, inner, b.out1, y, inner, y1, inner, 0, 0, o_sp ? M : 0);
-                launch_layernorm(ctx, y1, M, inner, b.ln2g, b.ln2b, 1e-5f, ln, sp);
+                linear_into(ctx, o, inner, M, inner, b.out1, y, inner, y1, inner, 0, 0, o_sp ? M : 0, 0, 0, lnp);
+                if (!fold) launch_layernorm(ctx, y1, M, inner, b.ln2g, b.ln2b, 1e-5f, ln, sp);
                 q = xp == 2 && first_block ? q_keep : ctx.ws.alloc_f((size_t)M * inner);
-                linear_into(ctx, ln, inner, M, inner, b.q2, nullptr, 0, q, inner, 0, 0, sp ? M : 0);
+                linear_into(ctx, ln, inner, M, inner, fold ? b.q2_ln : b.q2, nullptr, 0, q, inner, 0, 0, sp ? M : 0, 0, 0, lnc);
                 if (xp == 2 && first_block) {
                     prefix.y1 = y1;
                     prefix.q = q;
@@ -387,14 +403,14 @@
             attention_into(ctx, q, inner, s.dh, kv, 2 * inner, s.dh, kv + inner, 2 * inner, s.dh, B, s.heads, s.dh, HW,
                            kv_len, scale, o, inner, o_sp);
             float* y2 = ctx.ws.alloc_f((size_t)M * inner);
-            linear_into(ctx, o, inner, M, inner, b.out2, y1, inner, y2, inner, 0, 0, o_sp ? M : 0);
-            launch_layernorm(ctx, y2, M, inner, b.ln3g, b.ln3b, 1e-5f, ln, sp);
+            linear_into(ctx, o, inner, M, inner, b.out2, y1, inner, y2, inner, 0, 0, o_sp ? M : 0, 0, 0, lnp);
+            if (!fold) launch_layernorm(ctx, y2, M, inner, b.ln3g, b.ln3b, 1e-5f, ln, sp);
             float* g = ctx.ws.alloc_f((size_t)M * 4 * inner);
-            linear_into(ctx, ln, inner, M, inner, b.ff1, nullptr, 0, g, 4 * inner, 1, 0, sp ? M : 0, g_sp);
+            linear_into(ctx, ln, inner, M, inner, fold ? b.ff1_ln : b.ff1, nullptr, 0, g, 4 * inner, 1, 0, sp ? M : 0, g_sp, 0, lnc);
             float* y3 = ctx.ws.alloc_f((size_t)M * inner);
             const bool last = &b == &s.blocks.back();
             y_sp = last && sp && !no_osplit ? 1 : 0;
-            linear_into(ctx, g, 4 * inner, M, 4 * inner, b.ff2, y2, inner, y3, inner, 0, 0, g_sp ? M : 0, y_sp);
+            linear_into(ctx, g, 4 * inner, M, 4 * inner, b.ff2, y2, inner, y3, inner, 0, 0, g_sp ? M : 0, y_sp, 0, last ? nullptr : lnp);
             y = y3;
         }
         MAA_CHECK(B == Bo, "SpatialTransformer without a transformer block cannot part the halves of a guided step");
diff --git a/include/maa.h b/include/maa.h
--- a/include/maa.h
+++ b/include/maa.h
@@ -255,6 +255,9 @@
 
 int maa_op_linear(maa_ctx* ctx, const float* d_a, int M, int K, const float* h_w, const float* h_bias, int N,
                   int geglu, float* d_y, const float* d_res, int c_split);
+int maa_op_ln_linear(maa_ctx* ctx, const float* d_a, int M, int K0, const float* h_w0, const float* h_b0, const float* d_res,
+                     int C, const float* h_gamma, const float* h_beta, float eps, const float* h_w1, const float* h_b1, int N,
+                     int geglu, int fold, float* d_y);
 int maa_op_conv(maa_ctx* ctx, const float* d_x, int B, int Cin, int H, int W, const float* h_w, const float* h_bias,
                 int Cout, int KH, int KW, int stride, int pad, int dil, int upsample2, float leaky_slope,
                 float* d_y, int Ho, int Wo, const float* d_rowadd, const float* d_res, int c_split);
```

New measurement: 133.4 audio-seconds/sec. 2.6% lower.
